# fpthink/PDGN

Hardware: AMD Instinct MI355X
Metric: generator+D step points/sec (B=35, 256->2048 pts) (higher is better)
Workload: dtype f32; 1 GPU; PDGNet_v2 G+D iteration (models/PDGNet_v2.py:171-256), chair-shaped synthetic batch, per-GPU batch 35, 256->2048 pts, random-init weights; global_batch=35, parallelism=dp1, losses_finite=True, hipgraph=False, issue=list

## Files before the change

### include/pdgn_hip.h

```cpp
#ifndef PDGN_HIP_H
#define PDGN_HIP_H

#include <stdint.h>

#ifdef __cplusplus
extern "C" {
#endif

#define PDGN_ERR_INVALID (-1)
#define PDGN_KNN_MAX_NSAMPLE 200

typedef void *pdgn_stream_t;

#define PDGN_ABI_VERSION 38
int pdgn_abi_version(void);

int pdgn_knnquery(int b, int n, int m, int nsample, const float *xyz, const float *new_xyz,
                  int32_t *idx, float *dist2, pdgn_stream_t stream);

int pdgn_grouping_forward(int b, int c, int n, int m, int nsample, const float *points,
                          const int32_t *idx, float *out, pdgn_stream_t stream);

int pdgn_grouping_backward(int b, int c, int n, int m, int nsample, const float *grad_out,
                           const int32_t *idx, float *grad_points, pdgn_stream_t stream);

int pdgn_nearestneighbor(int b, int n, int m, const float *unknown, const float *known,
                         float *dist2, int32_t *idx, pdgn_stream_t stream);

int pdgn_interpolation_forward(int b, int c, int m, int n, const float *points,
                               const int32_t *idx, const float *weight, float *out,
                               pdgn_stream_t stream);

int pdgn_interpolation_backward(int b, int c, int n, int m, const float *grad_out,
                                const int32_t *idx, const float *weight, float *grad_points,
                                pdgn_stream_t stream);

int pdgn_nndistance(int b, int n, const float *xyz, int m, const float *xyz2, float *result,
                    int32_t *result_i, float *result2, int32_t *result2_i, pdgn_stream_t stream);

int pdgn_nndistance_grad(int b, int n, const float *xyz1, int m, const float *xyz2,
                         const float *grad_dist1, const int32_t *idx1, const float *grad_dist2,
                         const int32_t *idx2, float *grad_xyz1, float *grad_xyz2,
                         pdgn_stream_t stream);

int pdgn_approxmatch(int b, int n, int m, const float *xyz1, const float *xyz2, float *match,
                     float *temp, pdgn_stream_t stream);

int pdgn_matchcost(int b, int n, int m, const float *xyz1, const float *xyz2,
                   const float *match, float *out, pdgn_stream_t stream);

int pdgn_matchcost_grad(int b, int n, int m, const float *xyz1, const float *xyz2,
                        const float *match, float *grad1, float *grad2, pdgn_stream_t stream);

long long pdgn_emd_cost_temp_floats(long long pairs, int n, int m);
int pdgn_emd_cost(int b, int n, int m, const float *xyz1, const float *xyz2, float *temp,
                  float *out, pdgn_stream_t stream);

int pdgn_feature_knn(int b, int f, int n, int k, const float *x, float *sqnorm, int32_t *idx,
                     pdgn_stream_t stream);

int pdgn_window_gather_sum(int b, int n, int k, int ldy, int T, int P, int C, int off, int offc,
                           const float *Y, const int32_t *idx, const float *bias, int bias_bstride,
                           float *out, pdgn_stream_t stream);
int pdgn_window_gather_sum_stats(int b, int n, int k, int ldy, int T, int P, int C, int off, int offc,
                                 const float *Y, const int32_t *idx, const float *bias, int bias_bstride,
                                 float *out, float *scratch, pdgn_stream_t stream);

int pdgn_window_gather_sum_backward(int b, int n, int k, int ldy, int T, int P, int C, int off,
                                    int offc, const float *dout, const int32_t *idx, float *dY,
                                    pdgn_stream_t stream);

int pdgn_knn_graph_transpose(int b, int n, int k, const int32_t *idx, int32_t *rowptr, int32_t *edges,
                             int32_t *scratch, pdgn_stream_t stream);
int pdgn_window_gather_sum_backward_csr(int b, int n, int k, int ldy, int T, int P, int C, int off,
                                        int offc, const float *dout, const int32_t *rowptr,
                                        const int32_t *edges, float *dY, unsigned *max_out, int max_init, pdgn_stream_t stream);

long long pdgn_bn_scratch_floats(long long rows, int c);
int pdgn_bn_stats(long long rows, int c, float eps, float momentum, const float *x, const float *gamma,
                  const float *beta, const float *pre_bias, float *running_mean, float *running_var,
                  float *scratch, float *stats, pdgn_stream_t stream);
int pdgn_bn_eval_stats(int c, float eps, const float *gamma, const float *beta, const float *pre_bias,
                       const float *running_mean, const float *running_var, float *stats,
                       pdgn_stream_t stream);
int pdgn_bn_stats_from_partials(long long rows, int c, float eps, float momentum, const float *gamma,
                                const float *beta, const float *pre_bias, float *running_mean, float *running_var,
                                const float *scratch, float *stats, pdgn_stream_t stream);
int pdgn_bn_stats_from_gemm_partials(long long rows, int c, long long nparts, int block_rows, float eps, float momentum,
                                     const float *gamma, const float *beta, const float *pre_bias,
                                     float *running_mean, float *running_var, const float *partials,
                                     float *stats, double *scratch, pdgn_stream_t stream);
long long pdgn_bn_blocks_scratch_doubles(int c, long long nparts);
int pdgn_bn_act_forward(long long rows, int c, int act, const float *x, const float *stats,
                        const float *mul, float *y, int interleave_n, pdgn_stream_t stream);
int pdgn_bn_act_backward(long long rows, int c, int act, int training, const float *x,
                         const float *dy, const float *mul, const float *stats, float *scratch,
                         float *bsums, float *dx, float *dmul, int interleave_n, pdgn_stream_t stream);

long long pdgn_bn_maxpool_scratch_floats(int b, int c);
int pdgn_bn_act_maxpool(int b, int n, int c, int act, const float *x, const float *stats, float *scratch,
                        float *ymax, int32_t *yarg, pdgn_stream_t stream);
long long pdgn_bn_stats_maxpool_scratch_floats(int b, int c);
int pdgn_bn_stats_act_maxpool(int b, int n, int c, int act, float eps, float momentum, const float *x, const float *gamma,
                              const float *beta, const float *pre_bias, float *running_mean, float *running_var, float *scratch,
                              float *stats, float *ymax, int32_t *yarg, pdgn_stream_t stream);
int pdgn_bn_act_maxpool_backward(int b, int n, int c, int act, int training, const float *x,
                                 const float *dout, const int32_t *yarg, const float *stats,
                                 float *scratch, float *bsums, float *dx, pdgn_stream_t stream);
long long pdgn_dense_bn_maxpool_backward_scratch(int b, int c, int k);
int pdgn_dense_bn_maxpool_backward(int b, int n, int c, int k, int act, const float *x, const float *dout, const int32_t *yarg,
                                   const float *stats, const float *h, int ldh, const float *W, int ldw, float *scratch,
                                   float *dh, float *dW, int lddw, float *bsums, pdgn_stream_t stream);
long long pdgn_dense_bn_maxpool_input_grad_scratch(int b, int c, int k);
int pdgn_dense_bn_maxpool_input_grad(int b, int n, int c, int k, int act, const float *x, const float *dout,
                                     const int32_t *yarg, const float *stats, const float *h, int ldh,
                                     const float *W, int ldw, float *scratch, float *dh, pdgn_stream_t stream);

int pdgn_group_colsum(long long groups, long long group_rows, int c, const float *x, long long ldx, float *out,
                      pdgn_stream_t stream);

int pdgn_softmax_slots_permute(long long m, int k, int c, const float *h, float *w, pdgn_stream_t stream);
int pdgn_bn_softmax_slots_permute(long long m, int k, int c, int act, const float *x, const float *stats,
                                  float *w, pdgn_stream_t stream);
int pdgn_bn_softmax_slots_permute_mul(long long m, int k, int c, int act, const float *x, const float *stats,
                                      int act_u, const float *u, const float *stats_u, float *w, float *y,
                                      unsigned *max_out, const float *gamma_u, const float *beta_u, float bound_scale,
                                      unsigned *cmax_out, pdgn_stream_t stream);
long long pdgn_bilateral_scratch_floats(long long m, int k, int c);
int pdgn_bilateral_weighting_backward(long long m, int k, int c, int act, int training, const float *x,
                                      const float *stats_x, const float *u, const float *stats_u, const float *w,
                                      const float *dy, float *scratch, float *bsums_x, float *bsums_u, float *dx,
                                      float *du, pdgn_stream_t stream);
int pdgn_softmax_slots_permute_backward(long long m, int k, int c, const float *w, const float *dw,
                                        float *dh, pdgn_stream_t stream);

int pdgn_skinny_nt(int R, int N, int K, const float *A, int lda, const float *B, int ldb, const float *bias, float *C, int ldc,
                   pdgn_stream_t stream);
int pdgn_skinny_nn(int R, int N, int K, const float *A, int lda, const float *B, int ldb, float *C, int ldc, pdgn_stream_t stream);
int pdgn_skinny_nt_act(int R, int N, int K, const float *A, int lda, const float *B, int ldb, const float *bias, float *C, int ldc,
                       int act, pdgn_stream_t stream);
int pdgn_skinny_nn_masked(int R, int N, int K, const float *A, int lda, const float *P, int ldp, int act, const float *B,
                          int ldb, float *C, int ldc, pdgn_stream_t stream);
int pdgn_skinny_tn(int R, int N, int K, const float *A, int lda, const float *B, int ldb, float *C, int ldc, pdgn_stream_t stream);
int pdgn_split_bf16x3(int rows, int cols, const float *src, int ld_src, unsigned short *planes, int ld_planes,
                      long long plane_stride, unsigned short *planes_t, int ld_planes_t, long long plane_stride_t,
                      pdgn_stream_t stream);
int pdgn_gemm_nt_ps(long long m, int n, int k, const float *A, int lda, const unsigned short *Wplanes, int ldw, long long wplane,
                    int parts, const float *bias, const float *addend, int ldadd, float *C, int ldc, float *stat_part,
                    const float *row_bias, int ld_rb, int rows_per_group, int act, const float *gate, int ldgate,
                    pdgn_stream_t stream);
long long pdgn_gemm_tail_workspace_floats(long long m, int n, int k, int with_stats);
long long pdgn_gemm_tn_big_workspace_floats(long long m, int n, int k);
int pdgn_gemm_set_tail_workspace(float *ws, long long floats);
int pdgn_gemm_nt_ps_launch_info(long long m, int n, int k, int parts, const void **sym, int *grid);
int pdgn_gemm_aux_symbols(const void **reduce, const void **scan);
int pdgn_gemm_set_mode(int mode);
int pdgn_gemm_set_scale_slots(void *slots, long long bytes);
int pdgn_absmax_rows_cols(long long rows, int cols, const float *src, int ld, unsigned *rowmax, unsigned *colmax,
                          pdgn_stream_t stream);
int pdgn_gemm_set_operand_scales(const unsigned *max_a, const unsigned *max_w);
int pdgn_gemm_two_part(long long m, int n, int k, long long scan_bytes);
int pdgn_gemm_two_part_planes(long long m, int n, int k, long long scan_bytes);
long long pdgn_gemm_nt_ps_stat_rows(long long m, int n, int k, int parts, int plain);
int pdgn_gemm_nt_ps_stat_block_rows(long long m, int n, int k, int parts, int plain);
int pdgn_gemm_nt_ps_row_panel(long long m, int n, int k, int parts, int plain);
long long pdgn_gemm_nt_ps_workspace_floats(long long m, int n, int k, int parts, int with_stats);
int pdgn_split_f16x2(int rows, int cols, const float *src, int ld_src, unsigned short *planes, int ld_planes,
                     long long plane_stride, unsigned short *planes_t, int ld_planes_t, long long plane_stride_t,
                     pdgn_stream_t stream);
int pdgn_gemm_set_config(int cfg);
int pdgn_gemm_set_shape(int shape);
int pdgn_gemm_nt(long long m, int n, int k, const float *A, int lda, const float *W, int ldw,
                 const float *bias, const float *addend, int ldadd, float *C, int ldc, float *stat_part,
                 pdgn_stream_t stream);
long long pdgn_thin_stat_rows(long long m);
int pdgn_thin_stat_block_rows(void);
int pdgn_thin_nt(long long m, int n, int k, const float *X, int ldx, const float *W, int wrs, int wcs,
                 const float *bias, float *Y, int ldy, float *stat_part, pdgn_stream_t stream);
int pdgn_thin_nt_ex(long long m, int n, int k, const float *X, int ldx, const float *W, int wrs, int wcs,
                    const float *bias, float *Y, int ldy, float *stat_part, const float *gate, int ldgate, pdgn_stream_t stream);
int pdgn_thin_tn(long long m, int ta, int wb, const float *A, int lda, const float *B, int ldb, float *O, int osi,
                 int osj, float *sum_a, float *sum_b, pdgn_stream_t stream);
int pdgn_gemm_nn(long long m, int n, int k, const float *A, int lda, const float *Wt, int ldw,
                 const float *bias, const float *addend, int ldadd, float *C, int ldc, float *stat_part,
                 pdgn_stream_t stream);
int pdgn_gemm_tn_big(long long m, int n, int k, const float *dY, int ldy, const float *X, int ldx, float *dW, int dw_is_zero,
                     pdgn_stream_t stream);
int pdgn_gemm_nt_ex(long long m, int n, int k, const float *A, int lda, const float *W, int ldw, const float *bias,
                    const float *addend, int ldadd, float *C, int ldc, float *stat_part, const float *row_bias, int ld_rb,
                    int rows_per_group, int act, const float *gate, int ldgate, int transposed_w, pdgn_stream_t stream);
long long pdgn_gemm_nt_stat_rows(long long m, int n, int k);
int pdgn_gemm_nt_stat_block_rows(long long m, int n, int k);
int pdgn_gemm_nt_config(long long m, int n, int k, int with_stats);

int pdgn_gemm_tn(long long m, int n, int k, const float *dY, const float *X, float *dW,
                 pdgn_stream_t stream);

int pdgn_local_stats(int b, int n, int m, int k, const float *xyz, const int32_t *idx, float *mu,
                     float *cov, pdgn_stream_t stream);
int pdgn_local_stats_backward(int b, int n, int m, int k, const float *xyz, const int32_t *idx,
                              const float *dmu, const float *dcov, float *dxyz, pdgn_stream_t stream);

int pdgn_chamfer_gram(int b, int m, int n, int d, const float *x, const float *y, float *minx,
                      int32_t *argx, float *miny, int32_t *argy, pdgn_stream_t stream);
int pdgn_chamfer_gram_grad(int b, int m, int n, int d, const float *x, const float *y,
                           const float *gminx, const int32_t *argx, const float *gminy,
                           const int32_t *argy, float *gx, float *gy, pdgn_stream_t stream);
int pdgn_chamfer_gram_grad_uniform(int b, int m, int n, int d, const float *x, const float *y, const float *g,
                                   float scale, const int32_t *argx, const int32_t *argy, float *gx, float *gy,
                                   pdgn_stream_t stream);
int pdgn_scaled_sum(long long n, const float *x, float scale, float *out, pdgn_stream_t stream);
int pdgn_mse_const(long long n, const float *x, float target, float scale, float *out, pdgn_stream_t stream);
int pdgn_mse_const_count(long long n, const float *x, float target, float scale, float boundary, float *out, int32_t *count,
                         pdgn_stream_t stream);
int pdgn_mse_const_backward(long long n, const float *x, float target, float scale, const float *g, float *dx,
                            pdgn_stream_t stream);

int pdgn_emd_cost_indexed(int npairs, int n, int m, const float *xyz1, const int32_t *ia,
                          const float *xyz2, const int32_t *ib, float *temp, float *out,
                          pdgn_stream_t stream);
int pdgn_chamfer_gram_indexed(int npairs, int m, int n, int d, const float *x, const int32_t *ia,
                              const float *y, const int32_t *ib, float *minx, int32_t *argx,
                              float *miny, int32_t *argy, pdgn_stream_t stream);

int pdgn_deconv_assemble(int F, int Fo, int k, int T, int fc, const float *Wi, const float *W2, const float *Wf,
                         float *WcatC, float *WcatV, float *Wb, pdgn_stream_t stream);
int pdgn_deconv_assemble_backward(int F, int Fo, int k, int T, int fc, const float *gWcatC, const float *gWcatV,
                                  const float *gWb, float *dWi, float *dW2, float *dWf, pdgn_stream_t stream);

int pdgn_sample_bias(int b, int ldy, int nspec, const int *T, const int *C, const int *off, const int *offc,
                     const float *const *bias, const float *Yc, float *bb, pdgn_stream_t stream);
int pdgn_sample_bias_backward(int b, int ldy, int nspec, const int *T, const int *C, const int *off, const int *offc,
                              const float *g, float *dYc, float *const *dbias, pdgn_stream_t stream);

int pdgn_small_mlp_forward(int r, int k, int n, int act, int bn_mode, float eps, float momentum, const float *x,
                           const float *W, const float *bias, const float *gamma, const float *beta,
                           float *running_mean, float *running_var, float *y, float *pre, float *stat,
                           pdgn_stream_t stream);
int pdgn_small_mlp_backward(int r, int k, int n, int act, int bn_mode, const float *x, const float *dy, const float *pre,
                            const float *stat, const float *gamma, const float *beta, float *dpre, float *dgamma,
                            float *dbeta, float *dbias, float *dW, pdgn_stream_t stream);

int pdgn_ballquery(int b, int n, int m, float radius, int nsample, const float *new_xyz, const float *xyz,
                   int32_t *idx, pdgn_stream_t stream);
int pdgn_furthestsampling(int b, int n, int m, const float *xyz, float *temp, int32_t *idx, pdgn_stream_t stream);
int pdgn_gathering_forward(int b, int c, int n, int m, const float *points, const int32_t *idx, float *out,
                           pdgn_stream_t stream);
int pdgn_gathering_backward(int b, int c, int n, int m, const float *grad_out, const int32_t *idx,
                            float *grad_points, pdgn_stream_t stream);
int pdgn_grouping_int_forward(int b, int c, int n, int m, int nsample, const long long *points, const int32_t *idx,
                              long long *out, pdgn_stream_t stream);
int pdgn_featuredistribute(int b, int n, int m, const float *max_xyz, const float *xyz, int32_t *distribute_idx,
                           pdgn_stream_t stream);
int pdgn_labelstat_idx(int b, int n, int m, int nsample, int nclass, const int32_t *label_stat, const int32_t *idx,
                       int32_t *new_label_stat, pdgn_stream_t stream);
int pdgn_labelstat_ballrange(int b, int n, int m, float radius, int nclass, const float *new_xyz, const float *xyz,
                             const int32_t *label_stat, int32_t *new_label_stat, pdgn_stream_t stream);
int pdgn_labelstat_and_ballquery(int b, int n, int m, float radius, int nsample, int nclass, const float *new_xyz,
                                 const float *xyz, const int32_t *label_stat, int32_t *idx, int32_t *new_label_stat,
                                 pdgn_stream_t stream);

long long pdgn_point_max_scratch(int b, int n, int c);
int pdgn_point_max(int b, int n, int c, const float *x, float *scratch_val, int32_t *scratch_arg, float *out, int32_t *arg,
                   pdgn_stream_t stream);
int pdgn_point_max_backward(int b, int n, int c, const float *grad_out, const int32_t *arg, float *grad_x,
                            pdgn_stream_t stream);

int pdgn_spin(unsigned int microseconds, pdgn_stream_t stream);

// ... 147 lines not shown
```

### pdgn_amd/csrc/bnact.hip

```cpp
#include "common.h"

#include "bn_geom.h"
#define ACT_NONE 0
#define ACT_RELU 1
#define ACT_LEAKY 2

__device__ __forceinline__ float act_fwd(float z, int act) {
    if (act == ACT_RELU) return fmaxf(z, 0.f);
    if (act == ACT_LEAKY) return z > 0.f ? z : 0.01f * z;
    return z;
}
__device__ __forceinline__ float act_grad(float z, int act) {
    if (act == ACT_RELU) return z > 0.f ? 1.f : 0.f;
    if (act == ACT_LEAKY) return z > 0.f ? 1.f : 0.01f;
    return 1.f;
}

struct ClGeom {
    int cg, cgb, rl;
};

__global__ __launch_bounds__(BN_THREADS) void cl_stats_kernel(long long R, int C, int cgb, int rows_per_block,
                                                              const float *__restrict__ x,
                                                              float *__restrict__ part) {
// ... 784 lines not shown
    return pdgn_launch_status();
}

#define MP_SPLIT 16

__global__ __launch_bounds__(BN_THREADS) void cl_apply_max_kernel(int N, int C, int cgb, int act,
                                                                  const float *__restrict__ x,
                                                                  const float *__restrict__ stats,
                                                                  float *__restrict__ pmax, int32_t *__restrict__ parg) {
    __shared__ float smax[BN_THREADS][4];
    __shared__ int sarg[BN_THREADS][4];
    const int cgl = threadIdx.x % cgb, rlane = threadIdx.x / cgb, rl = BN_THREADS / cgb;
    const int cgi = blockIdx.x * cgb + cgl;
    const bool cok = cgi * 4 < C;
    const int b = blockIdx.z, sp = blockIdx.y;
    const int per = (N + MP_SPLIT - 1) / MP_SPLIT;
    const int n0 = sp * per, n1 = min(N, n0 + per);
    float best[4] = {-INFINITY, -INFINITY, -INFINITY, -INFINITY};
    int arg[4] = {n0, n0, n0, n0};
    if (cok) {
        float sc[4], sh[4];
        *reinterpret_cast<float4 *>(sc) = *reinterpret_cast<const float4 *>(stats + cgi * 4);
        *reinterpret_cast<float4 *>(sh) = *reinterpret_cast<const float4 *>(stats + C + cgi * 4);
        const float *X = x + ((size_t)b * N) * C + cgi * 4;
        for (int n = n0 + rlane; n < n1; n += rl) {
            float v[4];
            *reinterpret_cast<float4 *>(v) = *reinterpret_cast<const float4 *>(X + (size_t)n * C);
#pragma unroll
            for (int j = 0; j < 4; ++j) {
                const float y = act_fwd(__fmaf_rn(v[j], sc[j], sh[j]), act);
                if (y > best[j]) { best[j] = y; arg[j] = n; }
            }
        }
    }
#pragma unroll
    for (int j = 0; j < 4; ++j) { smax[threadIdx.x][j] = best[j]; sarg[threadIdx.x][j] = arg[j]; }
    __syncthreads();
    if (rlane == 0 && cok) {
        for (int q = 1; q < rl; ++q)
#pragma unroll
            for (int j = 0; j < 4; ++j) {
                const float y = smax[q * cgb + cgl][j];
                const int a = sarg[q * cgb + cgl][j];
                if (y > best[j] || (y == best[j] && a < arg[j])) { best[j] = y; arg[j] = a; }
            }
        const size_t o = ((size_t)b * MP_SPLIT + sp) * C + cgi * 4;
        *reinterpret_cast<float4 *>(pmax + o) = *reinterpret_cast<float4 *>(best);
        *reinterpret_cast<int4 *>(parg + o) = *reinterpret_cast<int4 *>(arg);
    }
}

__global__ void cl_max_finalize_kernel(int B, int C, const float *__restrict__ pmax, const int32_t *__restrict__ parg,
                                       float *__restrict__ ymax, int32_t *__restrict__ yarg) {
    const int e = blockIdx.x * blockDim.x + threadIdx.x;
    if (e >= B * C) return;
    const int b = e / C, c = e % C;
    float best = -INFINITY;
    int arg = 0;
    for (int s = 0; s < MP_SPLIT; ++s) {
        const float y = pmax[((size_t)b * MP_SPLIT + s) * C + c];
        if (y > best) { best = y; arg = parg[((size_t)b * MP_SPLIT + s) * C + c]; }
    }
    ymax[e] = best;
    yarg[e] = arg;
}

__global__ __launch_bounds__(BN_THREADS) void cl_stats_max_kernel(int N, int C, int cgb, const float *__restrict__ x,
                                                                  float *__restrict__ part, float *__restrict__ pmax,
                                                                  int32_t *__restrict__ pargmax, float *__restrict__ pmin,
                                                                  int32_t *__restrict__ pargmin) {
    __shared__ float4 red[4][BN_THREADS];
    __shared__ int4 redi[2][BN_THREADS];
    const int cgl = threadIdx.x % cgb, rlane = threadIdx.x / cgb, rl = BN_THREADS / cgb;
    const int cgi = blockIdx.x * cgb + cgl;
    const bool cok = cgi * 4 < C;
    const int b = blockIdx.z, sp = blockIdx.y;
    const int per = (N + MP_SPLIT - 1) / MP_SPLIT;
    const int n0 = sp * per, n1 = min(N, n0 + per);
    float s[4] = {0.f, 0.f, 0.f, 0.f}, q[4] = {0.f, 0.f, 0.f, 0.f};
    float mx[4] = {-INFINITY, -INFINITY, -INFINITY, -INFINITY}, mn[4] = {INFINITY, INFINITY, INFINITY, INFINITY};
    int amx[4] = {n0, n0, n0, n0}, amn[4] = {n0, n0, n0, n0};
    if (cok) {
        float pv[4];
        *reinterpret_cast<float4 *>(pv) = *reinterpret_cast<const float4 *>(x + cgi * 4);
        const float *X = x + ((size_t)b * N) * C + cgi * 4;
        for (int n = n0 + rlane; n < n1; n += rl) {
            float v[4];
            *reinterpret_cast<float4 *>(v) = *reinterpret_cast<const float4 *>(X + (size_t)n * C);
#pragma unroll
            for (int j = 0; j < 4; ++j) {
                const float d = v[j] - pv[j];
                s[j] += d;
                q[j] = __fmaf_rn(d, d, q[j]);
                if (v[j] > mx[j]) { mx[j] = v[j]; amx[j] = n; }
                if (v[j] < mn[j]) { mn[j] = v[j]; amn[j] = n; }
            }
        }
    }
    red[0][threadIdx.x] = make_float4(s[0], s[1], s[2], s[3]);
    red[1][threadIdx.x] = make_float4(q[0], q[1], q[2], q[3]);
    red[2][threadIdx.x] = make_float4(mx[0], mx[1], mx[2], mx[3]);
    red[3][threadIdx.x] = make_float4(mn[0], mn[1], mn[2], mn[3]);
    redi[0][threadIdx.x] = make_int4(amx[0], amx[1], amx[2], amx[3]);
    redi[1][threadIdx.x] = make_int4(amn[0], amn[1], amn[2], amn[3]);
    __syncthreads();
    if (rlane || !cok) return;
    for (int k = 1; k < rl; ++k) {
        const int t = k * cgb + cgl;
        const float *a = &red[0][t].x, *bq = &red[1][t].x, *c2 = &red[2][t].x, *d2 = &red[3][t].x;
        const int *i2 = &redi[0][t].x, *j2 = &redi[1][t].x;
#pragma unroll
        for (int j = 0; j < 4; ++j) {
            s[j] += a[j];
            q[j] += bq[j];
            if (c2[j] > mx[j] || (c2[j] == mx[j] && i2[j] < amx[j])) { mx[j] = c2[j]; amx[j] = i2[j]; }
            if (d2[j] < mn[j] || (d2[j] == mn[j] && j2[j] < amn[j])) { mn[j] = d2[j]; amn[j] = j2[j]; }
        }
    }
    const size_t blk = (size_t)b * MP_SPLIT + sp;
    float *P = part + blk * 2 * C;
    *reinterpret_cast<float4 *>(P + cgi * 4) = make_float4(s[0], s[1], s[2], s[3]);
    *reinterpret_cast<float4 *>(P + C + cgi * 4) = make_float4(q[0], q[1], q[2], q[3]);
    const size_t o = blk * C + cgi * 4;
    *reinterpret_cast<float4 *>(pmax + o) = make_float4(mx[0], mx[1], mx[2], mx[3]);
    *reinterpret_cast<int4 *>(pargmax + o) = make_int4(amx[0], amx[1], amx[2], amx[3]);
    *reinterpret_cast<float4 *>(pmin + o) = make_float4(mn[0], mn[1], mn[2], mn[3]);
    *reinterpret_cast<int4 *>(pargmin + o) = make_int4(amn[0], amn[1], amn[2], amn[3]);
}

__global__ void cl_max_pick_kernel(int B, int C, int act, const float *__restrict__ stats, const float *__restrict__ pmax,
                                   const int32_t *__restrict__ pargmax, const float *__restrict__ pmin,
                                   const int32_t *__restrict__ pargmin, float *__restrict__ ymax, int32_t *__restrict__ yarg) {
    const int e = blockIdx.x * blockDim.x + threadIdx.x;
    if (e >= B * C) return;
    const int b = e / C, c = e - b * C;
    const float sc = stats[c], sh = stats[C + c];
    const bool up = sc >= 0.f;
    const float *pv = up ? pmax : pmin;
    const int32_t *pa = up ? pargmax : pargmin;
    float best = pv[((size_t)b * MP_SPLIT) * C + c];
    int arg = pa[((size_t)b * MP_SPLIT) * C + c];
    for (int s = 1; s < MP_SPLIT; ++s) {
        const float v = pv[((size_t)b * MP_SPLIT + s) * C + c];
        if (up ? v > best : v < best) { best = v; arg = pa[((size_t)b * MP_SPLIT + s) * C + c]; }
    }
    ymax[e] = act_fwd(__fmaf_rn(best, sc, sh), act);
    yarg[e] = arg;
}

__global__ __launch_bounds__(256) void cl_max_bwd_sums_kernel(int B, int N, int C, int act, int training,
                                                              const float *__restrict__ x, const float *__restrict__ dout,
                                                              const int32_t *__restrict__ yarg, const float *__restrict__ stats,
                                                              float *__restrict__ dz, float *__restrict__ bsums,
                                                              float *__restrict__ coef, float *__restrict__ zero, int nzero) {
    __shared__ double p1[16][17], p2[16][17];
    for (int e = blockIdx.x * 256 + threadIdx.x; e < nzero; e += gridDim.x * 256) zero[e] = 0.f;
    const int cl = threadIdx.x & 15, bl = threadIdx.x >> 4;
    const int c = blockIdx.x * 16 + cl;
    double s1 = 0, s2 = 0;
    float sc = 0.f, mu = 0.f, is = 0.f;
    if (c < C) {
        sc = stats[c];
        mu = stats[2 * C + c];
        is = stats[3 * C + c];
        const float sh = stats[C + c];
        for (int b = bl; b < B; b += 16) {
            const int n = yarg[b * C + c];
            const float v = x[((size_t)b * N + n) * C + c];
            const float g = dout[b * C + c] * act_grad(__fmaf_rn(v, sc, sh), act);
            dz[b * C + c] = g;
            s1 += g;
            s2 += (double)g * (double)((v - mu) * is);
        }
    }
    p1[bl][cl] = s1;
    p2[bl][cl] = s2;
    __syncthreads();
    if (bl || c >= C) return;
    for (int q = 1; q < 16; ++q) { s1 += p1[q][cl]; s2 += p2[q][cl]; }
    bsums[c] = (float)s1;
    bsums[C + c] = (float)s2;
    float ca = 0.f, cb = 0.f;
    if (training) {
        const double R = (double)B * (double)N;
        cb = sc * is * (float)(s2 / R);
        ca = sc * (float)(s1 / R) - cb * mu;
    }
    coef[c] = ca;
    coef[C + c] = cb;
}

__global__ __launch_bounds__(BN_THREADS) void cl_max_bwd_apply_kernel(int N, int C, int cgb, const float *__restrict__ x,
                                                                      const float *__restrict__ stats,
                                                                      const float *__restrict__ coef,
                                                                      const float *__restrict__ dz,
                                                                      const int32_t *__restrict__ yarg,
                                                                      float *__restrict__ dx) {
    const int cgl = threadIdx.x % cgb, rlane = threadIdx.x / cgb, rl = BN_THREADS / cgb;
    const int cgi = blockIdx.x * cgb + cgl;
    if (cgi * 4 >= C) return;
    const int b = blockIdx.z, sp = blockIdx.y;
    const int per = (N + MP_SPLIT - 1) / MP_SPLIT;
    const int n0 = sp * per, n1 = min(N, n0 + per);
    float sc[4], ca[4], cb[4], g[4];
    int arg[4];
    *reinterpret_cast<float4 *>(sc) = *reinterpret_cast<const float4 *>(stats + cgi * 4);
    *reinterpret_cast<float4 *>(ca) = *reinterpret_cast<const float4 *>(coef + cgi * 4);
    *reinterpret_cast<float4 *>(cb) = *reinterpret_cast<const float4 *>(coef + C + cgi * 4);
    *reinterpret_cast<float4 *>(g) = *reinterpret_cast<const float4 *>(dz + (size_t)b * C + cgi * 4);
    *reinterpret_cast<int4 *>(arg) = *reinterpret_cast<const int4 *>(yarg + (size_t)b * C + cgi * 4);
    const size_t base = ((size_t)b * N) * C + cgi * 4;
    for (int n = n0 + rlane; n < n1; n += rl) {
        float v[4], o[4];
        *reinterpret_cast<float4 *>(v) = *reinterpret_cast<const float4 *>(x + base + (size_t)n * C);
#pragma unroll
        for (int j = 0; j < 4; ++j) o[j] = (n == arg[j] ? sc[j] * g[j] : 0.f) - ca[j] - cb[j] * v[j];
        *reinterpret_cast<float4 *>(dx + base + (size_t)n * C) = *reinterpret_cast<float4 *>(o);
    }
}

static void mp_geometry(int C, int *cgb, int *gx) {
    const int cg = C / 4;
    int p = 1;
    while (p < cg && p < 64) p <<= 1;
    *cgb = p;
    *gx = (cg + p - 1) / p;
}

extern "C" long long pdgn_bn_maxpool_scratch_floats(int b, int c) { return 2LL * b * MP_SPLIT * c; }

extern "C" int pdgn_bn_act_maxpool(int b, int n, int c, int act, const float *x, const float *stats, float *scratch,
                                   float *ymax, int32_t *yarg, pdgn_stream_t stream) {
    if (b < 1 || n < 1 || c < 4 || c % 4 || act < 0 || act > 2 || b > 65535) return PDGN_ERR_INVALID;
    hipStream_t s = (hipStream_t)stream;
    int cgb, gx;
    mp_geometry(c, &cgb, &gx);
    float *pmax = scratch;
    int32_t *parg = reinterpret_cast<int32_t *>(scratch + (size_t)b * MP_SPLIT * c);
    hipLaunchKernelGGL(cl_apply_max_kernel, dim3(gx, MP_SPLIT, b), dim3(BN_THREADS), 0, s, n, c, cgb, act, x, stats, pmax, parg);
    hipLaunchKernelGGL(cl_max_finalize_kernel, dim3(cdiv((long long)b * c, 256)), dim3(256), 0, s, b, c, pmax, parg, ymax, yarg);
    return pdgn_launch_status();
}

extern "C" long long pdgn_bn_stats_maxpool_scratch_floats(int b, int c) { return 6LL * b * MP_SPLIT * c; }

extern "C" int pdgn_bn_stats_act_maxpool(int b, int n, int c, int act, float eps, float momentum, const float *x, const float *gamma,
                                         const float *beta, const float *pre_bias, float *running_mean, float *running_var,
                                         float *scratch, float *stats, float *ymax, int32_t *yarg, pdgn_stream_t stream) {
    if (b < 1 || n < 1 || c < 4 || c % 4 || act < 0 || act > 2 || b > 65535) return PDGN_ERR_INVALID;
    hipStream_t s = (hipStream_t)stream;
    int cgb, gx;
    mp_geometry(c, &cgb, &gx);
    const size_t bc = (size_t)b * MP_SPLIT * c;
    float *part = scratch, *pmax = part + 2 * bc, *pmin = pmax + 2 * bc;
    int32_t *pargmax = reinterpret_cast<int32_t *>(pmax + bc), *pargmin = reinterpret_cast<int32_t *>(pmin + bc);
    hipLaunchKernelGGL(cl_stats_max_kernel, dim3(gx, MP_SPLIT, b), dim3(BN_THREADS), 0, s, n, c, cgb, x, part, pmax, pargmax, pmin,
                       pargmin);
    hipLaunchKernelGGL(cl_finalize_kernel, dim3(cdiv(c, FIN_CH)), dim3(FIN_CH * FIN_PL), 0, s, (long long)b * n, c, b * MP_SPLIT, eps,
                       momentum, part, gamma, beta, pre_bias, running_mean, running_var, stats, x);
    hipLaunchKernelGGL(cl_max_pick_kernel, dim3(cdiv((long long)b * c, 256)), dim3(256), 0, s, b, c, act, stats, pmax, pargmax, pmin,
                       pargmin, ymax, yarg);
    return pdgn_launch_status();
}

extern "C" int pdgn_bn_act_maxpool_backward(int b, int n, int c, int act, int training, const float *x,
                                            const float *dout, const int32_t *yarg, const float *stats, float *scratch,
                                            float *bsums, float *dx, pdgn_stream_t stream) {
    if (b < 1 || n < 1 || c < 4 || c % 4 || act < 0 || act > 2 || b > 65535) return PDGN_ERR_INVALID;
    hipStream_t s = (hipStream_t)stream;
    float *dz = scratch, *coef = scratch + (size_t)b * c;
    hipLaunchKernelGGL(cl_max_bwd_sums_kernel, dim3(cdiv(c, 16)), dim3(256), 0, s, b, n, c, act, training, x, dout, yarg,
                       stats, dz, bsums, coef, nullptr, 0);
    int cgb, gx;
    mp_geometry(c, &cgb, &gx);
    hipLaunchKernelGGL(cl_max_bwd_apply_kernel, dim3(gx, MP_SPLIT, b), dim3(BN_THREADS), 0, s, n, c, cgb, x, stats, coef, dz,
                       yarg, dx);
    return pdgn_launch_status();
}

#define CF_TILE 32
#define CF_CSPLIT 8
#define CF_RSPLIT 32

__global__ __launch_bounds__(256) void cf_gram_kernel(int C, int K, const float *__restrict__ W, int ldw,
                                                      const float *__restrict__ coef, float *__restrict__ Gneg,
                                                      float *__restrict__ vneg) {
    __shared__ float part[3][64][20];
    const int t = threadIdx.x, o = t & 63, sl = __builtin_amdgcn_readfirstlane(t >> 6);
    const int i = blockIdx.y * CF_TILE + (o >> 3) * 4, j = blockIdx.x * CF_TILE + (o & 7) * 4;
    const bool ok = i < K && j < K, do_v = blockIdx.y == 0 && (o >> 3) == 0 && j < K;
    const int ii = min(i, K - 4), jj = min(j, K - 4);
    const int nsl = CF_CSPLIT * 4, per = (C + nsl - 1) / nsl;
    const int c0 = (blockIdx.z * 4 + sl) * per, c1 = min(C, c0 + per);
    const float *cb = coef + C;
    float acc[4][4] = {}, av[4] = {};
    for (int c = c0; c < c1; c += 8) {
        float4 wi[8], wj[8];
#pragma unroll
        for (int u = 0; u < 8; ++u) {
            const float *w = W + (size_t)min(c + u, c1 - 1) * ldw;
            wi[u] = *reinterpret_cast<const float4 *>(w + ii);
            wj[u] = *reinterpret_cast<const float4 *>(w + jj);
        }
        __builtin_amdgcn_sched_barrier(0);
#pragma unroll
        for (int u = 0; u < 8; ++u) {
            const int cc = min(c + u, c1 - 1);
            const float live = c + u < c1 ? 1.f : 0.f;
            const float s = cb[cc] * live, a = coef[cc] * live;
            const float x[4] = {wi[u].x * s, wi[u].y * s, wi[u].z * s, wi[u].w * s};
            const float y[4] = {wj[u].x, wj[u].y, wj[u].z, wj[u].w};
#pragma unroll
            for (int p = 0; p < 4; ++p)
#pragma unroll
                for (int q = 0; q < 4; ++q) acc[p][q] = __fmaf_rn(x[p], y[q], acc[p][q]);
#pragma unroll
            for (int q = 0; q < 4; ++q) av[q] = __fmaf_rn(a, y[q], av[q]);
        }
    }
    if (sl) {
#pragma unroll
        for (int p = 0; p < 4; ++p)
#pragma unroll
            for (int q = 0; q < 4; ++q) part[sl - 1][o][p * 4 + q] = acc[p][q];
#pragma unroll
        for (int q = 0; q < 4; ++q) part[sl - 1][o][16 + q] = av[q];
    }
    __syncthreads();
    if (sl) return;
#pragma unroll
    for (int w = 0; w < 3; ++w) {
#pragma unroll
        for (int p = 0; p < 4; ++p)
#pragma unroll
            for (int q = 0; q < 4; ++q) acc[p][q] += part[w][o][p * 4 + q];
#pragma unroll
        for (int q = 0; q < 4; ++q) av[q] += part[w][o][16 + q];
    }
    if (ok)
#pragma unroll
        for (int p = 0; p < 4; ++p)
#pragma unroll
            for (int q = 0; q < 4; ++q) atomicAdd(&Gneg[(size_t)(i + p) * K + j + q], -acc[p][q]);
    if (do_v)
#pragma unroll
        for (int q = 0; q < 4; ++q) atomicAdd(&vneg[j + q], -av[q]);
}

__global__ __launch_bounds__(256) void cf_scatter_kernel(int N, int C, int K, const float *__restrict__ W, int ldw,
                                                         const float *__restrict__ stats, const float *__restrict__ dz,
                                                         const int32_t *__restrict__ yarg, float *__restrict__ dh) {
    extern __shared__ unsigned char cf_lds[];
    __shared__ unsigned int ndist;
    const int maxd = min(N, C);
    unsigned short *table = reinterpret_cast<unsigned short *>(cf_lds);
    unsigned short *rows = table + N;
    unsigned short *args = rows + maxd;
    unsigned int *cnt = reinterpret_cast<unsigned int *>(cf_lds + (((size_t)(N + maxd + C) * 2 + 15) & ~(size_t)15));
    float *cf = reinterpret_cast<float *>(cnt + 256);
    const int t = threadIdx.x, b = blockIdx.y;
    const int32_t *arg = yarg + (size_t)b * C;
    for (int n = t; n < N; n += 256) table[n] = 0;
    __syncthreads();
    for (int c = t; c < C; c += 256) {
        const int a = arg[c];
        table[a] = 1;
        args[c] = (unsigned short)a;
        cf[c] = stats[c] * dz[(size_t)b * C + c];
    }
    __syncthreads();
    const int per = (N + 255) / 256, lo = t * per, hi = min(N, lo + per);
    unsigned int mine = 0;
    for (int n = lo; n < hi; ++n) mine += table[n];
    cnt[t] = mine;
    __syncthreads();
    if (t < 64) {
        const unsigned int v0 = cnt[4 * t], v1 = cnt[4 * t + 1], v2 = cnt[4 * t + 2], v3 = cnt[4 * t + 3];
        const unsigned int s = v0 + v1 + v2 + v3;
        unsigned int incl = s;
#pragma unroll
        for (int d = 1; d < 64; d <<= 1) {
            const unsigned int up = __shfl_up(incl, d, 64);
            if (t >= d) incl += up;
        }
        const unsigned int ex = incl - s;
        cnt[4 * t] = ex;
        cnt[4 * t + 1] = ex + v0;
        cnt[4 * t + 2] = ex + v0 + v1;
        cnt[4 * t + 3] = ex + v0 + v1 + v2;
    }
    __syncthreads();
    unsigned int at = cnt[t];
    for (int n = lo; n < hi; ++n)
        if (table[n]) rows[at++] = (unsigned short)n;
    if (t == 255) ndist = at;
    __syncthreads();
    const int nd = (int)ndist, lane = t & 63, wv = t >> 6;
    const bool lok = lane * 4 < K;
    const int col = min(lane * 4, K - 4);
    for (int r = blockIdx.x * 4 + wv; r < nd; r += CF_RSPLIT * 4) {
        const int n = rows[r];
        float *dst = dh + ((size_t)b * N + n) * K + col;
        const float4 cur = *reinterpret_cast<const float4 *>(dst);
        float4 acc = make_float4(0.f, 0.f, 0.f, 0.f);
        for (int c0 = 0; c0 < C; c0 += 64) {
            unsigned long long m = __ballot(c0 + lane < C && args[min(c0 + lane, C - 1)] == n);
            while (m) {
                const int c = c0 + __builtin_ctzll(m);
                m &= m - 1;
                const float g = cf[c];
                const float4 w = *reinterpret_cast<const float4 *>(W + (size_t)c * ldw + col);
                acc.x = __fmaf_rn(g, w.x, acc.x);
                acc.y = __fmaf_rn(g, w.y, acc.y);
                acc.z = __fmaf_rn(g, w.z, acc.z);
                acc.w = __fmaf_rn(g, w.w, acc.w);
            }
        }
        if (lok) *reinterpret_cast<float4 *>(dst) = make_float4(cur.x + acc.x, cur.y + acc.y, cur.z + acc.z, cur.w + acc.w);
    }
}

static size_t cf_scatter_lds(int n, int c) {
    const int maxd = n < c ? n : c;
    return (((size_t)(n + maxd + c) * 2 + 15) & ~(size_t)15) + 256 * 4 + (size_t)c * 4;
}

#define CFS_THREADS 1024
__global__ __launch_bounds__(CFS_THREADS) void cf_colsum_kernel(long long rows, int K, const float *__restrict__ h, int ldh,
                                                                float *__restrict__ hs) {
    __shared__ float4 red[CFS_THREADS];
    const int kg = K / 4, cg = threadIdx.x % kg, rl = threadIdx.x / kg, nrl = CFS_THREADS / kg;
    const long long per = (rows + gridDim.x - 1) / gridDim.x, r0 = blockIdx.x * per, r1 = min(rows, r0 + per);
    float4 acc = make_float4(0.f, 0.f, 0.f, 0.f);
    for (long long r = r0 + rl; r < r1; r += 8 * nrl) {
        float4 v[8];
#pragma unroll
        for (int u = 0; u < 8; ++u) {
            const long long rr = r + (long long)u * nrl;
            v[u] = rr < r1 ? *reinterpret_cast<const float4 *>(h + rr * ldh + cg * 4) : make_float4(0.f, 0.f, 0.f, 0.f);
        }
#pragma unroll
        for (int u = 0; u < 8; ++u) { acc.x += v[u].x; acc.y += v[u].y; acc.z += v[u].z; acc.w += v[u].w; }
    }
    red[threadIdx.x] = acc;
    __syncthreads();
    if (rl) return;
    for (int q = 1; q < nrl; ++q) {
        const float4 v = red[q * kg + cg];
        acc.x += v.x; acc.y += v.y; acc.z += v.z; acc.w += v.w;
    }
    atomicAdd(&hs[cg * 4], acc.x); atomicAdd(&hs[cg * 4 + 1], acc.y); atomicAdd(&hs[cg * 4 + 2], acc.z); atomicAdd(&hs[cg * 4 + 3], acc.w);
}

__global__ __launch_bounds__(256) void cf_dw_kernel(int B, int N, int C, int K, const float *__restrict__ h, int ldh,
                                                    const int32_t *__restrict__ yarg, const float *__restrict__ stats,
                                                    const float *__restrict__ dz, const float *__restrict__ coef,
                                                    const float *__restrict__ hs, const float *__restrict__ T,
                                                    float *__restrict__ dW, int lddw) {
    const int lane = threadIdx.x & 63, c = blockIdx.x * 4 + (threadIdx.x >> 6);
    if (c >= C || lane * 4 >= K) return;
    const int col = lane * 4;
    const float sc = stats[c];
    float4 acc = make_float4(0.f, 0.f, 0.f, 0.f);
    for (int b0 = 0; b0 < B; b0 += 8) {
        float4 v[8];
        float g[8];
#pragma unroll
        for (int u = 0; u < 8; ++u) {
            const int b = min(b0 + u, B - 1);
            g[u] = b0 + u < B ? sc * dz[(size_t)b * C + c] : 0.f;
            v[u] = *reinterpret_cast<const float4 *>(h + ((size_t)b * N + yarg[(size_t)b * C + c]) * ldh + col);
        }
#pragma unroll
        for (int u = 0; u < 8; ++u) {
            acc.x = __fmaf_rn(g[u], v[u].x, acc.x);
            acc.y = __fmaf_rn(g[u], v[u].y, acc.y);
            acc.z = __fmaf_rn(g[u], v[u].z, acc.z);
            acc.w = __fmaf_rn(g[u], v[u].w, acc.w);
        }
    }
    const float ca = coef[c], cb = coef[C + c];
    const float4 s = *reinterpret_cast<const float4 *>(hs + col), t = *reinterpret_cast<const float4 *>(T + (size_t)c * K + col);
    *reinterpret_cast<float4 *>(dW + (size_t)c * lddw + col) =
        make_float4(acc.x - ca * s.x - cb * t.x, acc.y - ca * s.y - cb * t.y, acc.z - ca * s.z - cb * t.z, acc.w - ca * s.w - cb * t.w);
}

extern "C" long long pdgn_dense_bn_maxpool_backward_scratch(int b, int c, int k) {
    return (long long)b * c + 2LL * c + 2LL * ((long long)k * k + k) + (long long)c * k;
}

extern "C" int pdgn_dense_bn_maxpool_backward(int b, int n, int c, int k, int act, const float *x, const float *dout,
                                              const int32_t *yarg, const float *stats, const float *h, int ldh, const float *W,
                                              int ldw, float *scratch, float *dh, float *dW, int lddw, float *bsums,
                                              pdgn_stream_t stream) {
    if (b < 1 || n < 1 || n > 65535 || c < 4 || c % 4 || k < 4 || k % 4 || k > 256 || ldw % 4 || ((uintptr_t)W & 15) ||
        ((uintptr_t)dh & 15) || act < 0 || act > 2 || b > 65535 || cf_scatter_lds(n, c) > 64 * 1024)
        return PDGN_ERR_INVALID;
    if (dW && (k < 16 || (k & (k - 1)) || ldh % 4 || lddw % 4 || ((uintptr_t)h & 15) || ((uintptr_t)dW & 15)))
        return PDGN_ERR_INVALID;
    hipStream_t s = (hipStream_t)stream;
    const size_t kk = (size_t)k * k;
    float *dz = scratch, *coef = dz + (size_t)b * c, *G = coef + 2 * (size_t)c, *v = G + kk, *H = v + k, *hs = H + kk, *T = hs + k;
    float *bs = bsums ? bsums : T;
    hipLaunchKernelGGL(cl_max_bwd_sums_kernel, dim3(cdiv(c, 16)), dim3(256), 0, s, b, n, c, act, 1, x, dout, yarg, stats, dz, bs,
                       coef, G, (int)(2 * (kk + k)));
    int rc = pdgn_launch_status();
    if (rc) return rc;
    if (dh) {
        const int gt = cdiv(k, CF_TILE);
        hipLaunchKernelGGL(cf_gram_kernel, dim3(gt, gt, CF_CSPLIT), dim3(256), 0, s, c, k, W, ldw, coef, G, v);
        if ((rc = pdgn_launch_status())) return rc;
        if ((rc = pdgn_gemm_nt((long long)b * n, k, k, h, ldh, G, k, v, nullptr, 0, dh, k, nullptr, stream))) return rc;
        hipLaunchKernelGGL(cf_scatter_kernel, dim3(CF_RSPLIT, b), dim3(256), cf_scatter_lds(n, c), s, n, c, k, W, ldw, stats, dz,
                           yarg, dh);
        if ((rc = pdgn_launch_status())) return rc;
    }
    if (dW) {
        const long long rows = (long long)b * n;
        hipLaunchKernelGGL(cf_colsum_kernel, dim3(rows >= 32768 ? 128 : (rows >= 8192 ? 64 : 16)), dim3(CFS_THREADS), 0, s, rows, k, h, ldh, hs);
        if ((rc = pdgn_launch_status())) return rc;
        if ((rc = pdgn_gemm_tn_big(rows, k, k, h, ldh, h, ldh, H, 1, stream))) return rc;
        if ((rc = pdgn_gemm_nt(c, k, k, W, ldw, H, k, nullptr, nullptr, 0, T, k, nullptr, stream))) return rc;
        hipLaunchKernelGGL(cf_dw_kernel, dim3(cdiv(c, 4)), dim3(256), 0, s, b, n, c, k, h, ldh, yarg, stats, dz, coef, hs, T, dW, lddw);
        rc = pdgn_launch_status();
    }
    return rc;
}

extern "C" long long pdgn_dense_bn_maxpool_input_grad_scratch(int b, int c, int k) {
    return pdgn_dense_bn_maxpool_backward_scratch(b, c, k);
}

extern "C" int pdgn_dense_bn_maxpool_input_grad(int b, int n, int c, int k, int act, const float *x, const float *dout,
                                                const int32_t *yarg, const float *stats, const float *h, int ldh,
                                                const float *W, int ldw, float *scratch, float *dh, pdgn_stream_t stream) {
    return pdgn_dense_bn_maxpool_backward(b, n, c, k, act, x, dout, yarg, stats, h, ldh, W, ldw, scratch, dh, nullptr, 4, nullptr,
                                          stream);
}

__global__ __launch_bounds__(256) void group_colsum_kernel(long long group_rows, int C, const float *__restrict__ x, long long ldx,
                                                           float *__restrict__ out) {
    __shared__ float4 red[256];
    const int kg = C / 4, per_pass = kg < 256 ? kg : 256;
    const int cgl = threadIdx.x % per_pass, rl = threadIdx.x / per_pass, nrl = 256 / per_pass;
    const long long g = blockIdx.y;
    const long long per = (group_rows + gridDim.x - 1) / gridDim.x, r0 = blockIdx.x * per, r1 = min(group_rows, r0 + per);
    const float *X = x + g * group_rows * ldx;
    for (int c0 = 0; c0 < kg; c0 += per_pass) {
        const int cg = c0 + cgl;
        float4 acc = make_float4(0.f, 0.f, 0.f, 0.f);
        for (long long r = r0 + rl; r < r1; r += 8 * nrl) {
            float4 v[8];
#pragma unroll
            for (int u = 0; u < 8; ++u) {
                const long long rr = r + (long long)u * nrl;
                v[u] = rr < r1 ? *reinterpret_cast<const float4 *>(X + rr * ldx + cg * 4) : make_float4(0.f, 0.f, 0.f, 0.f);
            }
#pragma unroll
            for (int u = 0; u < 8; ++u) { acc.x += v[u].x; acc.y += v[u].y; acc.z += v[u].z; acc.w += v[u].w; }
        }
        __syncthreads();
        red[threadIdx.x] = acc;
        __syncthreads();
        if (rl == 0) {
            for (int q = 1; q < nrl; ++q) {
                const float4 v = red[q * per_pass + cgl];
                acc.x += v.x; acc.y += v.y; acc.z += v.z; acc.w += v.w;
            }
            float *o = out + g * C + cg * 4;
            if (gridDim.x == 1) *reinterpret_cast<float4 *>(o) = acc;
            else { atomicAdd(o, acc.x); atomicAdd(o + 1, acc.y); atomicAdd(o + 2, acc.z); atomicAdd(o + 3, acc.w); }
        }
    }
}

extern "C" int pdgn_group_colsum(long long groups, long long group_rows, int c, const float *x, long long ldx, float *out,
                                 pdgn_stream_t stream) {
    if (groups < 1 || group_rows < 1 || c < 16 || c > 1024 || (c & (c - 1)) || ldx < c || ldx % 4 || ((uintptr_t)x & 15) ||
        ((uintptr_t)out & 15) || groups > 65535)
        return PDGN_ERR_INVALID;
    const int kg = c / 4, nrl = kg < 256 ? 256 / kg : 1;
    long long splits = 1024 / groups;
    splits = splits > 128 ? 128 : splits;
    const long long max_splits = group_rows / (8LL * nrl * 8) > 0 ? group_rows / (8LL * nrl * 8) : 1;
    splits = splits < 1 ? 1 : (splits > max_splits ? max_splits : splits);
    hipLaunchKernelGGL(group_colsum_kernel, dim3((unsigned)splits, (unsigned)groups), dim3(256), 0, (hipStream_t)stream, group_rows, c, x,
                       ldx, out);
    return pdgn_launch_status();
}
```

### pdgn_amd/csrc/gemm_shared.h

```cpp
#pragma once
#include <type_traits>

#include "common.h"

typedef float f32x4 __attribute__((ext_vector_type(4)));
typedef unsigned u32x4 __attribute__((ext_vector_type(4)));
typedef __attribute__((address_space(3))) void lds_void_t;

#define NT_BK 32
#define NT_GROUP_M 8
#define NT_OOB 0x40000000u

typedef int i32x4 __attribute__((ext_vector_type(4)));

__device__ __forceinline__ i32x4 nt_srd(const void *base, unsigned bytes) {
    const unsigned long long b = (unsigned long long)base;
    i32x4 r;
    r.x = __builtin_amdgcn_readfirstlane((int)(unsigned)b);
    r.y = __builtin_amdgcn_readfirstlane((int)((unsigned)(b >> 32) & 0xffffu));
    r.z = __builtin_amdgcn_readfirstlane((int)bytes);
    r.w = 0x00020000;
    return r;
}

__device__ __forceinline__ void nt_dma16(i32x4 srd, unsigned lds_base, unsigned voff, unsigned soff) {
    asm volatile("s_mov_b32 m0, %0\n\ts_nop 0\n\tbuffer_load_dwordx4 %1, %2, %3 offen lds"
                 :
                 : "s"(lds_base), "v"(voff), "s"(srd), "s"(soff)
                 : "memory", "m0");
}

struct NtArgs {
    long long M;
    int N, K, lda, ldw, ldc, ldadd;
    const float *A, *W, *bias, *addend;
    float *C, *stat_part;
    int tiles_m, tiles_n, tile_begin, tile_end, kchunks;
    long long sk_per_wg;
    int sk_split;
    float *sk_ws;
    int sk_seg;
    int dbg;
    const float *row_bias;
    int ld_rb, rows_per_group;
    unsigned rpg_magic;
    int rb_bytes;
    int act;
    const float *gate;
    int ldgate;
    const unsigned short *Wp;
    long long wplane;
    const unsigned *max_a, *max_w;
};

__device__ __forceinline__ int x2_exponent(unsigned maxbits) {
    const int e = 14 - ((int)(maxbits >> 23) - 127);
    return e > 126 ? 126 : (e < -126 ? -126 : e);
}
__device__ __forceinline__ int x2_scale_field(unsigned maxbits) {
    const int f = 268 - (int)(maxbits >> 23);
    return f < 1 ? 1 : (f > 253 ? 253 : f);
}
__device__ __forceinline__ float x2_scale(unsigned maxbits) { return __int_as_float(x2_scale_field(maxbits) << 23); }
__device__ __forceinline__ float x2_unscale(unsigned maxbits) { return __int_as_float((254 - x2_scale_field(maxbits)) << 23); }

struct NtDev {
    int cus;
};
static inline int nt_cus() {
    static int cached = 0;
    if (!cached) {
        int dev = 0, cus = 0;
        if (hipGetDevice(&dev) != hipSuccess ||
            hipDeviceGetAttribute(&cus, hipDeviceAttributeMultiprocessorCount, dev) != hipSuccess || cus < 1)
            return 256;
        cached = cus;
    }
    return cached;
}

struct NtSwitches {
    int mode, cfg, splitk, shape16, shape16_default;
};
NtSwitches &nt_switches();

struct NtEpi {
    const float *row_bias = nullptr;
    int ld_rb = 0, rows_per_group = 1, act = 0;
    const float *gate = nullptr;
    int ldgate = 0;
    bool any() const { return row_bias || act || gate; }
};


int fp32_gemm_nt(long long m, int n, int k, const float *A, int lda, const float *W, int ldw, const float *bias,
                 const float *addend, int ldadd, float *C, int ldc, float *stat_part, pdgn_stream_t stream);
int fp32_gemm_nn(long long m, int n, int k, const float *A, int lda, const float *Wt, int ldw, const float *bias,
                 const float *addend, int ldadd, float *C, int ldc, float *stat_part, pdgn_stream_t stream);
int fp32_gemm_nt_ex(long long m, int n, int k, const float *A, int lda, const float *W, int ldw, const float *bias,
                    const float *addend, int ldadd, float *C, int ldc, float *stat_part, const float *row_bias, int ld_rb,
                    int rows_per_group, int act, const float *gate, int ldgate, int transposed_w, pdgn_stream_t stream);
int fp32_gemm_tn_big(long long m, int n, int k, const float *dY, int ldy, const float *X, int ldx, float *dW,
                     pdgn_stream_t stream);
long long fp32_gemm_nt_stat_rows(long long m, int n, int k);
int fp32_gemm_nt_stat_block_rows(long long m, int n, int k);
int fp32_gemm_nt_config(long long m, int n, int k, int with_stats);
```

### pdgn_amd/csrc/gemm_x3.hip

```cpp
#include <atomic>
#include <type_traits>

#include "gemm_shared.h"

#ifndef X3_FENCE
#define X3_FENCE 2
#endif
#ifndef X3_DEFAULT_MASK
#define X3_DEFAULT_MASK 0x000
#endif
#ifndef X3_FENCE16
#define X3_FENCE16 2
#endif
#ifndef X3_ABLATE
#define X3_ABLATE 0
#endif

typedef float f32x16 __attribute__((ext_vector_type(16)));
typedef float f32x2 __attribute__((ext_vector_type(2)));
typedef __bf16 bf16x8 __attribute__((ext_vector_type(8)));
typedef __bf16 bf16x2 __attribute__((ext_vector_type(2)));

struct X3Parts {
    u32x4 h, m, l;
};

__device__ __forceinline__ unsigned x3_cvt_pk(float a, float b) {
    const f32x2 v = {a, b};
    return __builtin_bit_cast(unsigned, __builtin_convertvector(v, bf16x2));
}

__device__ __forceinline__ void x3_split_pair(float a, float b, X3Parts &P, int e) {
    const unsigned h = x3_cvt_pk(a, b);
    const float ra = a - __uint_as_float(h << 16), rb = b - __uint_as_float(h & 0xffff0000u);
    const unsigned m = x3_cvt_pk(ra, rb);
    const float sa = ra - __uint_as_float(m << 16), sb = rb - __uint_as_float(m & 0xffff0000u);
    P.h[e] = h;
    P.m[e] = m;
    P.l[e] = x3_cvt_pk(sa, sb);
}

__device__ __forceinline__ f32x16 x3_mfma(const u32x4 a, const u32x4 b, const f32x16 c) {
    return __builtin_amdgcn_mfma_f32_32x32x16_bf16(__builtin_bit_cast(bf16x8, a), __builtin_bit_cast(bf16x8, b), c, 0, 0, 0);
}

typedef _Float16 f16x8 __attribute__((ext_vector_type(8)));
typedef _Float16 f16x2 __attribute__((ext_vector_type(2)));
__device__ __forceinline__ unsigned x2_cvt_pk(float a, float b) {
    const f32x2 v = {a, b};
    return __builtin_bit_cast(unsigned, __builtin_convertvector(v, f16x2));
}
__device__ __forceinline__ f32x16 x2_mfma(const u32x4 a, const u32x4 b, const f32x16 c) {
    return __builtin_amdgcn_mfma_f32_32x32x16_f16(__builtin_bit_cast(f16x8, a), __builtin_bit_cast(f16x8, b), c, 0, 0, 0);
}
#ifndef X2_PRODUCTS
#define X2_PRODUCTS 3
#endif

typedef float f32x4a __attribute__((ext_vector_type(4)));
__device__ __forceinline__ f32x4a x3_mfma16(const u32x4 a, const u32x4 b, const f32x4a c) {
    return __builtin_amdgcn_mfma_f32_16x16x32_bf16(__builtin_bit_cast(bf16x8, a), __builtin_bit_cast(bf16x8, b), c, 0, 0, 0);
}

template <int MS>
__device__ __forceinline__ unsigned x3_sw(unsigned r) {
    const unsigned x = (r >> 2) & 3u;
    return MS == 32 ? x : ((0x78u >> (2u * x)) & 3u);
}

template <int CTRL, int ROW_MASK>
__device__ __forceinline__ float x3_dpp_add(float v) {
    return v + __int_as_float(__builtin_amdgcn_update_dpp(0, __float_as_int(v), CTRL, ROW_MASK, 0xf, true));
}

__device__ __forceinline__ float x3_half_wave_sum(float v) {
    v = x3_dpp_add<0x111, 0xf>(v);
    v = x3_dpp_add<0x112, 0xf>(v);
    v = x3_dpp_add<0x114, 0xf>(v);
    v = x3_dpp_add<0x118, 0xf>(v);
    return x3_dpp_add<0x142, 0xa>(v);
}

__device__ __forceinline__ float x3_row_sum(float v) {
    v = x3_dpp_add<0x111, 0xf>(v);
    v = x3_dpp_add<0x112, 0xf>(v);
    v = x3_dpp_add<0x114, 0xf>(v);
    return x3_dpp_add<0x118, 0xf>(v);
}

template <int TM, int TN, int WM, int WN, int OCC, bool ATOMIC, bool WT, bool AT, bool EPI = false, bool PW = false, int MS = 32, int NP = 3>
__global__ __launch_bounds__(64 * WM * WN, OCC) void gemm_x3_kernel(const NtArgs p) {
    static_assert(!PW || (!WT && !AT), "pre-split second operand: row-major (N x K) planes only");
    static_assert(MS == 32 || MS == 16, "matrix instruction: 32x32x16 or 16x16x32");
    static_assert(NP == 3 || (NP == 2 && MS == 32), "parts: three bf16, or two fp16 on the 32x32x16 instruction");
    constexpr int NW = WM * WN, NTH = 64 * NW, BM = 32 * TM * WM, BN = 32 * TN * WN;
    constexpr int PART_A = BM * 64, PART_W = BN * 64, STAGE = NP * (PART_A + PART_W);
    constexpr int UNT = NP == 2 ? (BM + BN) * 4 : 0;
    constexpr bool STG = OCC == 1 && !ATOMIC && !(X3_ABLATE & 128) && 2 * STAGE + NW * 4096 + UNT <= 160 * 1024;
    __shared__ __attribute__((aligned(1024))) unsigned char smem[2 * STAGE + (STG ? NW * 4096 : 0) + UNT];
    float *const untab = reinterpret_cast<float *>(smem + 2 * STAGE + (STG ? NW * 4096 : 0));

    const int tid = threadIdx.x, lane = tid & 63;
    const int wave = __builtin_amdgcn_readfirstlane(tid >> 6);
    const int wm = wave / WN, wn = wave % WN;
    const int li = MS == 32 ? lane & 31 : lane & 15, lg = MS == 32 ? lane >> 5 : lane >> 4;

    const int G = gridDim.x, pid = blockIdx.x;
    const int gq = G >> 3, gr = G & 7, xcd = pid & 7;
    const int v = xcd * gq + min(xcd, gr) + (pid >> 3);

    const int KC = p.kchunks;
    auto decode = [&](int tile, int &tm, int &tn) {
        const int per_group = NT_GROUP_M * p.tiles_n;
        const int grp = tile / per_group, r = tile - grp * per_group;
        const int first = grp * NT_GROUP_M;
        const int gsz = min(NT_GROUP_M, p.tiles_m - first);
        tn = r / gsz;
        tm = first + (r - tn * gsz);
    };
    struct Cur {
        int tile, kb, kc, ke;
        int j;
        long long f, f1;
        bool valid;
    };
    auto next_item = [&](Cur &c) {
        if (p.sk_split && (ATOMIC || p.sk_ws)) {
            const int slice = v / p.sk_split;
            c.tile = p.tile_begin + v % p.sk_split;
            c.kc = c.kb = (int)(slice * p.sk_per_wg);
            c.ke = min(KC, c.kb + (int)p.sk_per_wg);
            c.valid = c.j == 0 && c.kb < KC;
            c.j++;
        } else if (ATOMIC || (p.sk_ws && p.sk_seg)) {
            c.valid = c.f < c.f1;
            c.j++;
            if (c.valid) {
                c.tile = p.tile_begin + (int)(c.f / KC);
                c.kc = c.kb = (int)(c.f % KC);
                const long long left = c.f1 - c.f;
                c.ke = (left < (long long)(KC - c.kc)) ? c.kc + (int)left : KC;
                c.f += c.ke - c.kc;
            }
        } else {
            c.tile = p.tile_begin + v + c.j * G;
            c.valid = c.tile < p.tile_end;
            c.kc = c.kb = 0;
            c.ke = KC;
            c.j++;
        }
    };
    Cur ld, cp;
    ld.j = 0;
    ld.f = (long long)v * p.sk_per_wg;
    {
        const long long total = (long long)(p.tile_end - p.tile_begin) * KC;
        ld.f1 = min(total, ld.f + p.sk_per_wg);
    }
    ld.tile = ld.kb = ld.kc = ld.ke = 0;
    ld.valid = false;
    next_item(ld);
    cp = ld;
    if (!ld.valid) return;

    constexpr int QA = BM * 8 / NTH, QW = PW ? BN * 4 / NTH : BN * 8 / NTH, NQ = QA + QW;
    static_assert(QA * NTH == BM * 8 && QW * NTH == BN * (PW ? 4 : 8), "loader quads must divide over the threads");
    constexpr int CUA = QA % 4 == 0 ? 4 : 2, CUW = QW % 4 == 0 ? 4 : 2;
    static_assert((!AT || QA % CUA == 0) && (!WT || QW % CUW == 0), "transposed operand: whole units per thread");
    float raw[NQ][4];
    unsigned rawp[PW ? QW : 1][12];
    unsigned goffA0, goffW0, woffA0, woffW0;
    int kqA, kqW;
    {
        const int r8 = lane >> 3, c16 = lane & 7;
        kqA = kqW = c16;
        if (!AT) {
            const int row = wave * 8 + r8;
            goffA0 = (unsigned)(row * p.lda + 4 * c16) * 4u;
            woffA0 = (unsigned)(row * 64 + (((c16 >> 1) ^ x3_sw<MS>(row)) * 16) + (c16 & 1) * 8);
        } else {
            const int cq = tid % (BM / CUA), kq = tid / (BM / CUA);
            goffA0 = (unsigned)((4 * kq) * p.lda + CUA * cq) * 4u;
            woffA0 = 0;
        }
        if (PW) {
            const int row = tid >> 2, col = tid & 3;
            kqW = 2 * col;
            goffW0 = (unsigned)(row * p.ldw + 8 * col) * 2u;
            woffW0 = (unsigned)(NP * PART_A + row * 64 + ((col ^ x3_sw<MS>(row)) * 16));
        } else if (!WT) {
            const int row = wave * 8 + r8;
            goffW0 = (unsigned)(row * p.ldw + 4 * c16) * 4u;
            woffW0 = (unsigned)(NP * PART_A + row * 64 + (((c16 >> 1) ^ x3_sw<MS>(row)) * 16) + (c16 & 1) * 8);
        } else {
            const int cq = tid % (BN / CUW), kq = tid / (BN / CUW);
            goffW0 = (unsigned)((4 * kq) * p.ldw + CUW * cq) * 4u;
            woffW0 = 0;
        }
    }
    constexpr int KQ_STEP_A = NTH / (BM / CUA > NTH ? NTH : BM / CUA), KQ_STEP_W = NTH / (BN / CUW > NTH ? NTH : BN / CUW);
    static_assert(!AT || (BM / CUA <= NTH && NTH % (BM / CUA) == 0), "A^T units");
    static_assert(!WT || (BN / CUW <= NTH && NTH % (BN / CUW) == 0), "W^T units");

    __amdgpu_buffer_rsrc_t rsA, rsW;
    long long ld_m0 = 0;
    int ld_n0 = 0, ld_mrows = 0, ld_nrows = 0;
    constexpr int NSA = NP == 2 ? (AT ? CUA : QA) : 1, NSW = (NP == 2 && !PW) ? (WT ? CUW : QW) : 1;
    float scA[NSA], scW[NSW];
    unsigned nxA[NSA], nxW[NSW];
    auto make_srds = [&](int tile) {
        int tm, tn;
        decode(tile, tm, tn);
        ld_m0 = (long long)tm * BM;
        ld_n0 = tn * BN;
        ld_mrows = (int)min((long long)BM, p.M - ld_m0);
        ld_nrows = min(BN, p.N - ld_n0);
    };
    make_srds(ld.tile);
    auto fetch_maxima = [&]() {
        if (NP != 2) return;
        int lane_ = __builtin_amdgcn_mbcnt_hi(~0u, __builtin_amdgcn_mbcnt_lo(~0u, 0u));
        asm volatile("" : "+v"(lane_));
        const int tid_ = wave * 64 + lane_;
        const __amdgpu_buffer_rsrc_t rA = __builtin_amdgcn_make_buffer_rsrc((void *)(p.max_a + ld_m0), 0, ld_mrows * 4, 0x00020000);
        if (!AT) {
#pragma unroll
            for (int j = 0; j < NSA; ++j) nxA[j] = (unsigned)__builtin_amdgcn_raw_buffer_load_b32(rA, (unsigned)(wave * 8 + (lane_ >> 3) + j * NW * 8) * 4u, 0, 0);
        } else if (CUA == 4) {
            const u32x4 x = __builtin_bit_cast(u32x4, __builtin_amdgcn_raw_buffer_load_b128(rA, (unsigned)(tid_ % (BM / CUA)) * 16u, 0, 0));
#pragma unroll
            for (int j = 0; j < NSA; ++j) nxA[j] = x[j];
        } else {
            typedef unsigned u32x2_ __attribute__((ext_vector_type(2)));
            const u32x2_ x = __builtin_bit_cast(u32x2_, __builtin_amdgcn_raw_buffer_load_b64(rA, (unsigned)(tid_ % (BM / CUA)) * 8u, 0, 0));
#pragma unroll
            for (int j = 0; j < NSA; ++j) nxA[j] = x[j];
        }
        if (PW) return;
        const __amdgpu_buffer_rsrc_t rW = __builtin_amdgcn_make_buffer_rsrc((void *)(p.max_w + ld_n0), 0, ld_nrows * 4, 0x00020000);
        if (!WT) {
#pragma unroll
            for (int j = 0; j < NSW; ++j) nxW[j] = (unsigned)__builtin_amdgcn_raw_buffer_load_b32(rW, (unsigned)(wave * 8 + (lane_ >> 3) + j * NW * 8) * 4u, 0, 0);
        } else if (CUW == 4) {
            const u32x4 x = __builtin_bit_cast(u32x4, __builtin_amdgcn_raw_buffer_load_b128(rW, (unsigned)(tid_ % (BN / CUW)) * 16u, 0, 0));
#pragma unroll
            for (int j = 0; j < NSW; ++j) nxW[j] = x[j];
        } else {
            typedef unsigned u32x2_ __attribute__((ext_vector_type(2)));
            const u32x2_ x = __builtin_bit_cast(u32x2_, __builtin_amdgcn_raw_buffer_load_b64(rW, (unsigned)(tid_ % (BN / CUW)) * 8u, 0, 0));
#pragma unroll
            for (int j = 0; j < NSW; ++j) nxW[j] = x[j];
// ... 93 lines not shown
            const float a2 = a * sc, b2 = b * sc;
            const unsigned h = x2_cvt_pk(a2, b2);
            const f16x2 hh = __builtin_bit_cast(f16x2, h);
            cvh[e] = h;
            cvl[e] = x2_cvt_pk(a2 - (float)hh[0], b2 - (float)hh[1]);
            return;
        }
        const unsigned h = x3_cvt_pk(a, b);
        const float ra = a - __uint_as_float(h << 16), rb = b - __uint_as_float(h & 0xffff0000u);
        const unsigned m = x3_cvt_pk(ra, rb);
        const float sa = ra - __uint_as_float(m << 16), sb = rb - __uint_as_float(m & 0xffff0000u);
        cvh[e] = h;
        cvm[e] = m;
        cvl[e] = x3_cvt_pk(sa, sb);
    };
    auto conv_write = [&](int st, int q) {
        const bool isA = q < QA;
        const bool tr = isA ? AT : WT;
        const int j = isA ? q : q - QA;
        const int ps = isA ? PART_A : PART_W;
        unsigned off = isA ? woffA0 : woffW0;
        if (PW && !isA) {
            off += (unsigned)(j * (NTH / 4) * 64);
        } else if (!tr) {
            off += (unsigned)(j * NW * 8 * 64);
        } else {
            const int CU = isA ? CUA : CUW;
            const int d = (j / CU) * (isA ? KQ_STEP_A : KQ_STEP_W);
            const int kq0 = isA ? (int)(tid / (BM / CUA)) : (int)(tid / (BN / CUW));
            const int cq = isA ? (int)(tid % (BM / CUA)) : (int)(tid % (BN / CUW));
            const int row = CU * cq + (j % CU), kq = kq0 + d;
            off = (unsigned)((isA ? 0 : NP * PART_A) + row * 64 + (((kq >> 1) ^ x3_sw<MS>(row)) * 16) + (kq & 1) * 8);
        }
        unsigned char *dst = smem + st * STAGE + off;
        typedef unsigned u32x2 __attribute__((ext_vector_type(2)));
        if (PW && !isA) {
#pragma unroll
            for (int part = 0; part < NP; ++part)
                *reinterpret_cast<u32x4 *>(dst + part * ps) = (u32x4){rawp[j][4 * part], rawp[j][4 * part + 1], rawp[j][4 * part + 2], rawp[j][4 * part + 3]};
            return;
        }
        if (X3_ABLATE & 64) {
            *reinterpret_cast<u32x2 *>(dst) = (u32x2){cvh[0] ^ cvm[0] ^ cvl[0], cvh[1] ^ cvm[1] ^ cvl[1]};
            return;
        }
        *reinterpret_cast<u32x2 *>(dst) = (u32x2){cvh[0], cvh[1]};
        if (NP == 2) {
            *reinterpret_cast<u32x2 *>(dst + ps) = (u32x2){cvl[0], cvl[1]};
            return;
        }
        *reinterpret_cast<u32x2 *>(dst + ps) = (u32x2){cvm[0], cvm[1]};
        *reinterpret_cast<u32x2 *>(dst + 2 * ps) = (u32x2){cvl[0], cvl[1]};
    };

    constexpr int FR = MS == 32 ? 32 : 16;
    constexpr int FA = 32 * TM / FR, FW = 32 * TN / FR, NPAR = MS == 32 ? 2 : 1;
    const unsigned a_rd = (unsigned)((wm * 32 * TM + li) * 64 + ((lg ^ x3_sw<MS>(li)) * 16));
    const unsigned w_rd = (unsigned)(NP * PART_A + (wn * 32 * TN + li) * 64 + ((lg ^ x3_sw<MS>(li)) * 16));
    X3Parts fa[NPAR][FA], fw[NPAR][FW];
    auto read_frag = [&](int st, int s, int par, int r) {
        const int f = r / NP, part = NP == 2 ? 2 * (r % NP) : r % NP;
        if (f < FA) {
            const u32x4 x = *reinterpret_cast<const u32x4 *>(smem + st * STAGE + ((a_rd ^ (unsigned)(32 * s)) + f * FR * 64 + (NP == 2 ? part / 2 : part) * PART_A));
            if (part == 0) fa[par][f].h = x;
            else if (part == 1) fa[par][f].m = x;
            else fa[par][f].l = x;
        } else {
            const int b = f - FA;
            const u32x4 x = *reinterpret_cast<const u32x4 *>(smem + st * STAGE + ((w_rd ^ (unsigned)(32 * s)) + b * FR * 64 + (NP == 2 ? part / 2 : part) * PART_W));
            if (part == 0) fw[par][b].h = x;
            else if (part == 1) fw[par][b].m = x;
            else fw[par][b].l = x;
        }
    };
    auto read_part = [&](int st, bool isA, int part, int f) {
        read_frag(st, 0, 0, 3 * (isA ? f : FA + f) + part);
    };

    f32x16 acc[TM][TN];
#pragma unroll
    for (int a = 0; a < TM; ++a)
#pragma unroll
        for (int b = 0; b < TN; ++b)
#pragma unroll
            for (int r = 0; r < 16; ++r) acc[a][b][r] = 0.f;

    constexpr int NBB = MS == 32 ? 4 * TN : 2 * TN, NA = FA;
    auto coloff = [](int bb) { return MS == 32 ? 32 * (bb >> 2) + 8 * (bb & 3) : 16 * bb; };
    auto get4 = [&](int a, int bb) {
        const int A_ = MS == 32 ? a : a >> 1, b = MS == 32 ? bb >> 2 : bb >> 1, q = MS == 32 ? bb & 3 : 2 * (a & 1) + (bb & 1);
        return (f32x4){acc[A_][b][4 * q], acc[A_][b][4 * q + 1], acc[A_][b][4 * q + 2], acc[A_][b][4 * q + 3]};
    };
    auto set4 = [&](int a, int bb, const f32x4 x) {
        const int A_ = MS == 32 ? a : a >> 1, b = MS == 32 ? bb >> 2 : bb >> 1, q = MS == 32 ? bb & 3 : 2 * (a & 1) + (bb & 1);
        acc[A_][b][4 * q] = x[0]; acc[A_][b][4 * q + 1] = x[1]; acc[A_][b][4 * q + 2] = x[2]; acc[A_][b][4 * q + 3] = x[3];
    };
    const int ldc_eff = (!ATOMIC && p.sk_ws) ? BN : p.ldc;
    __amdgpu_buffer_rsrc_t rsC = __builtin_amdgcn_make_buffer_rsrc((void *)p.C, 0, 0, 0x00020000);
    unsigned st_off[NBB];
#pragma unroll
    for (int bb = 0; bb < NBB; ++bb) st_off[bb] = NT_OOB;
    unsigned stg_off[TN];
#pragma unroll
    for (int b = 0; b < TN; ++b) stg_off[b] = NT_OOB;
    unsigned char *const stg = smem + 2 * STAGE + wave * 4096;
    u32x4 pend[4];
    auto stage_block = [&](int a, int b) {
        int lane = __builtin_amdgcn_mbcnt_hi(~0u, __builtin_amdgcn_mbcnt_lo(~0u, 0u));
        asm volatile("" : "+v"(lane));
        const int li = MS == 32 ? lane & 31 : lane & 15, lg = MS == 32 ? lane >> 5 : lane >> 4;
        const unsigned stg_wr = (unsigned)(li * 128), stg_sw = (unsigned)(li & 7);
        const unsigned stg_rd = (unsigned)((lane >> 3) * 128 + (((lane & 7) ^ (lane >> 3)) * 16));
#pragma unroll
        for (int q = 0; q < 4; ++q) {
            if (MS == 32)
                *reinterpret_cast<u32x4 *>(stg + stg_wr + (((unsigned)(2 * q + lg) ^ stg_sw) * 16)) = __builtin_bit_cast(u32x4, get4(a, 4 * b + q));
            else
                *reinterpret_cast<u32x4 *>(stg + stg_wr + (q >> 1) * 2048 + (((unsigned)(4 * (q & 1) + lg) ^ stg_sw) * 16)) =
                    __builtin_bit_cast(u32x4, get4(2 * a + (q >> 1), 2 * b + (q & 1)));
        }
#pragma unroll
        for (int j = 0; j < 4; ++j) pend[j] = *reinterpret_cast<const u32x4 *>(stg + stg_rd + j * 1024);
    };
    auto flush_block = [&](int a, int b) {
#pragma unroll
        for (int j = 0; j < 4; ++j)
            if (!(X3_ABLATE & 4))
                __builtin_amdgcn_raw_buffer_store_b128(pend[j], rsC, stg_off[b] + (unsigned)((a * 32 + 8 * j) * ldc_eff) * 4u, 0, 0);
    };
    auto store_block = [&](int a, int b) {
        if (STG) {
            stage_block(a, b);
            flush_block(a, b);
            return;
        }
#pragma unroll
        for (int q = 0; q < 4; ++q) {
            const int ra = MS == 32 ? a : 2 * a + (q >> 1), bb = MS == 32 ? 4 * b + q : 2 * b + (q & 1);
            const unsigned off = st_off[bb] + (unsigned)(ra * FR * ldc_eff) * 4u;
            if (!(X3_ABLATE & 4)) __builtin_amdgcn_raw_buffer_store_b128(__builtin_bit_cast(u32x4, get4(ra, bb)), rsC, off, 0, 0);
        }
    };
    auto finish_item = [&]() {
        int lane = __builtin_amdgcn_mbcnt_hi(~0u, __builtin_amdgcn_mbcnt_lo(~0u, 0u));
        asm volatile("" : "+v"(lane));
        const int li = MS == 32 ? lane & 31 : lane & 15, lg = MS == 32 ? lane >> 5 : lane >> 4;
        const int mloc0 = wm * 32 * TM + li, nloc0 = wn * 32 * TN + 4 * lg;
        int tm, tn;
        decode(cp.tile, tm, tn);
        const long long m0 = (long long)tm * BM;
        const int n0 = tn * BN;
        const bool to_ws = !ATOMIC && p.sk_ws != nullptr;
        if (NP == 2) {
            if (!ATOMIC) {
                float ua[TM];
#pragma unroll
                for (int a = 0; a < TM; ++a) ua[a] = untab[mloc0 + 32 * a];
#pragma unroll
                for (int bb = 0; bb < NBB; ++bb) {
                    const f32x4 uw = *reinterpret_cast<const f32x4 *>(untab + BM + nloc0 + coloff(bb));
#pragma unroll
                    for (int a = 0; a < TM; ++a) set4(a, bb, (get4(a, bb) * ua[a]) * uw);
                }
            } else {
                const int mla = wm * 32 * TM + 4 * lg, nla = wn * 32 * TN + li;
#pragma unroll
                for (int b = 0; b < TN; ++b) {
                    const float uw = untab[BM + nla + 32 * b];
#pragma unroll
                    for (int a = 0; a < TM; ++a)
#pragma unroll
                        for (int q = 0; q < 4; ++q) {
                            const f32x4 ua4 = *reinterpret_cast<const f32x4 *>(untab + mla + 32 * a + 8 * q);
#pragma unroll
                            for (int r = 0; r < 4; ++r) acc[a][b][4 * q + r] = (acc[a][b][4 * q + r] * ua4[r]) * uw;
                        }
                }
            }
        }
        const long long mrows = to_ws ? BM : min((long long)BM, p.M - m0);
        const int ncols = to_ws ? BN : min(BN, p.N - n0);
        if (!ATOMIC) {
            if (to_ws) rsC = __builtin_amdgcn_make_buffer_rsrc((void *)(p.sk_ws + (size_t)(p.sk_seg ? v * p.sk_seg + (cp.j - 1) : v) * BM * BN), 0,
                                                               BM * BN * 4, 0x00020000);
            else rsC = __builtin_amdgcn_make_buffer_rsrc((void *)(p.C + m0 * p.ldc + n0), 0, (int)(mrows * p.ldc * 4), 0x00020000);
#pragma unroll
            for (int bb = 0; bb < NBB; ++bb)
                st_off[bb] = (nloc0 + coloff(bb) < ncols && !(p.dbg & 1)) ? (unsigned)(mloc0 * ldc_eff + nloc0 + coloff(bb)) * 4u : NT_OOB;
#pragma unroll
            for (int b = 0; b < TN; ++b) {
                const int nl = wn * 32 * TN + 32 * b + 4 * (lane & 7);
                stg_off[b] = (nl < ncols && !(p.dbg & 1)) ? (unsigned)((wm * 32 * TM + (lane >> 3)) * ldc_eff + nl) * 4u : NT_OOB;
            }
            if (p.addend) {
                __amdgpu_buffer_rsrc_t rsD = __builtin_amdgcn_make_buffer_rsrc((void *)(p.addend + m0 * p.ldadd + n0), 0,
                                                                               (int)(mrows * p.ldadd * 4), 0x00020000);
#pragma unroll
                for (int bb = 0; bb < NBB; ++bb)
#pragma unroll
                    for (int a = 0; a < NA; ++a) {
                        const int ml = mloc0 + FR * a, nl = nloc0 + coloff(bb);
                        set4(a, bb, get4(a, bb) + __builtin_bit_cast(f32x4, __builtin_amdgcn_raw_buffer_load_b128(
                                                      rsD, nl < ncols ? (unsigned)(ml * p.ldadd + nl) * 4u : NT_OOB, 0, 0)));
                    }
            }
            if (p.bias) {
                __amdgpu_buffer_rsrc_t rsB = __builtin_amdgcn_make_buffer_rsrc((void *)(p.bias + n0), 0, ncols * 4, 0x00020000);
#pragma unroll
                for (int bb = 0; bb < NBB; ++bb) {
                    const f32x4 bz = __builtin_bit_cast(f32x4, __builtin_amdgcn_raw_buffer_load_b128(rsB, (unsigned)(nloc0 + coloff(bb)) * 4u, 0, 0));
#pragma unroll
                    for (int a = 0; a < NA; ++a) set4(a, bb, get4(a, bb) + bz);
                }
            }
            if (EPI && p.row_bias) {
                __amdgpu_buffer_rsrc_t rsR = __builtin_amdgcn_make_buffer_rsrc((void *)p.row_bias, 0, p.rb_bytes, 0x00020000);
#pragma unroll
                for (int a = 0; a < NA; ++a) {
                    const unsigned row = (unsigned)(m0 + mloc0 + FR * a);
                    const unsigned grp = row < (unsigned)p.M ? (p.rows_per_group == 1 ? row : __umulhi(row, p.rpg_magic)) : 0u;
#pragma unroll
                    for (int bb = 0; bb < NBB; ++bb) {
                        const int nl = nloc0 + coloff(bb);
                        set4(a, bb, get4(a, bb) + __builtin_bit_cast(f32x4, __builtin_amdgcn_raw_buffer_load_b128(
                                                      rsR, nl < ncols ? (grp * (unsigned)p.ld_rb + n0 + nl) * 4u : NT_OOB, 0, 0)));
                    }
                }
            }
            if (EPI && p.act == 2) {
#pragma unroll
                for (int a = 0; a < TM; ++a)
#pragma unroll
                    for (int b = 0; b < TN; ++b)
#pragma unroll
                        for (int r = 0; r < 16; ++r) acc[a][b][r] = acc[a][b][r] > 0.f ? acc[a][b][r] : 0.01f * acc[a][b][r];
            }
            if (EPI && p.gate) {
                __amdgpu_buffer_rsrc_t rsG = __builtin_amdgcn_make_buffer_rsrc((void *)(p.gate + m0 * p.ldgate + n0), 0,
                                                                               (int)(mrows * p.ldgate * 4), 0x00020000);
#pragma unroll
                for (int bb = 0; bb < NBB; ++bb)
#pragma unroll
                    for (int a = 0; a < NA; ++a) {
                        const int ml = mloc0 + FR * a, nl = nloc0 + coloff(bb);
                        const f32x4 g = __builtin_bit_cast(f32x4, __builtin_amdgcn_raw_buffer_load_b128(
                                                                     rsG, nl < ncols ? (unsigned)(ml * p.ldgate + nl) * 4u : NT_OOB, 0, 0));
                        f32x4 x = get4(a, bb);
#pragma unroll
                        for (int r = 0; r < 4; ++r) x[r] *= g[r] > 0.f ? 1.f : 0.01f;
                        set4(a, bb, x);
                    }
            }
            if (p.stat_part) {
                float *P = p.stat_part + ((size_t)tm * WM + wm) * 3 * p.N;
#pragma unroll
                for (int bb = 0; bb < NBB; ++bb) {
                    float cs[4] = {0.f, 0.f, 0.f, 0.f}, cq[4] = {0.f, 0.f, 0.f, 0.f}, pv[4];
                    const f32x4 x0 = get4(0, bb);
#pragma unroll
                    for (int r = 0; r < 4; ++r) {
                        if (MS == 32) {
                            const float p0 = __int_as_float(__builtin_amdgcn_readlane(__float_as_int(x0[r]), 0));
                            const float p1 = __int_as_float(__builtin_amdgcn_readlane(__float_as_int(x0[r]), 32));
                            pv[r] = lg ? p1 : p0;
                        } else {
                            const float p0 = __int_as_float(__builtin_amdgcn_readlane(__float_as_int(x0[r]), 0));
                            const float p1 = __int_as_float(__builtin_amdgcn_readlane(__float_as_int(x0[r]), 16));
                            const float p2 = __int_as_float(__builtin_amdgcn_readlane(__float_as_int(x0[r]), 32));
                            const float p3 = __int_as_float(__builtin_amdgcn_readlane(__float_as_int(x0[r]), 48));
                            pv[r] = (lg & 2) ? ((lg & 1) ? p3 : p2) : ((lg & 1) ? p1 : p0);
                        }
                    }
#pragma unroll
                    for (int a = 0; a < NA; ++a)
                        if (mloc0 + FR * a < mrows) {
                            const f32x4 x = get4(a, bb);
#pragma unroll
                            for (int r = 0; r < 4; ++r) {
                                const float d = x[r] - pv[r];
                                cs[r] += d;
                                cq[r] = __fmaf_rn(d, d, cq[r]);
                            }
                        }
#pragma unroll
                    for (int r = 0; r < 4; ++r) {
                        cs[r] = MS == 32 ? x3_half_wave_sum(cs[r]) : x3_row_sum(cs[r]);
                        cq[r] = MS == 32 ? x3_half_wave_sum(cq[r]) : x3_row_sum(cq[r]);
                    }
                    const int nl = nloc0 + coloff(bb);
                    if (li == FR - 1 && nl < ncols) {
                        *reinterpret_cast<float4 *>(P + n0 + nl) = make_float4(cs[0], cs[1], cs[2], cs[3]);
                        *reinterpret_cast<float4 *>(P + p.N + n0 + nl) = make_float4(cq[0], cq[1], cq[2], cq[3]);
                        *reinterpret_cast<float4 *>(P + 2 * p.N + n0 + nl) = make_float4(pv[0], pv[1], pv[2], pv[3]);
                    }
                }
            }
        } else {
            const bool head = cp.kb == 0;
            const int mla = wm * 32 * TM + 4 * lg, nla = wn * 32 * TN + li;
#pragma unroll
            for (int b = 0; b < FW; ++b) {
                const int nl = nla + FR * b;
                const bool nok = nl < ncols;
                const float bz = (head && p.bias && nok) ? p.bias[n0 + nl] : 0.f;
#pragma unroll
                for (int a = 0; a < FA; ++a)
#pragma unroll
                    for (int j = 0; j < (MS == 32 ? 16 : 4); ++j) {
                        const int ml = mla + FR * a + (MS == 32 ? 8 * (j >> 2) + (j & 3) : j);
                        if (nok && ml < mrows) {
                            float o = (MS == 32 ? acc[a][b][j] : acc[a >> 1][b >> 1][4 * (2 * (a & 1) + (b & 1)) + j]) + bz;
                            if (head && p.addend) o += p.addend[(m0 + ml) * p.ldadd + n0 + nl];
                            atomicAdd(p.C + (m0 + ml) * p.ldc + n0 + nl, o);
                        }
                    }
            }
        }
    };

    constexpr int NPROD = NP == 3 ? 6 : X2_PRODUCTS;
    constexpr int SM = NPROD * TM * TN, NM = 2 * SM, NFR = NP * (TM + TN);
    constexpr int BAR = 2 * TM * TN > NFR + 2 ? 2 * TM * TN : NFR + 2;
    constexpr int CT_PER_Q = 4, NCT = NQ * CT_PER_Q;
    constexpr int C_LO = 1, C_HI = NM - BAR - 1;
    static_assert(MS == 16 || (BAR < SM && NFR + 2 <= SM), "k step too short for its fragment reads");
    auto conv_task = [&](int st, int k) {
        const int q = k / CT_PER_Q, sub = k % CT_PER_Q;
        if (X3_ABLATE & 1) return;
        if (sub < 2) conv_pair(q, sub);
        else if (sub == 2) conv_write(st, q);
        else {
            const bool tr = q < QA ? AT : WT;
            if (X3_ABLATE & 2) return;
            const int CU = q < QA ? CUA : CUW, j = q < QA ? q : q - QA;
            if (!tr) load_quad(q);
            else if (j % CU == CU - 1) load_quad(q - (CU - 1));
        }
    };
    auto chunk = [&](auto first_c, int st) {
        constexpr bool FIRST = decltype(first_c)::value;
#pragma unroll
        for (int s = 0; s < 2; ++s)
#pragma unroll
            for (int t = 0; t < NPROD; ++t)
#pragma unroll
                for (int a = 0; a < TM; ++a)
#pragma unroll
                    for (int b = 0; b < TN; ++b) {
                        const int is = (t * TM + a) * TN + b, idx = s * SM + is;
                        if (idx == NM - BAR) {
                            __builtin_amdgcn_sched_barrier(0);
                            asm volatile("s_waitcnt lgkmcnt(0)" ::: "memory");
                            if (!(X3_ABLATE & 8)) __builtin_amdgcn_s_barrier();
                            asm volatile("" ::: "memory");
                            __builtin_amdgcn_sched_barrier(0);
                        }
                        f32x16 c = acc[a][b];
                        if (FIRST && s == 0 && t == 0) {
                            if (STG) {
                                if (a + b > 0) flush_block(b ? a : a - 1, b ? b - 1 : TN - 1);
                                stage_block(a, b);
                            } else if (!ATOMIC) {
                                store_block(a, b);
                            }
#pragma unroll
                            for (int r = 0; r < 16; ++r) c[r] = 0.f;
                        }
                        if (FIRST && STG && s == 0 && t == 1 && a == 0 && b == 0) flush_block(TM - 1, TN - 1);
                        const X3Parts &A = fa[s][a], &W = fw[s][b];
                        if (NP == 2) {
                            const int u = t + 4 - NPROD;
                            const u32x4 ap = u <= 1 ? A.l : A.h, wp = (u == 0 || u == 2) ? W.l : W.h;
                            acc[a][b] = ATOMIC ? x2_mfma(ap, wp, c) : x2_mfma(wp, ap, c);
                        } else {
                        const u32x4 ap = t == 0 ? A.l : (t == 1 || t == 3) ? A.m : A.h;
                        const u32x4 wp = t == 2 ? W.l : (t == 1 || t == 4) ? W.m : W.h;
                        acc[a][b] = ATOMIC ? x3_mfma(ap, wp, c) : x3_mfma(wp, ap, c);
                        }
                        if (idx % X3_FENCE == 0) __builtin_amdgcn_sched_barrier(0);
                        if (!(X3_ABLATE & 16)) {
                            if (s == 0 && is >= 1 && is < 1 + NFR) read_frag(st, 1, 1, is - 1);
                            if (s == 1 && idx >= NM - BAR && idx < NM - BAR + NFR) read_frag(st ^ 1, 0, 0, idx - (NM - BAR));
                        }
                        if (idx >= C_LO && idx < C_HI) {
                            const int i0 = idx - C_LO, span = C_HI - C_LO;
                            const int k0 = (i0 * NCT) / span, k1 = ((i0 + 1) * NCT) / span;
#pragma unroll
                            for (int k = k0; k < k1; ++k) conv_task(st ^ 1, k);
                        }
                    }
    };

    constexpr int PM = FA * FW, NM16 = 6 * PM;
    constexpr int SP = PM >= 32 ? 4 : (PM >= 16 ? 2 : 1);
    constexpr int BAR16 = 2 * FA + 4 > NM16 / 5 ? 2 * FA + 4 : NM16 / 5;
    constexpr int C_HI16 = NM16 - BAR16 - 1;
    constexpr int L1 = 2 * FW + 2 * FA;
    static_assert(MS == 32 || (1 + SP * (FW - 1) + 6 <= PM && 1 + SP * (2 * FW - 1) + 6 <= 2 * PM && 1 + SP * (2 * FW + FA - 1) + 6 <= 3 * PM &&
                               1 + SP * (L1 - 1) + 6 <= 4 * PM && 1 + SP * (L1 - 1) < NM16 - BAR16),
                  "16x16x32: a part would not be back before its first use");
    static_assert(MS == 32 || (NM16 - BAR16 >= 3 * PM && NM16 - BAR16 + 1 + 2 * (FA - 1) < NM16 && 5 * PM + 2 * (FW - 1) < NM16),
                  "16x16x32: the next chunk's first parts do not fit behind the barrier");
    auto chunk16 = [&](auto first_c, int st) {
        constexpr bool FIRST = decltype(first_c)::value;
#pragma unroll
        for (int t = 0; t < 6; ++t)
#pragma unroll
        for (int sb = 0; sb < PM / 4; ++sb)
#pragma unroll
        for (int q = 0; q < 4; ++q) {
            const int idx = t * PM + 4 * sb + q;
            const int a32 = sb / TN, b32 = sb % TN, a16 = 2 * a32 + (q >> 1), b16 = 2 * b32 + (q & 1);
            if (idx == NM16 - BAR16) {
                __builtin_amdgcn_sched_barrier(0);
                asm volatile("s_waitcnt lgkmcnt(0)" ::: "memory");
                if (!(X3_ABLATE & 8)) __builtin_amdgcn_s_barrier();
                asm volatile("" ::: "memory");
                __builtin_amdgcn_sched_barrier(0);
            }
            f32x4a c = {acc[a32][b32][4 * q], acc[a32][b32][4 * q + 1], acc[a32][b32][4 * q + 2], acc[a32][b32][4 * q + 3]};
            if (FIRST && t == 0) {
                if (q == 0) {
                    if (STG) {
                        if (sb > 0) flush_block((sb - 1) / TN, (sb - 1) % TN);
                        stage_block(a32, b32);
                    } else if (!ATOMIC) {
                        store_block(a32, b32);
                    }
                }
                c = (f32x4a){0.f, 0.f, 0.f, 0.f};
            }
            if (FIRST && STG && idx == PM) flush_block(TM - 1, TN - 1);
            const X3Parts &A = fa[0][a16], &W = fw[0][b16];
            const u32x4 ap = t <= 2 ? A.h : (t == 4 ? A.l : A.m);
            const u32x4 wp = (t == 0 || t == 3 || t == 4) ? W.h : (t == 2 ? W.l : W.m);
            c = ATOMIC ? x3_mfma16(ap, wp, c) : x3_mfma16(wp, ap, c);
            acc[a32][b32][4 * q] = c[0]; acc[a32][b32][4 * q + 1] = c[1]; acc[a32][b32][4 * q + 2] = c[2]; acc[a32][b32][4 * q + 3] = c[3];
            if (idx % X3_FENCE16 == 0) __builtin_amdgcn_sched_barrier(0);
            if (!(X3_ABLATE & 16)) {
                if (idx >= 1 && idx < 1 + SP * L1 && (idx - 1) % SP == 0) {
                    const int j = (idx - 1) / SP;
                    if (j < FW) read_part(st, false, 1, j);
                    else if (j < 2 * FW) read_part(st, false, 2, j - FW);
                    else if (j < 2 * FW + FA) read_part(st, true, 1, j - 2 * FW);
                    else read_part(st, true, 2, j - 2 * FW - FA);
                }
                const int ja = idx - (NM16 - BAR16 + 1), jw = idx - 5 * PM;
                if (ja >= 0 && ja < 2 * FA && ja % 2 == 0) read_part(st ^ 1, true, 0, ja / 2);
                if (jw >= 0 && jw < 2 * FW && jw % 2 == 0) read_part(st ^ 1, false, 0, jw / 2);
            }
            if (idx >= C_LO && idx < C_HI16) {
                const int i0 = idx - C_LO, span = C_HI16 - C_LO;
                const int k0 = (i0 * NCT) / span, k1 = ((i0 + 1) * NCT) / span;
#pragma unroll
                for (int k = k0; k < k1; ++k) conv_task(st ^ 1, k);
            }
        }
    };

    constexpr int NUN = NP == 2 ? (BM + BN + NTH - 1) / NTH : 1;
    unsigned unb[NUN];
    auto fetch_unscales = [&]() {
        if (NP != 2) return;
        int tm, tn;
        decode(cp.tile, tm, tn);
        const long long m0 = (long long)tm * BM;
        const int n0 = tn * BN;
        const int mrows = (int)min((long long)BM, p.M - m0), ncols = min(BN, p.N - n0);
        const __amdgpu_buffer_rsrc_t rA = __builtin_amdgcn_make_buffer_rsrc((void *)(p.max_a + m0), 0, mrows * 4, 0x00020000);
        const __amdgpu_buffer_rsrc_t rW = __builtin_amdgcn_make_buffer_rsrc((void *)(p.max_w + n0), 0, ncols * 4, 0x00020000);
        int lane_ = __builtin_amdgcn_mbcnt_hi(~0u, __builtin_amdgcn_mbcnt_lo(~0u, 0u));
        asm volatile("" : "+v"(lane_));
#pragma unroll
        for (int i = 0; i < NUN; ++i) {
            const int e = wave * 64 + lane_ + i * NTH;
            unb[i] = (unsigned)__builtin_amdgcn_raw_buffer_load_b32(rA, e < BM ? (unsigned)e * 4u : NT_OOB, 0, 0) |
                     (unsigned)__builtin_amdgcn_raw_buffer_load_b32(rW, e >= BM ? (unsigned)(e - BM) * 4u : NT_OOB, 0, 0);
        }
    };
    auto store_unscales = [&]() {
        if (NP != 2) return;
        int lane_ = __builtin_amdgcn_mbcnt_hi(~0u, __builtin_amdgcn_mbcnt_lo(~0u, 0u));
        asm volatile("" : "+v"(lane_));
#pragma unroll
        for (int i = 0; i < NUN; ++i) {
            const int e = wave * 64 + lane_ + i * NTH;
            if (e < BM + BN) untab[e] = x2_unscale(unb[i]);
        }
    };

    issue_begin();
    fetch_maxima();
    adopt_scales();
#pragma unroll
    for (int q = 0; q < NQ; ++q) load_quad(q);
    advance_load();
#pragma unroll
    for (int q = 0; q < NQ; ++q) {
        conv_pair(q, 0);
        conv_pair(q, 1);
        conv_write(0, q);
    }
    if (NP == 2 && ld.valid && ld.kc == ld.kb) {
        fetch_maxima();
        adopt_scales();
    }
    issue_begin();
#pragma unroll
    for (int q = 0; q < NQ; ++q) load_quad(q);
    advance_load();
    asm volatile("s_waitcnt lgkmcnt(0)" ::: "memory");
    __builtin_amdgcn_s_barrier();
    asm volatile("" ::: "memory");
    if (MS == 32) {
#pragma unroll
        for (int r = 0; r < NFR; ++r) read_frag(0, 0, 0, r);
    } else {
#pragma unroll
        for (int f = 0; f < FA; ++f) read_part(0, true, 0, f);
#pragma unroll
        for (int f = 0; f < FW; ++f) read_part(0, false, 0, f);
    }
    int stage = 0;
    while (cp.valid) {
        const bool open0 = NP == 2 && ld.valid && ld.kc == ld.kb;
        if (open0) fetch_maxima();
        fetch_unscales();
        issue_begin();
        __builtin_amdgcn_sched_barrier(0);
        if constexpr (MS == 32) chunk(std::true_type(), stage);
        else chunk16(std::true_type(), stage);
        __builtin_amdgcn_sched_barrier(0);
        if (open0) adopt_scales();
        store_unscales();
        advance_load();
        stage ^= 1;
        cp.kc++;
        while (cp.kc != cp.ke) {
            const bool open1 = NP == 2 && ld.valid && ld.kc == ld.kb;
            if (open1) fetch_maxima();
            issue_begin();
            __builtin_amdgcn_sched_barrier(0);
            if constexpr (MS == 32) chunk(std::false_type(), stage);
            else chunk16(std::false_type(), stage);
            __builtin_amdgcn_sched_barrier(0);
            if (open1) adopt_scales();
            advance_load();
            stage ^= 1;
            cp.kc++;
        }
        __builtin_amdgcn_sched_barrier(0);
        if (NP == 2 && cp.ke - cp.kb == 1) {
            asm volatile("s_waitcnt lgkmcnt(0)" ::: "memory");
            __builtin_amdgcn_s_barrier();
            asm volatile("" ::: "memory");
        }
        finish_item();
        __builtin_amdgcn_sched_barrier(0);
        next_item(cp);
    }
    if (!ATOMIC) {
#pragma unroll
        for (int a = 0; a < TM; ++a)
#pragma unroll
            for (int b = 0; b < TN; ++b) store_block(a, b);
    }
}

#ifndef X3_KERNEL_ONLY
static bool x3_shape16(int cfg_index, bool atomic, bool epi, bool pw);

static thread_local float *x3_tail_ws = nullptr;
static thread_local long long x3_tail_ws_floats = 0;
static thread_local float *x3_cur_ws;
static thread_local long long x3_cur_ws_floats;
static float *x3_take_workspace(size_t floats) {
    static const bool off = [] { const char *e = getenv("PDGN_X3_SK_WS"); return e && e[0] == '0'; }();
    float *p = (!off && x3_cur_ws && (size_t)x3_cur_ws_floats >= floats) ? x3_cur_ws : nullptr;
    x3_cur_ws = nullptr;
    x3_cur_ws_floats = 0;
    return p;
}

__global__ __launch_bounds__(256) void x3_sk_reduce_kernel(const float *__restrict__ ws, int S, int T, int BM, int BN, int tile_begin,
                                                           int tiles_m, int tiles_n, long long M, int N, float *__restrict__ C, int ldc,
                                                           const float *__restrict__ bias, const float *__restrict__ addend, int ldadd,
                                                           int seg, long long per, int KC) {
    const int t = blockIdx.x, tile = tile_begin + t;
    const int per_group = NT_GROUP_M * tiles_n;
    const int grp = tile / per_group, r = tile - grp * per_group, first = grp * NT_GROUP_M;
    const int gsz = min(NT_GROUP_M, tiles_m - first);
    const int tn = r / gsz, tm = first + (r - tn * gsz);
    const long long m0 = (long long)tm * BM;
    const int n0 = tn * BN;
    const int mrows = (int)min((long long)BM, M - m0), ncols = min(BN, N - n0);
    const int q4 = BN / 4;
    const int rows_per = BM / (int)gridDim.y;
    const int ne = rows_per * q4;
    const int G = (!seg && ne < 256) ? 256 / ne : 1;
    __shared__ float4 red[256];
    for (int e0 = 0; e0 < ne; e0 += 256 / G) {
        const int e = e0 + (int)threadIdx.x % (256 / G), g = (int)threadIdx.x / (256 / G);
        const int row = blockIdx.y * rows_per + e / q4, c4 = (e % q4) * 4;
        const bool in = e < ne && row < mrows && c4 < ncols;
        float4 a = make_float4(0.f, 0.f, 0.f, 0.f);
        if (in && !seg) {
            bool have = false;
#pragma unroll 4
            for (int sl = g; sl < S; sl += G) {
                const float4 b = *reinterpret_cast<const float4 *>(ws + (((size_t)sl * T + t) * BM + row) * BN + c4);
                if (!have) { a = b; have = true; }
                else { a.x += b.x; a.y += b.y; a.z += b.z; a.w += b.w; }
            }
        } else if (in) {
            const long long f0 = (long long)t * KC, f1 = f0 + KC - 1;
            const long long v0 = f0 / per, v1 = f1 / per;
            for (long long vv = v0; vv <= v1; ++vv) {
                const size_t slot = (size_t)(vv * seg + (t - (vv * per) / KC));
                const float4 b = *reinterpret_cast<const float4 *>(ws + (slot * BM + row) * BN + c4);
                a.x += b.x; a.y += b.y; a.z += b.z; a.w += b.w;
            }
        }
        if (G > 1) {
            red[threadIdx.x] = a;
            __syncthreads();
            if (g == 0)
                for (int gg = 1; gg < G; ++gg) {
                    const float4 b = red[gg * (256 / G) + (int)threadIdx.x];
                    a.x += b.x; a.y += b.y; a.z += b.z; a.w += b.w;
                }
            __syncthreads();
        }
        if (!in || g != 0) continue;
        if (bias) { const float4 b = *reinterpret_cast<const float4 *>(bias + n0 + c4); a.x += b.x; a.y += b.y; a.z += b.z; a.w += b.w; }
        if (addend) {
            const float4 b = *reinterpret_cast<const float4 *>(addend + (m0 + row) * ldadd + n0 + c4);
            a.x += b.x; a.y += b.y; a.z += b.z; a.w += b.w;
        }
        *reinterpret_cast<float4 *>(C + (m0 + row) * ldc + n0 + c4) = a;
    }
}
template <int NU>
__global__ __launch_bounds__(1024) void x2_maxima_kernel(const float *__restrict__ X, long long rows, int cols, int ld, int slab_units,
                                                         long long rows_per_wg, unsigned *__restrict__ rowmax,
                                                         unsigned *__restrict__ colmax, int row_atomic, int upr) {
    extern __shared__ unsigned x2_cmax[];
    const int lane = threadIdx.x & 63, wave = threadIdx.x >> 6;
    const int u0 = blockIdx.y * slab_units, nu = min(slab_units, cols / 4 - u0);
    const long long r0 = (long long)blockIdx.x * rows_per_wg, r1 = min(rows, r0 + rows_per_wg);
    if (colmax) {
        for (int i = threadIdx.x; i < 4 * nu; i += 1024) x2_cmax[i] = 0u;
        __syncthreads();
    }
    const int G = 64 / upr, ul = lane & (upr - 1), gl = lane / upr;
    uint4 cm[NU];
#pragma unroll
    for (int i = 0; i < NU; ++i) cm[i] = make_uint4(0u, 0u, 0u, 0u);
    for (long long r = r0 + (long long)wave * G + gl; r < r1; r += 16 * G) {
        const uint4 *__restrict__ P = reinterpret_cast<const uint4 *>(X + r * ld) + u0;
        uint4 v[NU];
#pragma unroll
        for (int i = 0; i < NU; ++i) v[i] = ul + 64 * i < nu ? P[ul + 64 * i] : make_uint4(0u, 0u, 0u, 0u);
        unsigned rm = 0u;
#pragma unroll
        for (int i = 0; i < NU; ++i) {
            v[i].x &= 0x7fffffffu; v[i].y &= 0x7fffffffu; v[i].z &= 0x7fffffffu; v[i].w &= 0x7fffffffu;
            rm = max(rm, max(max(v[i].x, v[i].y), max(v[i].z, v[i].w)));
            cm[i].x = max(cm[i].x, v[i].x); cm[i].y = max(cm[i].y, v[i].y); cm[i].z = max(cm[i].z, v[i].z); cm[i].w = max(cm[i].w, v[i].w);
        }
        if (rowmax) {
            for (int o = upr >> 1; o >= 1; o >>= 1) rm = max(rm, (unsigned)__shfl_xor((int)rm, o));
            if (ul == 0) {
                if (row_atomic) atomicMax(rowmax + r, rm);
                else rowmax[r] = rm;
            }
        }
    }
    if (!colmax) return;
#pragma unroll
    for (int i = 0; i < NU; ++i)
        if (ul + 64 * i < nu) {
            unsigned *c = x2_cmax + 4 * (ul + 64 * i);
            atomicMax(c, cm[i].x); atomicMax(c + 1, cm[i].y); atomicMax(c + 2, cm[i].z); atomicMax(c + 3, cm[i].w);
        }
    __syncthreads();
    for (int i = threadIdx.x; i < 4 * nu; i += 1024) atomicMax(colmax + 4 * u0 + i, x2_cmax[i]);
}
static int x2_maxima_launch(const float *X, long long rows, int cols, int ld, unsigned *rowmax, unsigned *colmax, hipStream_t s) {
    if (rows < 1 || cols < 4 || cols % 4 || ld % 4 || ld < cols || ((uintptr_t)X & 15) || (!rowmax && !colmax)) return PDGN_ERR_INVALID;
    const int units = cols / 4;
    const int per = (units + 63) / 64;
    const int NU = per <= 1 ? 1 : per <= 2 ? 2 : per <= 4 ? 4 : 8;
    const int slab = 64 * NU, slabs = (units + slab - 1) / slab;
    const int cus = nt_cus();
    int upr = 64;
    if (NU == 1) { upr = 1; while (upr < units) upr *= 2; }
    long long wgs = (rows + 16 * (64 / upr) - 1) / (16 * (64 / upr));
    const long long cap = colmax ? (long long)cus / slabs + 1 : 8LL * cus;
    wgs = wgs < 1 ? 1 : (wgs > cap ? cap : wgs);
    const int rq = 16 * (64 / upr);
    const long long rpw = ((rows + wgs - 1) / wgs + rq - 1) / rq * rq;
    wgs = (rows + rpw - 1) / rpw;
    if (wgs > 0x7fffffffLL || slabs > 65535) return PDGN_ERR_INVALID;
    const int row_atomic = rowmax && slabs > 1;
    if (row_atomic && hipMemsetAsync(rowmax, 0, (size_t)rows * 4, s) != hipSuccess) return pdgn_launch_status();
    if (colmax && hipMemsetAsync(colmax, 0, (size_t)cols * 4, s) != hipSuccess) return pdgn_launch_status();
    const size_t lds = colmax ? (size_t)slab * 16 : 0;
#define X2_MAX_CALL(N_)                                                                                                         \
    hipLaunchKernelGGL((x2_maxima_kernel<N_>), dim3((unsigned)wgs, (unsigned)slabs), dim3(1024), lds, s, X, rows, cols, ld, slab, rpw, \
                       rowmax, colmax, row_atomic, upr)
    switch (NU) {
        case 1: X2_MAX_CALL(1); break;
        case 2: X2_MAX_CALL(2); break;
        case 4: X2_MAX_CALL(4); break;
// ... 17 lines not shown
        const unsigned long long at = next.fetch_add(need);
        const unsigned long long pos = at % slots;
        if (pos + need <= slots) return ring + (size_t)pos * 256;
    }
}
const unsigned *x2_scan(const float *X, long long rows, int cols, int ld, bool bycol, hipStream_t s) {
    unsigned *out = x2_arena_take(bycol ? cols : rows);
    if (!out) return nullptr;
    if (x2_maxima_launch(X, rows, cols, ld, bycol ? nullptr : out, bycol ? out : nullptr, s) != 0) return nullptr;
    return out;
}
static thread_local const unsigned *x2_next_max_a = nullptr, *x2_next_max_w = nullptr;

static thread_local const unsigned *x2_cur_max_a = nullptr, *x2_cur_max_w = nullptr;
struct X3Handover {
    X3Handover() {
        x3_cur_ws = x3_tail_ws; x3_cur_ws_floats = x3_tail_ws_floats;
        x2_cur_max_a = x2_next_max_a; x2_cur_max_w = x2_next_max_w;
        x3_tail_ws = nullptr; x3_tail_ws_floats = 0;
        x2_next_max_a = x2_next_max_w = nullptr;
    }
    ~X3Handover() {
        x3_cur_ws = nullptr; x3_cur_ws_floats = 0;
        x2_cur_max_a = x2_cur_max_w = nullptr;
    }
};

static int x3_reduce_split(int tiles) {
    int y = 8;
    while (tiles * y < 512 && y < 64) y *= 2;
    return y;
}

bool rp_takes(long long m, int n, int k);
int rp_launch(long long m, int n, int k, const float *A, int lda, const unsigned short *Wp, int ldw, long long wplane, float *C, int ldc,
              float *stat_part, hipStream_t s);
void x3_launch16(int cfg, int flags, int grid, hipStream_t s, const NtArgs &a);
void x3_launch_h2(int flags, int grid, hipStream_t s, const NtArgs &a, bool eight_waves);
const void *x3_symbol_h2(int flags, bool eight_waves);
static bool x2_pays(int cfg, long long m, int n, int k, long long scan_bytes) {
    if (nt_switches().mode != 2 || cfg != 0 || k < 128 || m >= (1LL << 28)) return false;
    const double flops = 2.0 * (double)m * n * k;
    static const double min_flops = [] { const char *e = getenv("PDGN_X2_MIN_GFLOP"); return (e && *e) ? atof(e) * 1e9 : 2e10; }();
    return flops >= min_flops && (double)scan_bytes <= 4.5e-3 * flops;
}

template <int TM, int TN, int WM, int WN, int OCC, int RATE, int CFG>
struct X3Cfg {
    static constexpr int BM = 32 * TM * WM, BN = 32 * TN * WN;
    static constexpr int LDS = 2 * 3 * (BM + BN) * 64;
    static constexpr int WG_PER_CU = OCC;

    struct Plan {
        int tiles_m, tiles_n, kchunks, grid_dp, dp_tiles, grid_sk;
        long long sk_per_wg;
        double cost;
    };
    static int dp_grid(long long tiles, int slots, int kc) {
        int tpw = (64 + kc - 1) / kc;
        tpw = tpw < 1 ? 1 : (tpw > 8 ? 8 : tpw);
        const long long g = (tiles + tpw - 1) / tpw;
        const long long lo = tiles < slots ? tiles : slots;
        return (int)(g < lo ? lo : g);
    }
    static double chunk_us(int w) { return 2.0 * BM * BN * NT_BK * w / (RATE * 1e3); }
    static Plan plan(long long m, int n, int k, bool allow_sk) {
        Plan pl;
        pl.tiles_m = cdiv(m, BM);
        pl.tiles_n = cdiv(n, BN);
        pl.kchunks = cdiv(k, NT_BK);
        const long long T = (long long)pl.tiles_m * pl.tiles_n;
        const int cus = nt_cus(), slots = cus * WG_PER_CU, KC = pl.kchunks;
        const long long rounds = T / slots, tail = T - rounds * slots;
        const double ov = 2.0;
        const double full = (double)rounds * (KC + ov) * chunk_us(WG_PER_CU);
        pl.dp_tiles = (int)T;
        pl.grid_dp = dp_grid(T, slots, KC);
        pl.grid_sk = 0;
        pl.sk_per_wg = 0;
        pl.cost = full + (tail ? (KC + ov) * chunk_us((int)((tail + cus - 1) / cus)) : 0.0);
        if (allow_sk && tail > 0) {
            const long long iters = tail * KC;
            const long long cand[3] = {(long long)slots, (long long)cus, iters / 16};
            for (int ci = 0; ci < 3; ++ci) {
                long long g = cand[ci] < 1 ? 1 : (cand[ci] > slots ? slots : cand[ci]);
                g = g < iters ? g : iters;
                const long long per = (iters + g - 1) / g;
                if (per < 8 && g > 1) continue;
                g = (iters + per - 1) / per;
                const double zero_rows = (double)(m - (long long)((rounds * slots) / (NT_GROUP_M * pl.tiles_n)) * NT_GROUP_M * BM);
                const double c = full + (per + ov) * chunk_us((int)((g + cus - 1) / cus)) + (double)(g + tail) * BM * BN * 4 / 1.3e6 +
                                 zero_rows * n * 4 / 3.0e6 + 4.0;
                if (c < pl.cost) {
                    pl.cost = c;
                    pl.dp_tiles = (int)(rounds * slots);
                    pl.grid_dp = rounds ? dp_grid(rounds * slots, slots, KC) : 0;
                    pl.grid_sk = (int)g;
                    pl.sk_per_wg = per;
                }
            }
        }
        return pl;
    }

    template <bool ATOMIC, bool WT, bool AT, bool EPI, bool PW = false>
    static void go(int grid, hipStream_t s, const NtArgs &a, bool two_part = false) {
        const int flags = (ATOMIC ? 1 : 0) | (WT ? 2 : 0) | (AT ? 4 : 0) | (EPI ? 8 : 0) | (PW ? 16 : 0);
        if (two_part) x3_launch_h2(flags, grid, s, a, a.stat_part == nullptr);
        else if (x3_shape16(CFG, ATOMIC, EPI, PW)) x3_launch16(CFG, flags, grid, s, a);
        else hipLaunchKernelGGL((gemm_x3_kernel<TM, TN, WM, WN, OCC, ATOMIC, WT, AT, EPI, PW, 32>), dim3(grid), dim3(64 * WM * WN), 0, s, a);
    }

    struct Tail {
        int t_tail, s_tail, per_tail, grid, seg;
        long long per_flat, floats;
    };
    static Tail tail_layout(const Plan &pl) {
        Tail t = {0, 0, 0, 0, 0, 0, 0};
        if (!pl.grid_sk) return t;
        const long long T = (long long)pl.tiles_m * pl.tiles_n;
        const int slots_ = nt_cus() * WG_PER_CU;
        t.t_tail = (int)(T - pl.dp_tiles);
        t.s_tail = slots_ / t.t_tail < 1 ? 1 : slots_ / t.t_tail;
        t.s_tail = t.s_tail > pl.kchunks ? pl.kchunks : t.s_tail;
        t.per_tail = (pl.kchunks + t.s_tail - 1) / t.s_tail;
        t.s_tail = (pl.kchunks + t.per_tail - 1) / t.per_tail;
        t.grid = t.s_tail * t.t_tail;
        const long long iters = (long long)t.t_tail * pl.kchunks;
        if (t.grid * 5 < slots_ * 4 && iters >= (long long)slots_ * 8) {
            t.per_flat = (iters + slots_ - 1) / slots_;
            t.grid = (int)((iters + t.per_flat - 1) / t.per_flat);
            t.seg = (int)((t.per_flat + pl.kchunks - 2) / pl.kchunks) + 1;
            t.floats = (long long)t.grid * t.seg * BM * BN;
        } else {
            t.floats = (long long)t.grid * BM * BN;
        }
        return t;
    }
    static long long tail_floats(long long m, int n, int k, bool allow_sk) { return tail_layout(plan(m, n, k, allow_sk)).floats; }
    static int at_slices(const Plan &pl) {
        const long long T = (long long)pl.tiles_m * pl.tiles_n;
        const int slots = nt_cus() * WG_PER_CU;
        const int S = (int)(slots / T) < pl.kchunks ? (int)(slots / T) : pl.kchunks;
        const int per = (pl.kchunks + S - 1) / S;
        return (pl.kchunks + per - 1) / per;
    }
    static long long at_floats(long long m, int n, int k) {
        const Plan pl = plan(m, n, k, true);
        const long long T = (long long)pl.tiles_m * pl.tiles_n;
        if (T > nt_cus() * WG_PER_CU || !nt_switches().splitk) return 0;
        return (long long)at_slices(pl) * T * BM * BN;
    }

    template <bool WT, bool AT = false>
    static int launch(long long m, int n, int k, const float *A, int lda, const float *W, int ldw, const float *bias,
                      const float *addend, int ldadd, float *C, int ldc, float *stat_part, hipStream_t s,
                      const NtEpi &epi = NtEpi(), bool prezeroed = false, const unsigned short *Wp = nullptr, long long wplane = 0,
                      int parts = 3) {
        const bool allow_sk = stat_part == nullptr && ldc == n && !epi.any();
        const Plan pl = plan(m, n, k, allow_sk);
        NtArgs a;
        a.M = m; a.N = n; a.K = k; a.lda = lda; a.ldw = ldw; a.ldc = ldc; a.ldadd = ldadd;
        a.A = A; a.W = W; a.bias = bias; a.addend = addend; a.C = C; a.stat_part = stat_part;
        a.row_bias = epi.row_bias; a.ld_rb = epi.ld_rb; a.rows_per_group = epi.rows_per_group > 0 ? epi.rows_per_group : 1;
        a.rpg_magic = a.rows_per_group > 1 ? (unsigned)(0x100000000ULL / (unsigned)a.rows_per_group) + 1u : 0u;
        a.rb_bytes = epi.row_bias ? (int)((((m + a.rows_per_group - 1) / a.rows_per_group - 1) * (long long)epi.ld_rb + n) * 4) : 0;
        a.act = epi.act; a.gate = epi.gate; a.ldgate = epi.ldgate; a.sk_split = 0;
        a.Wp = Wp; a.wplane = wplane;
        a.sk_ws = nullptr;
        a.sk_seg = 0;
        a.max_a = a.max_w = nullptr;
        const unsigned *hand_a = x2_cur_max_a, *hand_w = x2_cur_max_w;
        x2_cur_max_a = x2_cur_max_w = nullptr;
        const bool two = Wp ? parts == 2
                            : x2_pays(CFG, m, n, k, (hand_a ? 0 : (long long)m * k * 4) + (hand_w ? 0 : (long long)n * k * 4));
        if (two && CFG != 0) return PDGN_ERR_INVALID;
        if (two) {
            a.max_a = hand_a ? hand_a : x2_scan(A, AT ? (long long)k : m, AT ? (int)m : k, lda, AT, s);
            if (Wp) a.max_w = reinterpret_cast<const unsigned *>(Wp + 2 * wplane);
            else a.max_w = hand_w ? hand_w : x2_scan(W, WT ? k : n, WT ? n : k, ldw, WT, s);
            if (!a.max_a || !a.max_w) return PDGN_ERR_INVALID;
        }
        a.tiles_m = pl.tiles_m; a.tiles_n = pl.tiles_n; a.kchunks = pl.kchunks;
        a.dbg = 0;
#ifdef PDGN_NT_DEBUG
        { const char *e = getenv("PDGN_NT_DBG"); a.dbg = e ? atoi(e) : 0; }
#endif
        const long long T = (long long)pl.tiles_m * pl.tiles_n;
        if (AT && T <= nt_cus() * WG_PER_CU && nt_switches().splitk) {
            const int slots = nt_cus() * WG_PER_CU;
            const int S = (int)(slots / T) < pl.kchunks ? (int)(slots / T) : pl.kchunks;
            a.tile_begin = 0; a.tile_end = (int)T; a.sk_split = (int)T; a.sk_per_wg = (pl.kchunks + S - 1) / S;
            const int s_ws = at_slices(pl);
            float *ws = x3_take_workspace((size_t)s_ws * T * BM * BN);
            if (ws) {
                a.sk_ws = ws;
                go<false, WT, AT, false>((int)T * s_ws, s, a, two);
                hipLaunchKernelGGL(x3_sk_reduce_kernel, dim3((int)T, x3_reduce_split((int)T)), dim3(256), 0, s, ws, s_ws, (int)T, BM, BN, 0, pl.tiles_m, pl.tiles_n, m, n,
                                   C, ldc, nullptr, nullptr, 0, 0, 0LL, pl.kchunks);
                return pdgn_launch_status();
            }
            if (!prezeroed && hipMemsetAsync(C, 0, (size_t)m * ldc * sizeof(float), s) != hipSuccess) return pdgn_launch_status();
            go<true, WT, AT, false>((int)T * S, s, a, two);
            return pdgn_launch_status();
        }
        const Tail tl = tail_layout(pl);
        float *ws = (tl.t_tail > 0 && !AT) ? x3_take_workspace((size_t)tl.floats) : nullptr;
        if (pl.grid_sk && !ws) {
            const long long r0 = (long long)(pl.dp_tiles / (NT_GROUP_M * pl.tiles_n)) * NT_GROUP_M * BM;
            if (!prezeroed && hipMemsetAsync(C + r0 * ldc, 0, (size_t)(m - r0) * ldc * sizeof(float), s) != hipSuccess) return pdgn_launch_status();
        }
        constexpr bool CAN_PW = !WT && !AT;
        if (pl.grid_dp) {
            a.tile_begin = 0; a.tile_end = pl.dp_tiles; a.sk_per_wg = 0;
            if (CAN_PW && Wp) {
                if (epi.any()) go<false, false, false, true, CAN_PW>(pl.grid_dp, s, a, two);
                else go<false, false, false, false, CAN_PW>(pl.grid_dp, s, a, two);
            } else if (!AT && epi.any()) go<false, WT, false, true>(pl.grid_dp, s, a, two);
            else go<false, WT, AT, false>(pl.grid_dp, s, a, two);
        }
        if (pl.grid_sk && ws) {
            a.tile_begin = pl.dp_tiles; a.tile_end = (int)T; a.sk_ws = ws;
            a.sk_split = tl.seg ? 0 : tl.t_tail; a.sk_seg = tl.seg; a.sk_per_wg = tl.seg ? tl.per_flat : tl.per_tail;
            a.bias = nullptr; a.addend = nullptr;
            if (CAN_PW && Wp) go<false, false, false, false, CAN_PW>(tl.grid, s, a, two);
            else go<false, WT, AT, false>(tl.grid, s, a, two);
            hipLaunchKernelGGL(x3_sk_reduce_kernel, dim3(tl.t_tail, x3_reduce_split(tl.t_tail)), dim3(256), 0, s, ws, tl.s_tail, tl.t_tail, BM, BN, pl.dp_tiles, pl.tiles_m,
                               pl.tiles_n, m, n, C, ldc, bias, addend, ldadd, tl.seg, tl.per_flat, pl.kchunks);
        } else if (pl.grid_sk) {
            a.tile_begin = pl.dp_tiles; a.tile_end = (int)T; a.sk_per_wg = pl.sk_per_wg;
            if (CAN_PW && Wp) go<true, false, false, false, CAN_PW>(pl.grid_sk, s, a, two);
            else go<true, WT, AT, false>(pl.grid_sk, s, a, two);
        }
        return pdgn_launch_status();
    }
};

typedef X3Cfg<2, 2, 2, 2, 1, 660, 1> X3Square;
typedef X3Cfg<4, 2, 2, 2, 1, 760, 0> X3Big;
typedef X3Cfg<2, 1, 2, 2, 2, 540, 2> X3Narrow;

NtSwitches &nt_switches() {
    static NtSwitches sw = [] {
        NtSwitches s;
        const char *e = getenv("PDGN_GEMM");
        s.mode = (e && e[0] == 'f') ? 0 : (e && e[0] == 'x' && e[1] == '3') ? 1 : 2;
        e = getenv("PDGN_NT_CFG");
        s.cfg = (e && *e) ? atoi(e) : -1;
        e = getenv("PDGN_X3_SPLITK");
        s.splitk = !(e && e[0] == '0');
        s.shape16 = X3_DEFAULT_MASK;
        e = getenv("PDGN_X3_SHAPE");
        if (e && *e) s.shape16 = atoi(e) == 16 ? 0xfff : 0;
        e = getenv("PDGN_X3_SHAPE16_MASK");
        if (e && *e) s.shape16 = (int)strtol(e, nullptr, 16) & 0xfff;
        s.shape16_default = s.shape16;
        return s;
    }();
    return sw;
}

extern "C" int pdgn_gemm_set_mode(int mode) {
    const int old = nt_switches().mode;
    if (mode >= 0) nt_switches().mode = mode > 2 ? 1 : mode;
    return old;
}

extern "C" int pdgn_gemm_set_scale_slots(void *slots, long long bytes) {
    if (bytes < 0 || ((uintptr_t)slots & 15)) return PDGN_ERR_INVALID;
    const long long n = bytes / 1024;
    x2_ring_slots.store(0);
    x2_ring.store((unsigned *)slots);
    x2_ring_slots.store(slots ? (unsigned)(n > 0x7fffffff ? 0x7fffffff : n) : 0u);
    return 0;
}

extern "C" int pdgn_absmax_rows_cols(long long rows, int cols, const float *src, int ld, unsigned *rowmax, unsigned *colmax,
                                     pdgn_stream_t stream) {
    if (!src) return PDGN_ERR_INVALID;
    return x2_maxima_launch(src, rows, cols, ld, rowmax, colmax, (hipStream_t)stream);
}
extern "C" int pdgn_gemm_set_operand_scales(const unsigned *max_a, const unsigned *max_w) {
    x2_next_max_a = max_a;
    x2_next_max_w = max_w;
    return 0;
}

extern "C" int pdgn_gemm_set_config(int cfg) {
    const int old = nt_switches().cfg;
    if (cfg >= -1) nt_switches().cfg = cfg > 3 ? 3 : cfg;
    return old;
}

extern "C" int pdgn_gemm_set_shape(int shape) {
    const int old = nt_switches().shape16;
    if (shape == 16) nt_switches().shape16 = 0xfff;
    else if (shape == 32) nt_switches().shape16 = 0;
    else if (shape == -1) nt_switches().shape16 = nt_switches().shape16_default;
    else if (shape >= 0x1000 && shape <= 0x1fff) nt_switches().shape16 = shape & 0xfff;
    return old;
}

static int x3_mode() { return nt_switches().mode; }
static bool x3_shape16(int cfg_index, bool atomic, bool epi, bool pw) {
    const int cls = epi ? 3 : atomic ? 2 : pw ? 1 : 0;
    return (nt_switches().shape16 >> (4 * cfg_index + cls)) & 1;
}

static int x3_pick(long long m, int n, int k, bool stats) {
    const int forced = nt_switches().cfg;
    if (forced >= 0) return forced > 2 ? 2 : forced;
    const bool sk = !stats;
    const double c[3] = {X3Big::plan(m, n, k, sk).cost, X3Square::plan(m, n, k, sk).cost, X3Narrow::plan(m, n, k, sk).cost};
    int best = 0;
    for (int i = 1; i < 3; ++i)
        if (c[i] < c[best]) best = i;
    return best;
}

extern "C" int pdgn_gemm_two_part_planes(long long m, int n, int k, long long scan_bytes) {
    if (nt_switches().mode != 2 || m < 256 || n < 4 || k < 32) return 0;
    const double flops = 2.0 * (double)m * n * k;
    return (flops >= 2e9 && (double)scan_bytes <= 4.5e-3 * flops) ? 1 : 0;
}
extern "C" long long pdgn_gemm_nt_ps_workspace_floats(long long m, int n, int k, int parts, int with_stats);

extern "C" int pdgn_gemm_two_part(long long m, int n, int k, long long scan_bytes) {
    if (!x3_mode() || m < 1 || n < 4 || k < 4) return 0;
    return x2_pays(x3_pick(m, n, k, false), m, n, k, scan_bytes) ? 1 : 0;
}
static bool x3_args_ok(long long m, int n, int k, int lda, int ldw, int ldadd, int ldc, const float *addend, bool wt) {
    return m >= 1 && n >= 4 && k >= 4 && n % 4 == 0 && k % 4 == 0 && lda % 4 == 0 && ldw % 4 == 0 && ldc % 4 == 0 &&
           lda >= k && ldw >= (wt ? n : k) && ldc >= n && (!addend || (ldadd % 4 == 0 && ldadd >= n)) && lda < (1 << 19) &&
           ldw < (1 << 19) && ldc < (1 << 19) && (long long)cdiv(m, 128) * cdiv(n, 64) < 0x7fffffffLL &&
           (!wt || (long long)k * ldw < (1LL << 27));
}

template <bool WT>
static int x3_dispatch(long long m, int n, int k, const float *A, int lda, const float *W, int ldw, const float *bias,
                       const float *addend, int ldadd, float *C, int ldc, float *stat_part, hipStream_t s,
                       const NtEpi &epi = NtEpi(), const unsigned short *Wp = nullptr, long long wplane = 0, int parts = 3) {
    int cfg = x3_pick(m, n, k, stat_part != nullptr || epi.any());
    if (Wp && parts == 2) {
        if (stat_part && cfg != 0) return PDGN_ERR_INVALID;
        cfg = 0;
    }
    switch (cfg) {
        case 0: return X3Big::launch<WT>(m, n, k, A, lda, W, ldw, bias, addend, ldadd, C, ldc, stat_part, s, epi, false, Wp, wplane, parts);
        case 2: return X3Narrow::launch<WT>(m, n, k, A, lda, W, ldw, bias, addend, ldadd, C, ldc, stat_part, s, epi, false, Wp, wplane, parts);
        default: return X3Square::launch<WT>(m, n, k, A, lda, W, ldw, bias, addend, ldadd, C, ldc, stat_part, s, epi, false, Wp, wplane, parts);
    }
}

extern "C" int pdgn_gemm_nt(long long m, int n, int k, const float *A, int lda, const float *W, int ldw,
                            const float *bias, const float *addend, int ldadd, float *C, int ldc, float *stat_part,
                            pdgn_stream_t stream) {
    const X3Handover handover;
    if (!x3_mode()) return fp32_gemm_nt(m, n, k, A, lda, W, ldw, bias, addend, ldadd, C, ldc, stat_part, stream);
    if (!x3_args_ok(m, n, k, lda, ldw, ldadd, ldc, addend, false)) return PDGN_ERR_INVALID;
    return x3_dispatch<false>(m, n, k, A, lda, W, ldw, bias, addend, ldadd, C, ldc, stat_part, (hipStream_t)stream);
}

extern "C" int pdgn_gemm_nn(long long m, int n, int k, const float *A, int lda, const float *Wt, int ldw,
                            const float *bias, const float *addend, int ldadd, float *C, int ldc, float *stat_part,
                            pdgn_stream_t stream) {
    const X3Handover handover;
    if (!x3_mode()) return fp32_gemm_nn(m, n, k, A, lda, Wt, ldw, bias, addend, ldadd, C, ldc, stat_part, stream);
    if (!x3_args_ok(m, n, k, lda, ldw, ldadd, ldc, addend, true)) return PDGN_ERR_INVALID;
    return x3_dispatch<true>(m, n, k, A, lda, Wt, ldw, bias, addend, ldadd, C, ldc, stat_part, (hipStream_t)stream);
}

extern "C" int pdgn_gemm_nt_ex(long long m, int n, int k, const float *A, int lda, const float *W, int ldw, const float *bias,
                               const float *addend, int ldadd, float *C, int ldc, float *stat_part, const float *row_bias,
                               int ld_rb, int rows_per_group, int act, const float *gate, int ldgate, int transposed_w,
                               pdgn_stream_t stream) {
    const X3Handover handover;
    if (!x3_mode())
        return fp32_gemm_nt_ex(m, n, k, A, lda, W, ldw, bias, addend, ldadd, C, ldc, stat_part, row_bias, ld_rb, rows_per_group,
                               act, gate, ldgate, transposed_w, stream);
    if (!x3_args_ok(m, n, k, lda, ldw, ldadd, ldc, addend, transposed_w != 0)) return PDGN_ERR_INVALID;
    if ((act != 0 && act != 2) || (row_bias && (ld_rb < n || ld_rb % 4 || rows_per_group < 1)) ||
        (gate && (ldgate < n || ldgate % 4)) || m >= (1LL << 31) || (row_bias && m * rows_per_group >= (1LL << 32)) ||
        (row_bias && rows_per_group >= 1 && ((m + rows_per_group - 1) / rows_per_group) * (long long)ld_rb * 4 >= (long long)NT_OOB))
        return PDGN_ERR_INVALID;
    NtEpi e;
    e.row_bias = row_bias; e.ld_rb = ld_rb; e.rows_per_group = rows_per_group; e.act = act; e.gate = gate; e.ldgate = ldgate;
    return transposed_w ? x3_dispatch<true>(m, n, k, A, lda, W, ldw, bias, addend, ldadd, C, ldc, stat_part, (hipStream_t)stream, e)
                        : x3_dispatch<false>(m, n, k, A, lda, W, ldw, bias, addend, ldadd, C, ldc, stat_part, (hipStream_t)stream, e);
}

extern "C" int pdgn_gemm_nt_ps(long long m, int n, int k, const float *A, int lda, const unsigned short *Wplanes, int ldw,
                               long long wplane, int parts, const float *bias, const float *addend, int ldadd, float *C, int ldc,
                               float *stat_part, const float *row_bias, int ld_rb, int rows_per_group, int act, const float *gate,
                               int ldgate, pdgn_stream_t stream) {
    const X3Handover handover;
    if (!x3_mode() || !Wplanes || (parts != 3 && parts != 2)) return PDGN_ERR_INVALID;
    if (!x3_args_ok(m, n, k, lda, ldw, ldadd, ldc, addend, false)) return PDGN_ERR_INVALID;
    if (wplane < (long long)(n - 1) * ldw + k || wplane >= (1LL << 28) || ldw % 8 || wplane % 8 || ((uintptr_t)Wplanes & 15))
        return PDGN_ERR_INVALID;
    if ((act != 0 && act != 2) || (row_bias && (ld_rb < n || ld_rb % 4 || rows_per_group < 1)) ||
        (gate && (ldgate < n || ldgate % 4)) || m >= (1LL << 31) || (row_bias && m * rows_per_group >= (1LL << 32)) ||
        (row_bias && rows_per_group >= 1 && ((m + rows_per_group - 1) / rows_per_group) * (long long)ld_rb * 4 >= (long long)NT_OOB))
        return PDGN_ERR_INVALID;
    if (parts == 2 && x3_mode() == 2 && !bias && !addend && !row_bias && !act && !gate && rp_takes(m, n, k)) {
        return rp_launch(m, n, k, A, lda, Wplanes, ldw, wplane, C, ldc, stat_part, (hipStream_t)stream);
    }
    NtEpi e;
    e.row_bias = row_bias; e.ld_rb = ld_rb; e.rows_per_group = rows_per_group > 0 ? rows_per_group : 1; e.act = act; e.gate = gate;
    e.ldgate = ldgate;
    return x3_dispatch<false>(m, n, k, A, lda, nullptr, ldw, bias, addend, ldadd, C, ldc, stat_part, (hipStream_t)stream, e, Wplanes,
                              wplane, parts);
}

extern "C" long long pdgn_gemm_tail_workspace_floats(long long m, int n, int k, int with_stats) {
    if (!x3_mode() || m < 1 || n < 4 || k < 4) return 0;
    const bool sk = !with_stats;
    switch (x3_pick(m, n, k, with_stats != 0)) {
        case 0: return X3Big::tail_floats(m, n, k, sk);
        case 2: return X3Narrow::tail_floats(m, n, k, sk);
        default: return X3Square::tail_floats(m, n, k, sk);
    }
}
extern "C" long long pdgn_gemm_nt_ps_workspace_floats(long long m, int n, int k, int parts, int with_stats) {
    if (!x3_mode() || m < 1 || n < 4 || k < 4) return 0;
    if (parts == 2 && rp_takes(m, n, k)) return 0;
    if (parts == 2) return with_stats ? 0 : X3Big::tail_floats(m, n, k, true);
    return pdgn_gemm_tail_workspace_floats(m, n, k, with_stats);
}
extern "C" int pdgn_gemm_set_tail_workspace(float *ws, long long floats) {
    if (floats < 0 || ((uintptr_t)ws & 15)) return PDGN_ERR_INVALID;
    x3_tail_ws = ws;
    x3_tail_ws_floats = ws ? floats : 0;
    return 0;
}

extern "C" int pdgn_gemm_nt_ps_launch_info(long long m, int n, int k, int parts, const void **sym, int *grid) {
    if (!x3_mode() || m < 1 || n < 4 || k < 4 || !sym || !grid) return PDGN_ERR_INVALID;
    const int cfg = x3_pick(m, n, k, false);
    const bool s16 = x3_shape16(cfg, false, false, true);
    *sym = nullptr;
    if (parts == 2) {
        *grid = X3Big::plan(m, n, k, true).grid_dp;
        *sym = x3_symbol_h2(16, true);
    } else if (cfg == 0) {
        *grid = X3Big::plan(m, n, k, true).grid_dp;
        if (!s16) *sym = (const void *)gemm_x3_kernel<4, 2, 2, 2, 1, false, false, false, false, true, 32>;
    } else if (cfg == 2) {
        *grid = X3Narrow::plan(m, n, k, true).grid_dp;
        if (!s16) *sym = (const void *)gemm_x3_kernel<2, 1, 2, 2, 2, false, false, false, false, true, 32>;
    } else {
        *grid = X3Square::plan(m, n, k, true).grid_dp;
        if (!s16) *sym = (const void *)gemm_x3_kernel<2, 2, 2, 2, 1, false, false, false, false, true, 32>;
    }
    return 0;
}

extern "C" int pdgn_gemm_aux_symbols(const void **reduce, const void **scan) {
    if (reduce) *reduce = (const void *)x3_sk_reduce_kernel;
    if (scan) *scan = (const void *)x2_maxima_kernel<8>;
    return 0;
}

extern "C" int pdgn_gemm_tn_big(long long m, int n, int k, const float *dY, int ldy, const float *X, int ldx, float *dW,
                                int dw_is_zero, pdgn_stream_t stream) {
    const X3Handover handover;
    if (!x3_mode()) return fp32_gemm_tn_big(m, n, k, dY, ldy, X, ldx, dW, stream);
    if (m < 1 || n < 4 || k < 4 || n % 4 || k % 4 || ldy % 4 || ldx % 4 || ldy < n || ldx < k || ldy >= (1 << 19) ||
        ldx >= (1 << 19) || m > 0x7fffffffLL * 16)
        return PDGN_ERR_INVALID;
    hipStream_t s = (hipStream_t)stream;
    const int cfg = x3_pick(n, k, (int)(m > 0x7fffffff ? 0x7fffffff : m), false);
    switch (cfg) {
        case 0: return X3Big::launch<true, true>(n, k, (int)m, dY, ldy, X, ldx, nullptr, nullptr, 0, dW, k, nullptr, s, NtEpi(), dw_is_zero != 0);
        case 2: return X3Narrow::launch<true, true>(n, k, (int)m, dY, ldy, X, ldx, nullptr, nullptr, 0, dW, k, nullptr, s, NtEpi(), dw_is_zero != 0);
        default: return X3Square::launch<true, true>(n, k, (int)m, dY, ldy, X, ldx, nullptr, nullptr, 0, dW, k, nullptr, s, NtEpi(), dw_is_zero != 0);
    }
}

extern "C" long long pdgn_gemm_tn_big_workspace_floats(long long m, int n, int k) {
    if (!x3_mode() || m < 1 || n < 4 || k < 4) return 0;
    const int red = (int)(m > 0x7fffffff ? 0x7fffffff : m);
    switch (x3_pick(n, k, red, false)) {
        case 0: return X3Big::at_floats(n, k, red);
        case 2: return X3Narrow::at_floats(n, k, red);
        default: return X3Square::at_floats(n, k, red);
    }
}

extern "C" int pdgn_gemm_nt_ps_row_panel(long long m, int n, int k, int parts, int plain) {
    return (x3_mode() == 2 && parts == 2 && plain && m >= 1 && rp_takes(m, n, k)) ? 1 : 0;
}
extern "C" long long pdgn_gemm_nt_ps_stat_rows(long long m, int n, int k, int parts, int plain) {
    if (x3_mode() == 2 && parts == 2 && plain && m >= 1 && rp_takes(m, n, k)) return (m + 255) / 256;
    return pdgn_gemm_nt_stat_rows(m, n, k);
}
extern "C" int pdgn_gemm_nt_ps_stat_block_rows(long long m, int n, int k, int parts, int plain) {
    if (x3_mode() == 2 && parts == 2 && plain && m >= 1 && rp_takes(m, n, k)) return 256;
    return pdgn_gemm_nt_stat_block_rows(m, n, k);
}

extern "C" long long pdgn_gemm_nt_stat_rows(long long m, int n, int k) {
    if (!x3_mode()) return fp32_gemm_nt_stat_rows(m, n, k);
    if (m < 1 || n < 1 || k < 1) return PDGN_ERR_INVALID;
    switch (x3_pick(m, n, k, true)) {
        case 0: return (long long)cdiv(m, X3Big::BM) * 2;
        case 2: return (long long)cdiv(m, X3Narrow::BM) * 2;
        default: return (long long)cdiv(m, X3Square::BM) * 2;
    }
}

extern "C" int pdgn_gemm_nt_stat_block_rows(long long m, int n, int k) {
    if (!x3_mode()) return fp32_gemm_nt_stat_block_rows(m, n, k);
    if (m < 1 || n < 1 || k < 1) return PDGN_ERR_INVALID;
    switch (x3_pick(m, n, k, true)) {
        case 0: return X3Big::BM / 2;
// ... 16 lines not shown
```

### pdgn_amd/csrc/gemm_x3_h2.hip

```cpp
#define X3_KERNEL_ONLY
#include "gemm_x3.hip"

#define X2_INSTANCES(X)                                                                                                          \
    X(true, false, false, false, false) X(false, false, false, true, true) X(false, false, false, false, true)                    \
    X(true, false, false, false, true) X(false, false, false, true, false) X(false, false, false, false, false)                   \
    X(true, true, false, false, false) X(false, true, false, true, false) X(false, true, false, false, false)                     \
    X(true, true, true, false, false) X(false, true, true, false, false)

template <int TM, int TN, int WM, int WN>
static const void *x2_symbol_tile(int flags) {
#define X2_CASE(A_, WT_, AT_, EPI_, PW_)                                                                                          \
    case ((A_ ? 1 : 0) | (WT_ ? 2 : 0) | (AT_ ? 4 : 0) | (EPI_ ? 8 : 0) | (PW_ ? 16 : 0)):                                         \
        return (const void *)gemm_x3_kernel<TM, TN, WM, WN, 1, A_, WT_, AT_, EPI_, PW_, 32, 2>;
    switch (flags) {
        X2_INSTANCES(X2_CASE)
        default: return nullptr;
    }
#undef X2_CASE
}

const void *x3_symbol_h2(int flags, bool eight_waves) {
    return eight_waves ? x2_symbol_tile<2, 2, 4, 2>(flags) : x2_symbol_tile<4, 2, 2, 2>(flags);
}

void x3_launch_h2(int flags, int grid, hipStream_t s, const NtArgs &a, bool eight_waves) {
    const void *f = x3_symbol_h2(flags, eight_waves);
    if (!f) abort();
    NtArgs args = a;
    void *params[] = {&args};
    (void)hipLaunchKernel(f, dim3(grid), dim3(eight_waves ? 512 : 256), params, 0, s);
}
```

### pdgn_amd/deconv.py

```python
import ctypes

import torch
import torch.nn as nn
import torch.nn.functional as F
from ._fn import Function

from . import _lib
from . import streams as _streams
from ._lib import check, ptr, require, stream_of
from .fused import (Planes, split_planes, skinny_linear, _zeros, bilateral_weighting, bn_act,
                    small_sequential, bn_act_maxpool, bn_softmax_slots_permute, flush_bn_counters,
                    has_zero_colsum, linear_cl, softmax_slots_permute, DenseInput, group_colsum, mark_maxima, row_maxima_buffer)
from .fused import _STATS_MAX as STATS_MAX

F32, I32 = torch.float32, torch.int32
_KNN_OVERLAP = __import__("os").environ.get("PDGN_KNN_OVERLAP", "1") == "1"
_KNN_CONST = __import__("os").environ.get("PDGN_KNN_CONST", "0") == "1"

def _knn_stream(device):
    return _streams.plan(device).knn


def _w2d(conv):
    w = conv.weight
    return w.view(w.shape[0], w.shape[1])


KNN_LOG = None


def feature_knn(x, k):
    require(x, "x", F32, 3)
    b, f, n = x.shape
    if KNN_LOG is not None:
        KNN_LOG.append((b, f, n))
    idx = torch.empty((b, n, k), dtype=I32, device=x.device)
    sq = torch.empty((b, n), dtype=F32, device=x.device)
    check(_lib.lib().pdgn_feature_knn(b, f, n, int(k), ptr(x), ptr(sq), ptr(idx), stream_of(x)),
          "pdgn_feature_knn")
    return idx


def start_feature_knn(xt, const, k, x_cf=None):
    want_csr = torch.is_grad_enabled() and xt.requires_grad

    def channel_major():
        if x_cf is not None:
            return x_cf.detach().contiguous()
        x = xt.detach().transpose(1, 2)
        if const is not None and _KNN_CONST:
            x = torch.cat((const.detach().unsqueeze(2).expand(-1, -1, xt.shape[1]), x), 1)
        return x.contiguous()

    with torch.no_grad():
        if not (xt.is_cuda and _KNN_OVERLAP):
            return feature_knn(channel_major(), k), None
        cur = torch.cuda.current_stream(xt.device)
        side = _knn_stream(xt.device)
        side.wait_stream(cur)
        for t in (xt, const, x_cf):
            if t is not None:
                t.record_stream(side)
        with torch.cuda.stream(side):
            x_knn = channel_major()
            idx = feature_knn(x_knn, k)
            ready = torch.cuda.Event()
            ready.record(side)
            if want_csr:
                transposed_graph(idx)
                idx._pdgn_csr_ready = torch.cuda.Event()
                idx._pdgn_csr_ready.record(side)
    return idx, ready


class EdgeGatherSum(Function):

    @staticmethod
    def forward(ctx, Y, idx, specs, *biases):
        require(Y, "Y", F32, 3)
        require(idx, "idx", I32, 3)
        b, n, ldy = Y.shape
        k = idx.shape[2]
        outs, partials = [], []
        L = _lib.lib()
        for spec, bias in zip(specs, biases):
            T, P, C, off, offc = spec[:5]
            out = torch.empty((b, n, P, C), dtype=F32, device=Y.device)
            if bias is not None and bias.dim() == 2 and bias.stride(1) == 1:
                bias_c, bstride = bias.detach(), bias.stride(0)
            else:
                bias_c = bias.detach().contiguous() if bias is not None else None
                bstride = C if (bias is not None and bias.dim() == 2) else 0
            if len(spec) > 5 and spec[5]:
                scr = torch.empty(L.pdgn_bn_scratch_floats(b * n * P, C), dtype=F32, device=Y.device)
                check(L.pdgn_window_gather_sum_stats(b, n, k, ldy, T, P, C, off, offc, ptr(Y), ptr(idx), ptr(bias_c),
                                                     bstride, ptr(out), ptr(scr), stream_of(Y)),
                      "pdgn_window_gather_sum_stats")
                partials.append(scr)
            else:
                check(L.pdgn_window_gather_sum(b, n, k, ldy, T, P, C, off, offc, ptr(Y), ptr(idx),
                                               ptr(bias_c), bstride, ptr(out), stream_of(Y)),
                      "pdgn_window_gather_sum")
            outs.append(out)
        specs = tuple(tuple(spec[:5]) for spec in specs)
        ctx.mark_non_differentiable(*partials)
        ctx.set_materialize_grads(False)
        ctx.specs, ctx.shape = specs, (b, n, ldy, k)
        ctx.has_bias = [0 if bias is None else bias.dim() for bias in biases]
        ctx.save_for_backward(idx)
        return tuple(outs) + tuple(partials)

    @staticmethod
    def backward(ctx, *douts):
        (idx,) = ctx.saved_tensors
        b, n, ldy, k = ctx.shape
        douts = [d if d is not None else torch.zeros((b, n, P, C), dtype=F32, device=idx.device)
                 for d, (T, P, C, off, offc) in zip(douts, ctx.specs)]
        L = _lib.lib()
        covered = sum(T * C + (C if offc >= 0 else 0) for (T, P, C, off, offc) in ctx.specs)
        vec_ok = ldy % 4 == 0 and k <= 31 and all(C % 4 == 0 and off % 4 == 0 and (offc < 0 or offc % 4 == 0)
                                                 for (T, P, C, off, offc) in ctx.specs)
        dbias = []
        if vec_ok and covered == ldy:
            rowptr, edges = transposed_graph(idx)
            dY = torch.empty((b, n, ldy), dtype=F32, device=idx.device)
            dmax = row_maxima_buffer(b * n, idx.device) if (_lib.gemm_mode() == "x2" and b * n * ldy >= (1 << 24)) else None
            first = 1
            for (T, P, C, off, offc), dout, hb in zip(ctx.specs, douts, ctx.has_bias):
                hb = 3 if hb == 1 and has_zero_colsum(dout) else hb
                dout = dout.contiguous()
                check(L.pdgn_window_gather_sum_backward_csr(b, n, k, ldy, T, P, C, off, offc, ptr(dout), ptr(rowptr),
                                                            ptr(edges), ptr(dY), ptr(dmax), first, stream_of(dout)),
                      "pdgn_window_gather_sum_backward_csr")
                first = 0
                if hb == 2 and offc >= 0:
                    dbias.append(group_colsum(dY.view(b * n, ldy)[:, offc:offc + C], n))
                else:
                    dbias.append(_dbias(dout, hb))
            if dmax is not None:
                mark_maxima(dY, dmax)
            return (dY, None, None) + tuple(dbias)
        dY = torch.zeros((b, n, ldy), dtype=F32, device=idx.device)
        for (T, P, C, off, offc), dout, hb in zip(ctx.specs, douts, ctx.has_bias):
            hb = 3 if hb == 1 and has_zero_colsum(dout) else hb
            dout = dout.contiguous()
            check(L.pdgn_window_gather_sum_backward(b, n, k, ldy, T, P, C, off, offc, ptr(dout), ptr(idx), ptr(dY),
                                                    stream_of(dout)), "pdgn_window_gather_sum_backward")
            dbias.append(_dbias(dout, hb))
        return (dY, None, None) + tuple(dbias)


def _dbias(dout, kind):
    if kind == 0:
        return None
    if kind == 3:
        return _zeros((dout.shape[-1],), dout.device)
    C = dout.shape[-1]
    if dout.is_contiguous():
        return group_colsum(dout.view(-1, C))[0] if kind == 1 else group_colsum(dout.view(-1, C), dout.shape[1] * dout.shape[2])
    return dout.sum(dim=(0, 1, 2)) if kind == 1 else dout.sum(dim=(1, 2))


def transposed_graph(idx):
    cached = getattr(idx, "_pdgn_csr", None)
    if cached is not None:
        ev = getattr(idx, "_pdgn_csr_ready", None)
# ... 272 lines not shown
```

### pdgn_amd/fused.py

```python
import os
import weakref

import torch
from ._fn import Function

from . import _lib
from ._lib import check, ptr, require, stream_of

F32 = torch.float32
ACT = {"none": 0, "relu": 1, "leaky_relu": 2}


def _scratch_floats(L, rows, C):
    n = L.pdgn_bn_scratch_floats(rows, C)
    if n < 0:
        raise _lib.PdgnHipError("pdgn_bn_scratch_floats: argument outside the supported range")
    return n


_ZERO_COLSUM = {}


def mark_zero_colsum(dx):
    _ZERO_COLSUM[dx.data_ptr()] = weakref.ref(dx)


def has_zero_colsum(dy):
    ref = _ZERO_COLSUM.pop(dy.data_ptr(), None)
    src = ref() if ref is not None else None
    return src is not None and (src is dy or dy._base is src) and dy.numel() == src.numel() \
        and dy.shape[-1] == src.shape[-1]


def clear_zero_colsum():
    _ZERO_COLSUM.clear()
    _INPUT_GRADS.clear()
    _GRAD_MAXIMA.clear()


_GRAD_MAXIMA = {}


def mark_maxima(g, slot):
    _GRAD_MAXIMA[g.data_ptr()] = (weakref.ref(g), slot)


def take_maxima(dy):
    ent = _GRAD_MAXIMA.pop(dy.data_ptr(), None)
    if ent is None:
        return None
    src = ent[0]()
    same = src is not None and (src is dy or (dy.numel() == src.numel() and dy.is_contiguous() and src.is_contiguous()
                                              and (dy._base is src or (dy._base is not None and dy._base is src._base))))
    return ent[1] if same else None


_INPUT_GRADS = {}
_CLOSED_TAIL = os.environ.get("PDGN_CLOSED_TAIL", "1") == "1"
_STATS_MAX = os.environ.get("PDGN_STATS_MAX", "1") == "1"
_CLOSED_DW = os.environ.get("PDGN_CLOSED_DW", "1") == "1"


class DenseInput:

    def __init__(self, h, w):
        self.h, self.w = h, w


_NAN_SLOTS = {}


def _placeholder_with_input_grad(rows, C, dh, dw, device):
    pool = _NAN_SLOTS.get(device)
    if pool is None:
        pool = _NAN_SLOTS[device] = [torch.full((256,), float("nan"), dtype=F32, device=device), 0]
    i = pool[1]
    pool[1] = (i + 1) % 256
    tok = pool[0][i:i + 1].expand(rows, C)
    _INPUT_GRADS[tok.data_ptr()] = (weakref.ref(tok), (dh, dw))
    return tok


def is_placeholder(dy):
    return dy.dim() == 2 and dy.stride(0) == 0 and dy.stride(1) == 0 and dy.numel() > 1


def take_input_grad(dy):
    hit = _INPUT_GRADS.pop(dy.data_ptr(), None) if dy.stride(0) == 0 else None
    if hit is None:
        return None
    src = hit[0]()
    return hit[1] if src is not None and (src is dy or dy._base is src or dy._base is src._base) and dy.shape == src.shape else None


_ARENA = {"buf": None, "off": 0, "need": 0, "owner": None}


def reset_zero_arena(device, owner):
    a = _ARENA
    if a["owner"] is not None:
        a["owner"].zero_arena_floats = max(getattr(a["owner"], "zero_arena_floats", 0), a["need"])
    size = getattr(owner, "zero_arena_floats", 0)
    a["buf"] = torch.zeros(size, dtype=F32, device=device) if size else None
    a["off"] = a["need"] = 0
    a["owner"] = owner


def release_zero_arena():
    a = _ARENA
    if a["owner"] is not None:
        a["owner"].zero_arena_floats = max(getattr(a["owner"], "zero_arena_floats", 0), a["need"])
    a["buf"] = None
    a["owner"] = None
    a["off"] = a["need"] = 0


def _zeros(shape, device):
    n = 1
    for d in shape:
        n *= d
    step = (n + 63) // 64 * 64
    a = _ARENA
    a["need"] += step
    buf = a["buf"]
    if buf is None or buf.device != device or a["off"] + step > buf.numel():
        return torch.zeros(shape, dtype=F32, device=device)
    v = buf[a["off"]:a["off"] + n].view(shape)
    a["off"] += step
    return v


_GROUP_COLSUM = os.environ.get("PDGN_GROUP_COLSUM", "1") == "1"


def group_colsum(x2d, group_rows=None):
    rows, C = x2d.shape
    gr = rows if group_rows is None else int(group_rows)
    if not (_GROUP_COLSUM and x2d.is_cuda and x2d.dtype == F32 and x2d.stride(1) == 1 and x2d.stride(0) % 4 == 0
            and x2d.data_ptr() % 16 == 0 and 16 <= C <= 1024 and (C & (C - 1)) == 0 and gr > 0 and rows % gr == 0
            and rows // gr <= 65535):
        return x2d.sum(dim=0, keepdim=True) if gr == rows else x2d.reshape(rows // gr, gr, C).sum(dim=1)
    out = _zeros((rows // gr, C), x2d.device)
    check(_lib.lib().pdgn_group_colsum(rows // gr, gr, C, ptr(x2d), x2d.stride(0), ptr(out), stream_of(x2d)), "pdgn_group_colsum")
    return out


def _bn_stats(L, x, rows, C, g, b, pre_bias, running_mean, running_var, training, momentum, eps, partials=None):
    stats = torch.empty(4 * C, dtype=F32, device=x.device)
    pb = pre_bias.detach().contiguous() if pre_bias is not None else None
    block = None
    if isinstance(partials, tuple):
        partials, block = partials
    if training and block is not None:
        nparts = partials.shape[0]
        nd = L.pdgn_bn_blocks_scratch_doubles(C, nparts)
        scr = torch.empty(nd, dtype=torch.float64, device=x.device) if nd > 0 else None
        check(L.pdgn_bn_stats_from_gemm_partials(rows, C, nparts, block, eps, momentum, ptr(g), ptr(b), ptr(pb),
                                                 ptr(running_mean), ptr(running_var), ptr(partials), ptr(stats), ptr(scr), stream_of(x)),
              "pdgn_bn_stats_from_gemm_partials")
    elif training and partials is not None:
        check(L.pdgn_bn_stats_from_partials(rows, C, eps, momentum, ptr(g), ptr(b), ptr(pb), ptr(running_mean), ptr(running_var), ptr(partials),
                                            ptr(stats), stream_of(x)), "pdgn_bn_stats_from_partials")
    elif training:
        scratch = torch.empty(_scratch_floats(L, rows, C), dtype=F32, device=x.device)
        check(L.pdgn_bn_stats(rows, C, eps, momentum, ptr(x), ptr(g), ptr(b), ptr(pb), ptr(running_mean), ptr(running_var), ptr(scratch), ptr(stats),
                              stream_of(x)), "pdgn_bn_stats")
    else:
        check(L.pdgn_bn_eval_stats(C, eps, ptr(g), ptr(b), ptr(pb), ptr(running_mean),
                                   ptr(running_var), ptr(stats), stream_of(x)), "pdgn_bn_eval_stats")
    return stats


_NO_FOLD = os.environ.get("PDGN_FOLD_BIAS", "1") == "0"


def _fold_pre_bias(x2d, pre_bias, training):
    if pre_bias is not None and (_NO_FOLD or (not training and torch.is_grad_enabled() and pre_bias.requires_grad)):
        return x2d + pre_bias, None
    return x2d, pre_bias


def _pre_bias_grad(ctx_has, C, device):
    return _zeros((C,), device) if ctx_has else None


class BNActCL(Function):

    @staticmethod
    def forward(ctx, x, gamma, beta, running_mean, running_var, training, momentum, eps, act, mul, pre_bias=None,
                partials=None, interleave_n=0):
        rows, C = x.shape
        x = x.contiguous()
        L = _lib.lib()
        g, b = gamma.detach().contiguous(), beta.detach().contiguous()
        stats = _bn_stats(L, x, rows, C, g, b, pre_bias, running_mean, running_var, training, momentum, eps, partials)
        ctx.has_pre_bias = pre_bias is not None
        mul_c = mul.contiguous() if mul is not None else None
        y = torch.empty((rows * 2, C // 2), dtype=F32, device=x.device) if interleave_n else torch.empty_like(x)
        check(L.pdgn_bn_act_forward(rows, C, act, ptr(x), ptr(stats), ptr(mul_c), ptr(y), int(interleave_n), stream_of(x)), "pdgn_bn_act_forward")
        ctx.save_for_backward(x, stats, mul_c)
        ctx.cfg = (rows, C, act, bool(training), mul is not None and mul.requires_grad, int(interleave_n))
        return y

    @staticmethod
    def backward(ctx, dy):
        x, stats, mul = ctx.saved_tensors
        rows, C, act, training, need_dmul, inter = ctx.cfg
        dy = dy.contiguous()
        L = _lib.lib()
        scratch = torch.empty(_scratch_floats(L, rows, C), dtype=F32, device=x.device)
        bs = torch.empty(2 * C, dtype=F32, device=x.device)
        dx = torch.empty_like(x)
        dmul = torch.empty_like(x) if need_dmul else None
# ... 787 lines not shown
            return (skinny_nn_masked(dy, y, act, weight) if act else dy.matmul(weight)), None, None, None
        dev = dy.device
        dpre = torch.empty((R, N), dtype=F32, device=dev)
        dW = torch.empty((N, K), dtype=F32, device=dev) if ctx.needs_input_grad[1] else None
        dbias = torch.empty(N, dtype=F32, device=dev) if has_bias and ctx.needs_input_grad[2] else None
        check(_lib.lib().pdgn_small_mlp_backward(R, K, N, act, 0, ptr(x), ptr(dy), ptr(y), None, None, None, ptr(dpre), None, None,
                                                 ptr(dbias), ptr(dW), stream_of(dy)), "pdgn_small_mlp_backward")
        dx = skinny_nn(dpre, weight) if ctx.needs_input_grad[0] else None
        return dx, dW, dbias, None


_SKINNY_HEAD = os.environ.get("PDGN_SKINNY_HEAD", "1") == "1"


def small_sequential(seq, x, training):
    mods = list(seq)
    fusable = x.is_cuda and x.dim() == 2 and x.shape[0] <= 64 and all(
        isinstance(m, (torch.nn.Linear, torch.nn.BatchNorm1d, torch.nn.LeakyReLU, torch.nn.ReLU)) for m in mods)
    if fusable:
        fusable = all(m.in_features <= 1024 and x.shape[0] * (m.in_features + 4) * 4 + 1024 <= 160 * 1024
                      for m in mods if isinstance(m, torch.nn.Linear))
    if not fusable:
        return seq(x)
    i = 0
    while i < len(mods):
        lin = mods[i]
        if not isinstance(lin, torch.nn.Linear):
            return seq(x)
        i += 1
        bn = None
        if i < len(mods) and isinstance(mods[i], torch.nn.BatchNorm1d):
            bn = mods[i]
            i += 1
        act = 0
        if i < len(mods) and isinstance(mods[i], torch.nn.LeakyReLU):
            if mods[i].negative_slope != 0.01:
                return seq(x)
            act = 2
            i += 1
        elif i < len(mods) and isinstance(mods[i], torch.nn.ReLU):
            act = 1
            i += 1
        if bn is not None:
            use_batch = training or not bn.track_running_stats
            if training and bn.track_running_stats:
                _PENDING_COUNTS[bn.num_batches_tracked] = _PENDING_COUNTS.get(bn.num_batches_tracked, 0) + 1
            x = SmallLinearBNAct.apply(x, lin.weight, lin.bias, bn.weight, bn.bias,
                                       bn.running_mean if bn.track_running_stats else None,
                                       bn.running_var if bn.track_running_stats else None, 1 if use_batch else 2,
                                       bn.momentum if bn.momentum is not None else 0.1, bn.eps, act)
        elif _SKINNY_HEAD and _sk_ok(x, lin.weight) and lin.in_features % 4 == 0:
            x = SkinnyLinearAct.apply(x, lin.weight, lin.bias, act)
        else:
            x = SmallLinearBNAct.apply(x, lin.weight, lin.bias, None, None, None, None, 0, 0.0, 0.0, act)
    return x


class BNActMaxPool(Function):

    @staticmethod
    def forward(ctx, x, gamma, beta, running_mean, running_var, training, momentum, eps, act, B, N, pre_bias=None,
                partials=None, dense=None):
        x = x.contiguous()
        rows, C = x.shape
        dev = x.device
        L = _lib.lib()
        g, b = gamma.detach().contiguous(), beta.detach().contiguous()
        ctx.has_pre_bias = pre_bias is not None
        ymax = torch.empty((B, C), dtype=F32, device=dev)
        yarg = torch.empty((B, C), dtype=torch.int32, device=dev)
        if training and partials is None and _STATS_MAX:
            stats = torch.empty(4 * C, dtype=F32, device=dev)
            pb = pre_bias.detach().contiguous() if pre_bias is not None else None
            scr = torch.empty(L.pdgn_bn_stats_maxpool_scratch_floats(B, C), dtype=F32, device=dev)
            check(L.pdgn_bn_stats_act_maxpool(B, N, C, act, eps, momentum, ptr(x), ptr(g), ptr(b), ptr(pb),
                                              ptr(running_mean), ptr(running_var), ptr(scr), ptr(stats), ptr(ymax), ptr(yarg),
                                              stream_of(x)), "pdgn_bn_stats_act_maxpool")
        else:
            stats = _bn_stats(L, x, rows, C, g, b, pre_bias, running_mean, running_var, training, momentum, eps, partials)
            scr = torch.empty(L.pdgn_bn_maxpool_scratch_floats(B, C), dtype=F32, device=dev)
            check(L.pdgn_bn_act_maxpool(B, N, C, act, ptr(x), ptr(stats), ptr(scr), ptr(ymax), ptr(yarg), stream_of(x)),
                  "pdgn_bn_act_maxpool")
        ctx.save_for_backward(x, stats, yarg)
        ctx.cfg = (B, N, C, act, bool(training))
        ctx.dense = dense if (dense is not None and _CLOSED_TAIL and training
                              and not (pre_bias is not None and pre_bias.requires_grad and not _CLOSED_DW)
                              and _dense_input_ok(dense, x, rows, C, N)) else None
        return ymax

    @staticmethod
    def backward(ctx, dout):
        x, stats, yarg = ctx.saved_tensors
        B, N, C, act, training = ctx.cfg
        dout = dout.contiguous()
        if ctx.dense is not None:
            h, w = ctx.dense.h, ctx.dense.w
            K = w.shape[1]
            L = _lib.lib()
            want_w, want_bn = w.requires_grad, any(ctx.needs_input_grad[1:3])
            scr = torch.empty(L.pdgn_dense_bn_maxpool_backward_scratch(B, C, K), dtype=F32, device=x.device)
            dh = torch.empty((B * N, K), dtype=F32, device=x.device) if h.requires_grad else None
            dw = torch.empty((C, K), dtype=F32, device=x.device) if want_w else None
            bs = torch.empty(2 * C, dtype=F32, device=x.device) if want_bn else None
            check(L.pdgn_dense_bn_maxpool_backward(B, N, C, K, act, ptr(x), ptr(dout), ptr(yarg), ptr(stats), ptr(h), h.stride(0),
                                                   ptr(w), w.stride(0), ptr(scr), ptr(dh), ptr(dw), K, ptr(bs), stream_of(x)),
                  "pdgn_dense_bn_maxpool_backward")
            tok = _placeholder_with_input_grad(B * N, C, dh, dw, x.device)
            return (tok, bs[C:] if want_bn else None, bs[:C] if want_bn else None, None, None, None, None, None, None, None, None,
                    _pre_bias_grad(ctx.has_pre_bias, C, x.device), None, None)
        scr = torch.empty(B * C + 2 * C, dtype=F32, device=x.device)
        bs = torch.empty(2 * C, dtype=F32, device=x.device)
        dx = torch.empty_like(x)
        check(_lib.lib().pdgn_bn_act_maxpool_backward(B, N, C, act, int(training), ptr(x), ptr(dout), ptr(yarg),
                                                      ptr(stats), ptr(scr), ptr(bs), ptr(dx), stream_of(x)),
              "pdgn_bn_act_maxpool_backward")
        if training:
            mark_zero_colsum(dx)
        return (dx, bs[C:], bs[:C], None, None, None, None, None, None, None, None,
                _pre_bias_grad(ctx.has_pre_bias, C, x.device), None, None)


def _is_plain_linear_output(y2d, dense):
    fn = y2d.grad_fn
    if fn is None:
        return not y2d.requires_grad
    return (type(fn).__name__ == "LinearCLBackward" and not getattr(fn, "has_bias", True) and not getattr(fn, "has_addend", True)
            and len(fn.saved_tensors) == 2 and fn.saved_tensors[1].data_ptr() == dense.w.data_ptr()
            and fn.saved_tensors[0].data_ptr() == dense.h.data_ptr())


def _dense_input_ok(dense, x, rows, C, N):
    h, w = dense.h, dense.w
    return (x.is_cuda and h.dim() == 2 and w.dim() == 2 and h.shape[0] == rows and w.shape[0] == C and h.shape[1] == w.shape[1]
            and w.shape[1] % 4 == 0 and w.shape[1] <= 256 and w.stride(0) % 4 == 0 and w.data_ptr() % 16 == 0 and h.dtype == F32 and w.dtype == F32 and h.stride(1) == 1 and w.stride(1) == 1
            and (h.requires_grad or w.requires_grad) and rows >= _OWN_MIN_ROWS
            and (not w.requires_grad or (_CLOSED_DW and w.shape[1] >= 16 and (w.shape[1] & (w.shape[1] - 1)) == 0
                                         and h.stride(0) % 4 == 0 and h.data_ptr() % 16 == 0))
            and N <= 65535 and 2 * (N + min(N, C) + C) + 1040 + 4 * C <= 65536)


def bn_act_maxpool(x2d, bn, training, B, N, act="leaky_relu", pre_bias=None, partials=None, dense=None):
    y2d = x2d
    x2d, pre_bias = _fold_pre_bias(x2d, pre_bias, training)
    if dense is not None and not (x2d is y2d and _is_plain_linear_output(y2d, dense)):
        dense = None
    if x2d.shape[1] % 4:
        return bn_act(x2d, bn, training, act=act, pre_bias=pre_bias).view(B, N, -1).max(dim=1)[0]
    if training and bn.track_running_stats:
        _PENDING_COUNTS[bn.num_batches_tracked] = _PENDING_COUNTS.get(bn.num_batches_tracked, 0) + 1
    return BNActMaxPool.apply(x2d, bn.weight, bn.bias, bn.running_mean, bn.running_var, training, bn.momentum, bn.eps,
                              ACT[act], B, N, pre_bias, partials, dense)


class PointMax(Function):

    @staticmethod
    def forward(ctx, x):
        x = x.contiguous()
        require(x, "x", F32, 3)
        b, n, c = x.shape
        L = _lib.lib()
        ns = int(L.pdgn_point_max_scratch(b, n, c))
        sval = torch.empty(ns, dtype=F32, device=x.device)
        sarg = torch.empty(ns, dtype=torch.int32, device=x.device)
        out = torch.empty((b, c), dtype=F32, device=x.device)
        arg = torch.empty((b, c), dtype=torch.int32, device=x.device)
        check(L.pdgn_point_max(b, n, c, ptr(x), ptr(sval), ptr(sarg), ptr(out), ptr(arg), stream_of(x)), "pdgn_point_max")
        ctx.save_for_backward(arg)
        ctx.n = n
        return out

    @staticmethod
    def backward(ctx, g):
        arg, = ctx.saved_tensors
        b, c = arg.shape
        g = g.contiguous()
        if c % 4:
            dx = torch.zeros((b, ctx.n, c), dtype=F32, device=g.device)
            return dx.scatter_(1, arg.long().unsqueeze(1), g.unsqueeze(1))
        dx = torch.empty((b, ctx.n, c), dtype=F32, device=g.device)
        check(_lib.lib().pdgn_point_max_backward(b, ctx.n, c, ptr(g), ptr(arg), ptr(dx), stream_of(g)),
              "pdgn_point_max_backward")
        return dx


def point_max(x):
    return PointMax.apply(x) if x.is_cuda else x.max(dim=1)[0]
```

### pdgn_amd/generator.py

```python
import torch
import torch.nn as nn
import torch.nn.functional as F

from . import deconv as _deconv
from .deconv import PointDeconv


def _bn_act(x2d, bn, training, act="leaky_relu", pre_bias=None):
    return _deconv.bn_act(x2d, bn, training, act=act, pre_bias=pre_bias)


def _small_seq(seq, x, training):
    return _deconv.small_sequential(seq, x, training)


def _point_max(x):
    from .fused import point_max
    return point_max(x)


def _linear(rows, weight, bias=None):
    return _deconv.linear_cl(rows, weight, bias)


# ... 28 lines not shown
        super().__init__()
        self.level = level
        if level == 1:
            self.upsample_cov = nn.Sequential(PointDeconv(Fin, Fout, num_k // 2, bilateral=False),
                                              nn.BatchNorm1d(Fout), nn.LeakyReLU(inplace=True))
        else:
            self.upsample_cov = PointDeconv(Fin, Fout, num_k // 2, bilateral=True, softmax=softmax)
            self.bn_uc = nn.BatchNorm1d(Fout)
        self.fc = nn.Sequential(nn.Linear(Fin, Fin), nn.BatchNorm1d(Fin), nn.LeakyReLU(inplace=True),
                                nn.Linear(Fin, Fout), nn.BatchNorm1d(Fout), nn.LeakyReLU(inplace=True))
        if level < 4:
            self.g_fc = nn.Sequential(nn.Linear(Fout, 512), nn.BatchNorm1d(512), nn.LeakyReLU(inplace=True))

    def forward_cl(self, xt, pct=None, idx=None, const=None, idx_ready=None):
        B, N, _ = xt.shape
        pooled = _point_max(xt)
        if const is not None:
            pooled = torch.cat((const, pooled), 1)
        xs = _small_seq(self.fc, pooled, self.training)
        if self.level == 1:
            dec, bn = self.upsample_cov[0], self.upsample_cov[1]
        else:
            dec, bn = self.upsample_cov, self.bn_uc
        x_ec = dec.forward_cl(xt, pct, idx=idx, const=const, idx_ready=idx_ready)
        x_ec = _bn_act(x_ec.reshape(B * 2 * N, -1), bn, self.training).view(B, 2 * N, -1)
        g = _small_seq(self.g_fc, xs, self.training) if self.level < 4 else None
        return xs, x_ec, g

    def forward(self, x, pc=None, idx=None):
        xs, x_ec, g = self.forward_cl(x.transpose(1, 2).contiguous(),
                                      pc.transpose(1, 2).contiguous() if pc is not None else None, idx=idx)
        _deconv.flush_bn_counters()
        N2 = x_ec.shape[1]
        x_ec = x_ec.transpose(1, 2)
        x_out = torch.cat((xs.unsqueeze(2).expand(-1, -1, N2), x_ec), 1)
        if g is None:
            return x_out
        return x_out, torch.cat((g.unsqueeze(2).expand(-1, -1, N2), x_ec), 1)


def _mlp_head(cin):
    return nn.Sequential(nn.Conv1d(cin, 256, 1), nn.LeakyReLU(inplace=True), nn.Conv1d(256, 64, 1),
                         nn.LeakyReLU(inplace=True), nn.Conv1d(64, 3, 1, bias=True))


class PointGenerator(nn.Module):

    def __init__(self, num_point=2048, num_k=20, softmax=True, base_points=128):
        super().__init__()
        self.num_point, self.num_k, self.base_points = num_point, num_k, base_points
        self.fc1 = nn.Sequential(nn.Linear(128, 32 * base_points), nn.BatchNorm1d(32 * base_points),
                                 nn.LeakyReLU(inplace=True))
        self.bilateral1 = BilateralBlock(1, 32, 32, num_k)
        self.bilateral2 = BilateralBlock(2, 64, 64, num_k, softmax)
        self.bilateral3 = BilateralBlock(3, 128, 128, num_k, softmax)
        self.bilateral4 = BilateralBlock(4, 256, 256, num_k, softmax)
        self.mlp1, self.mlp2 = _mlp_head(512 + 32), _mlp_head(512 + 64)
        self.mlp3, self.mlp4 = _mlp_head(512 + 128), _mlp_head(512)

    def forward(self, z, idx=(None, None, None, None), stage_hook=None):
        s = self.begin(z)
        for lvl in range(4):
            self.level(s, lvl, idx, stage_hook)
        return self.finish(s)

    def begin(self, z):
        B = z.shape[0]
        xt = _small_seq(self.fc1, z, self.training).view(B, 32, self.base_points).transpose(1, 2).contiguous()
        return {"B": B, "xt": xt, "pct": None, "const": None, "clouds": [], "pending": (None, None)}

    def level(self, s, lvl, idx=(None, None, None, None), stage_hook=None):
        B = s["B"]
        blocks = (self.bilateral1, self.bilateral2, self.bilateral3, self.bilateral4)
        heads = (self.mlp1, self.mlp2, self.mlp3, self.mlp4)
        xt, pct, const, clouds = s["xt"], s["pct"], s["const"], s["clouds"]
        lvl_idx, lvl_ready = (idx[lvl], None) if idx[lvl] is not None else s["pending"]
        xs, x_ec, g = blocks[lvl].forward_cl(xt, pct, idx=lvl_idx, const=const, idx_ready=lvl_ready)
        s["pending"] = (None, None)
        if lvl < 3 and idx[lvl + 1] is None and x_ec.is_cuda:
            nxt = blocks[lvl + 1].upsample_cov
            s["pending"] = _deconv.start_feature_knn(x_ec, xs, nxt.k)
        M, Fo = x_ec.shape[1], x_ec.shape[2]
        rows = x_ec.reshape(B * M, Fo)
        if lvl < 3:
            p = _head_rows(heads[lvl], rows, B, g=g, n_const=512)
        else:
            p = _head_rows(heads[lvl], rows, B, g=xs, n_const=Fo)
        pct = p.view(B, M, 3)
        clouds.append(pct.transpose(1, 2))
        if stage_hook is not None:
            _deconv.flush_bn_counters()
            stage_hook(lvl, clouds[-1])
        s["xt"], s["const"], s["pct"] = x_ec, xs, pct

    def finish(self, s):
        _deconv.flush_bn_counters()
        return tuple(s["clouds"])

    def _deconvs(self):
        blocks = (self.bilateral1, self.bilateral2, self.bilateral3, self.bilateral4)
        return [(b.upsample_cov[0] if b.level == 1 else b.upsample_cov) for b in blocks]

    def preassemble(self, deepest_without_graph=False):
        decs = self._deconvs()
        for lvl, dec in enumerate(decs):
            Fc = 0 if lvl == 0 else dec.Fin - decs[lvl - 1].Fout
            if deepest_without_graph and lvl == len(decs) - 1:
                with torch.no_grad():
                    dec.preassemble(Fc)
            else:
                dec.preassemble(Fc)

    def drop_preassembled(self):
        for dec in self._deconvs():
            dec.drop_preassembled()

    def forward_hints(self):
        return [dec.forward_hints() for dec in self._deconvs()]

    def restore_forward_hints(self, hints):
        for dec, h in zip(self._deconvs(), hints):
            dec.restore_forward_hints(h)


class PointDiscriminator(nn.Module):

    WIDTHS = {1: (64, 128, 256), 2: (64, 128, 256, 512), 3: (64, 128, 256, 512), 4: (64, 128, 256, 1024)}
    HIDDEN = {1: (128, 64), 2: (256, 64), 3: (256, 64), 4: (512, 256, 64)}

    def __init__(self, level, num_point=None):
        super().__init__()
        self.level = level
        self.num_point = num_point if num_point is not None else 128 << level
        layers, cin = [], 3
        for w in self.WIDTHS[level]:
            layers += [nn.Conv1d(cin, w, 1), nn.BatchNorm1d(w), nn.LeakyReLU(inplace=True)]
            cin = w
        self.fc1 = nn.Sequential(*layers)
        mlp = []
        for h in self.HIDDEN[level]:
            mlp += [nn.Linear(cin, h), nn.LeakyReLU(inplace=True)]
            cin = h
        mlp.append(nn.Linear(cin, 1))
        self.mlp = nn.Sequential(*mlp)

    def forward(self, x, aug=None):
        B, _, N = x.shape
        h = x.transpose(1, 2).reshape(B * N, 3) if aug is None else aug.rows(x)
        last = len(self.fc1) - 3
        for i in range(0, last, 3):
            y, part = _linear_stats(h, _deconv._w2d(self.fc1[i]), self.training)
            h = _deconv.bn_act(y, self.fc1[i + 1], self.training, pre_bias=self.fc1[i].bias, partials=part)
        w_last = _deconv._w2d(self.fc1[last])
        y, part = _linear_stats(h, w_last, self.training and not _deconv.STATS_MAX)
        pooled = _deconv.bn_act_maxpool(y, self.fc1[last + 1], self.training, B, N, pre_bias=self.fc1[last].bias, partials=part,
                                        dense=_deconv.DenseInput(h, w_last))
        _deconv.flush_bn_counters()
        return _small_seq(self.mlp, pooled, self.training)


def PointDiscriminator_1(num_point=256):
    return PointDiscriminator(1, num_point)


def PointDiscriminator_2(num_point=512):
    return PointDiscriminator(2, num_point)


def PointDiscriminator_3(num_point=1024):
    return PointDiscriminator(3, num_point)


def PointDiscriminator_4(num_point=2048):
    return PointDiscriminator(4, num_point)


def load_reference_state_dict(module, state_dict):
    clean = {(k[len("module."):] if k.startswith("module.") else k): v for k, v in state_dict.items()}
    return module.load_state_dict(clean, strict=True)
```

Measured before the change: 3.085 million points/s.

## Fuse discriminator last GEMM with BN stats and max-pool epilogue

Adds a pooled GEMM epilogue that, instead of writing the full B*N x C product, emits per-block partial sums, shifted sum-of-squares and row max/min with argmax/argmin. A finalize kernel combines these into BN statistics and pooled outputs, and saves the best pre-activation value so backward no longer gathers from the full activation. This is meant to remove the large intermediate write/read of the last discriminator layer. The cost is an extra finalize kernel and a more complex epilogue. Stats now come from shifted partials combined in double, so numerics differ slightly from the previous path.

```diff
diff --git a/include/pdgn_hip.h b/include/pdgn_hip.h
--- a/include/pdgn_hip.h
+++ b/include/pdgn_hip.h
@@ -12,7 +12,7 @@
 
 typedef void *pdgn_stream_t;
 
-#define PDGN_ABI_VERSION 38
+#define PDGN_ABI_VERSION 39
 int pdgn_abi_version(void);
 
 int pdgn_knnquery(int b, int n, int m, int nsample, const float *xyz, const float *new_xyz,
@@ -115,6 +115,17 @@
 int pdgn_dense_bn_maxpool_input_grad(int b, int n, int c, int k, int act, const float *x, const float *dout,
                                      const int32_t *yarg, const float *stats, const float *h, int ldh,
                                      const float *W, int ldw, float *scratch, float *dh, pdgn_stream_t stream);
+
+long long pdgn_gemm_nt_pooled_part_rows(long long m, int n, int k, int rows_per_sample);
+int pdgn_gemm_nt_pooled_block_rows(long long m, int n, int k, int rows_per_sample);
+int pdgn_gemm_nt_pooled(long long m, int n, int k, const float *A, int lda, const float *W, int ldw, int rows_per_sample,
+                        float *part, pdgn_stream_t stream);
+int pdgn_bn_pooled_finalize(int b, int n, int c, int act, float eps, float momentum, long long nparts, int block_rows,
+                            const float *part, const float *gamma, const float *beta, const float *pre_bias, float *running_mean,
+                            float *running_var, float *stats, float *ymax, int32_t *yarg, float *xbest, pdgn_stream_t stream);
+int pdgn_dense_bn_maxpool_backward_pooled(int b, int n, int c, int k, int act, const float *xbest, const float *dout,
+                                          const int32_t *yarg, const float *stats, const float *h, int ldh, const float *W, int ldw,
+                                          float *scratch, float *dh, float *dW, int lddw, float *bsums, pdgn_stream_t stream);
 
 int pdgn_group_colsum(long long groups, long long group_rows, int c, const float *x, long long ldx, float *out,
                       pdgn_stream_t stream);
diff --git a/pdgn_amd/csrc/bnact.hip b/pdgn_amd/csrc/bnact.hip
--- a/pdgn_amd/csrc/bnact.hip
+++ b/pdgn_amd/csrc/bnact.hip
@@ -960,7 +960,8 @@
                                                               const float *__restrict__ x, const float *__restrict__ dout,
                                                               const int32_t *__restrict__ yarg, const float *__restrict__ stats,
                                                               float *__restrict__ dz, float *__restrict__ bsums,
-                                                              float *__restrict__ coef, float *__restrict__ zero, int nzero) {
+                                                              float *__restrict__ coef, float *__restrict__ zero, int nzero,
+                                                              const float *__restrict__ xbest) {
     __shared__ double p1[16][17], p2[16][17];
     for (int e = blockIdx.x * 256 + threadIdx.x; e < nzero; e += gridDim.x * 256) zero[e] = 0.f;
     const int cl = threadIdx.x & 15, bl = threadIdx.x >> 4;
@@ -974,7 +975,7 @@
         const float sh = stats[C + c];
         for (int b = bl; b < B; b += 16) {
             const int n = yarg[b * C + c];
-            const float v = x[((size_t)b * N + n) * C + c];
+            const float v = xbest ? xbest[b * C + c] : x[((size_t)b * N + n) * C + c];
             const float g = dout[b * C + c] * act_grad(__fmaf_rn(v, sc, sh), act);
             dz[b * C + c] = g;
             s1 += g;
@@ -1078,7 +1079,7 @@
     hipStream_t s = (hipStream_t)stream;
     float *dz = scratch, *coef = scratch + (size_t)b * c;
     hipLaunchKernelGGL(cl_max_bwd_sums_kernel, dim3(cdiv(c, 16)), dim3(256), 0, s, b, n, c, act, training, x, dout, yarg,
-                       stats, dz, bsums, coef, nullptr, 0);
+                       stats, dz, bsums, coef, nullptr, 0, nullptr);
     int cgb, gx;
     mp_geometry(c, &cgb, &gx);
     hipLaunchKernelGGL(cl_max_bwd_apply_kernel, dim3(gx, MP_SPLIT, b), dim3(BN_THREADS), 0, s, n, c, cgb, x, stats, coef, dz,
@@ -1297,10 +1298,11 @@
     return (long long)b * c + 2LL * c + 2LL * ((long long)k * k + k) + (long long)c * k;
 }
 
-extern "C" int pdgn_dense_bn_maxpool_backward(int b, int n, int c, int k, int act, const float *x, const float *dout,
-                                              const int32_t *yarg, const float *stats, const float *h, int ldh, const float *W,
-                                              int ldw, float *scratch, float *dh, float *dW, int lddw, float *bsums,
-                                              pdgn_stream_t stream) {
+static int dense_bn_maxpool_backward(int b, int n, int c, int k, int act, const float *x, const float *xbest, const float *dout,
+                                     const int32_t *yarg, const float *stats, const float *h, int ldh, const float *W,
+                                     int ldw, float *scratch, float *dh, float *dW, int lddw, float *bsums,
+                                     pdgn_stream_t stream) {
+    if ((x == nullptr) == (xbest == nullptr)) return PDGN_ERR_INVALID;
     if (b < 1 || n < 1 || n > 65535 || c < 4 || c % 4 || k < 4 || k % 4 || k > 256 || ldw % 4 || ((uintptr_t)W & 15) ||
         ((uintptr_t)dh & 15) || act < 0 || act > 2 || b > 65535 || cf_scatter_lds(n, c) > 64 * 1024)
         return PDGN_ERR_INVALID;
@@ -1311,7 +1313,7 @@
     float *dz = scratch, *coef = dz + (size_t)b * c, *G = coef + 2 * (size_t)c, *v = G + kk, *H = v + k, *hs = H + kk, *T = hs + k;
     float *bs = bsums ? bsums : T;
     hipLaunchKernelGGL(cl_max_bwd_sums_kernel, dim3(cdiv(c, 16)), dim3(256), 0, s, b, n, c, act, 1, x, dout, yarg, stats, dz, bs,
-                       coef, G, (int)(2 * (kk + k)));
+                       coef, G, (int)(2 * (kk + k)), xbest);
     int rc = pdgn_launch_status();
     if (rc) return rc;
     if (dh) {
@@ -1334,6 +1336,18 @@
     }
     return rc;
 }
+extern "C" int pdgn_dense_bn_maxpool_backward(int b, int n, int c, int k, int act, const float *x, const float *dout,
+                                              const int32_t *yarg, const float *stats, const float *h, int ldh, const float *W,
+                                              int ldw, float *scratch, float *dh, float *dW, int lddw, float *bsums,
+                                              pdgn_stream_t stream) {
+    return dense_bn_maxpool_backward(b, n, c, k, act, x, nullptr, dout, yarg, stats, h, ldh, W, ldw, scratch, dh, dW, lddw, bsums, stream);
+}
+extern "C" int pdgn_dense_bn_maxpool_backward_pooled(int b, int n, int c, int k, int act, const float *xbest, const float *dout,
+                                                     const int32_t *yarg, const float *stats, const float *h, int ldh, const float *W,
+                                                     int ldw, float *scratch, float *dh, float *dW, int lddw, float *bsums,
+                                                     pdgn_stream_t stream) {
+    return dense_bn_maxpool_backward(b, n, c, k, act, nullptr, xbest, dout, yarg, stats, h, ldh, W, ldw, scratch, dh, dW, lddw, bsums, stream);
+}
 
 extern "C" long long pdgn_dense_bn_maxpool_input_grad_scratch(int b, int c, int k) {
     return pdgn_dense_bn_maxpool_backward_scratch(b, c, k);
@@ -1344,6 +1358,92 @@
                                                 const float *W, int ldw, float *scratch, float *dh, pdgn_stream_t stream) {
     return pdgn_dense_bn_maxpool_backward(b, n, c, k, act, x, dout, yarg, stats, h, ldh, W, ldw, scratch, dh, nullptr, 4, nullptr,
                                           stream);
+}
+
+#define PF_CH 8
+#define PF_PL 64
+__global__ __launch_bounds__(PF_CH * PF_PL) void cl_pooled_finalize_kernel(
+    int B, int N, int C, int nparts, int rpp, int act, float eps, float momentum, const float *__restrict__ part,
+    const float *__restrict__ gamma, const float *__restrict__ beta, const float *__restrict__ pre_bias,
+    float *__restrict__ running_mean, float *__restrict__ running_var, float *__restrict__ stats, float *__restrict__ ymax,
+    int32_t *__restrict__ yarg, float *__restrict__ xbest) {
+    __shared__ double red[PF_PL][PF_CH], red2[PF_PL][PF_CH];
+    __shared__ float s_sc[PF_CH], s_sh[PF_CH];
+    const int cl = threadIdx.x % PF_CH, pl = threadIdx.x / PF_CH;
+    const int c = blockIdx.x * PF_CH + cl;
+    const bool ok = c < C;
+    const double R = (double)B * (double)N, n = (double)rpp, inv = 1.0 / (double)rpp;
+    double a = 0, b = 0;
+    if (ok)
+#pragma unroll 4
+        for (int p = pl; p < nparts; p += PF_PL) {
+            const float *q = part + (size_t)p * 7 * C + c;
+            const double s = (double)q[0], sq = (double)q[C], pv = (double)q[2 * C];
+            const double mb = pv + s * inv;
+            a += n * mb;
+            b += (sq - s * s * inv) + n * mb * mb;
+        }
+    red[pl][cl] = a;
+    red2[pl][cl] = b;
+    __syncthreads();
+    for (int h = PF_PL / 2; h > 0; h >>= 1) {
+        if (pl < h) {
+            red[pl][cl] += red[pl + h][cl];
+            red2[pl][cl] += red2[pl + h][cl];
+        }
+        __syncthreads();
+    }
+    if (ok && pl == 0) {
+        const double mean = red[0][cl] / R;
+        double var = red2[0][cl] / R - mean * mean;
+        var = var < 0 ? 0 : var;
+        const float invstd = (float)(1.0 / sqrt(var + (double)eps));
+        const float g = gamma ? gamma[c] : 1.f, be = beta ? beta[c] : 0.f;
+        const float scale = g * invstd, shift = be - (float)mean * scale;
+        stats[c] = scale;
+        stats[C + c] = shift;
+        stats[2 * C + c] = (float)mean;
+        stats[3 * C + c] = invstd;
+        s_sc[cl] = scale;
+        s_sh[cl] = shift;
+        if (running_mean) {
+            const double unbiased = R > 1 ? var * R / (R - 1) : var;
+            const float mb = (float)mean + (pre_bias ? pre_bias[c] : 0.f);
+            running_mean[c] = (1.f - momentum) * running_mean[c] + momentum * mb;
+            running_var[c] = (1.f - momentum) * running_var[c] + momentum * (float)unbiased;
+        }
+    }
+    __syncthreads();
+    if (!ok) return;
+    const float sc = s_sc[cl], sh = s_sh[cl];
+    const bool up = sc >= 0.f;
+    const int pps = N / rpp;
+    for (int bb = pl; bb < B; bb += PF_PL) {
+        const float *q = part + ((size_t)bb * pps) * 7 * C + (up ? 3 : 5) * C + c;
+        float best = q[0];
+        int arg = __float_as_int(q[C]);
+#pragma unroll 8
+        for (int s = 1; s < pps; ++s) {
+            const float v = q[(size_t)s * 7 * C];
+            const int r = __float_as_int(q[(size_t)s * 7 * C + C]);
+            if (up ? v > best : v < best) { best = v; arg = r; }
+        }
+        ymax[(size_t)bb * C + c] = act_fwd(__fmaf_rn(best, sc, sh), act);
+        yarg[(size_t)bb * C + c] = arg;
+        xbest[(size_t)bb * C + c] = best;
+    }
+}
+
+extern "C" int pdgn_bn_pooled_finalize(int b, int n, int c, int act, float eps, float momentum, long long nparts, int block_rows,
+                                       const float *part, const float *gamma, const float *beta, const float *pre_bias,
+                                       float *running_mean, float *running_var, float *stats, float *ymax, int32_t *yarg,
+                                       float *xbest, pdgn_stream_t stream) {
+    if (b < 1 || n < 1 || c < 4 || act < 0 || act > 2 || block_rows < 1 || n % block_rows || nparts != (long long)b * (n / block_rows) ||
+        nparts > 0x7fffffffLL || !part || !stats || !ymax || !yarg || !xbest)
+        return PDGN_ERR_INVALID;
+    hipLaunchKernelGGL(cl_pooled_finalize_kernel, dim3(cdiv(c, PF_CH)), dim3(PF_CH * PF_PL), 0, (hipStream_t)stream, b, n, c, (int)nparts,
+                       block_rows, act, eps, momentum, part, gamma, beta, pre_bias, running_mean, running_var, stats, ymax, yarg, xbest);
+    return pdgn_launch_status();
 }
 
 __global__ __launch_bounds__(256) void group_colsum_kernel(long long group_rows, int C, const float *__restrict__ x, long long ldx,
diff --git a/pdgn_amd/csrc/gemm_shared.h b/pdgn_amd/csrc/gemm_shared.h
--- a/pdgn_amd/csrc/gemm_shared.h
+++ b/pdgn_amd/csrc/gemm_shared.h
@@ -51,6 +51,8 @@
     const unsigned short *Wp;
     long long wplane;
     const unsigned *max_a, *max_w;
+    float *pool_part;
+    int pool_n;
 };
 
 __device__ __forceinline__ int x2_exponent(unsigned maxbits) {
diff --git a/pdgn_amd/csrc/gemm_x3.hip b/pdgn_amd/csrc/gemm_x3.hip
--- a/pdgn_amd/csrc/gemm_x3.hip
+++ b/pdgn_amd/csrc/gemm_x3.hip
@@ -88,15 +88,17 @@
     return x3_dpp_add<0x118, 0xf>(v);
 }
 
-template <int TM, int TN, int WM, int WN, int OCC, bool ATOMIC, bool WT, bool AT, bool EPI = false, bool PW = false, int MS = 32, int NP = 3>
+template <int TM, int TN, int WM, int WN, int OCC, bool ATOMIC, bool WT, bool AT, bool EPI = false, bool PW = false, int MS = 32, int NP = 3,
+          bool POOL = false>
 __global__ __launch_bounds__(64 * WM * WN, OCC) void gemm_x3_kernel(const NtArgs p) {
     static_assert(!PW || (!WT && !AT), "pre-split second operand: row-major (N x K) planes only");
     static_assert(MS == 32 || MS == 16, "matrix instruction: 32x32x16 or 16x16x32");
     static_assert(NP == 3 || (NP == 2 && MS == 32), "parts: three bf16, or two fp16 on the 32x32x16 instruction");
+    static_assert(!POOL || (MS == 32 && !ATOMIC && !EPI && !WT && !AT), "pooled epilogue: plain row-major product on the 32x32x16 instruction");
     constexpr int NW = WM * WN, NTH = 64 * NW, BM = 32 * TM * WM, BN = 32 * TN * WN;
     constexpr int PART_A = BM * 64, PART_W = BN * 64, STAGE = NP * (PART_A + PART_W);
     constexpr int UNT = NP == 2 ? (BM + BN) * 4 : 0;
-    constexpr bool STG = OCC == 1 && !ATOMIC && !(X3_ABLATE & 128) && 2 * STAGE + NW * 4096 + UNT <= 160 * 1024;
+    constexpr bool STG = OCC == 1 && !ATOMIC && !POOL && !(X3_ABLATE & 128) && 2 * STAGE + NW * 4096 + UNT <= 160 * 1024;
     __shared__ __attribute__((aligned(1024))) unsigned char smem[2 * STAGE + (STG ? NW * 4096 : 0) + UNT];
     float *const untab = reinterpret_cast<float *>(smem + 2 * STAGE + (STG ? NW * 4096 : 0));
 
@@ -496,7 +498,7 @@
         const int n0 = tn * BN;
         const bool to_ws = !ATOMIC && p.sk_ws != nullptr;
         if (NP == 2) {
-            if (!ATOMIC) {
+            if (!ATOMIC && !POOL) {
                 float ua[TM];
 #pragma unroll
                 for (int a = 0; a < TM; ++a) ua[a] = untab[mloc0 + 32 * a];
@@ -524,7 +526,49 @@
         }
         const long long mrows = to_ws ? BM : min((long long)BM, p.M - m0);
         const int ncols = to_ws ? BN : min(BN, p.N - n0);
-        if (!ATOMIC) {
+        if (POOL) {
+            const int nla = wn * 32 * TN + li;
+            const int row0 = (int)((m0 + wm * 32 * TM) % p.pool_n);
+            float *P = p.pool_part + ((size_t)tm * WM + wm) * 7 * p.N + n0;
+#pragma unroll
+            for (int b = 0; b < TN; ++b) {
+                const float pv = __int_as_float(__builtin_amdgcn_ds_bpermute(4 * li, __float_as_int(acc[0][b][0])));
+                float cs = 0.f, cq = 0.f, mx = -INFINITY, mn = INFINITY;
+                int amx = 0, amn = 0;
+#pragma unroll
+                for (int a = 0; a < TM; ++a)
+#pragma unroll
+                    for (int j = 0; j < 16; ++j) {
+                        const float x = acc[a][b][j];
+                        const int r = 32 * a + 8 * (j >> 2) + (j & 3);
+                        const float d = x - pv;
+                        cs += d;
+                        cq = __fmaf_rn(d, d, cq);
+                        if (x > mx) { mx = x; amx = r; }
+                        if (x < mn) { mn = x; amn = r; }
+                    }
+                amx += 4 * lg;
+                amn += 4 * lg;
+                const int o = 4 * (lane ^ 32);
+                const float os = __int_as_float(__builtin_amdgcn_ds_bpermute(o, __float_as_int(cs)));
+                const float oq = __int_as_float(__builtin_amdgcn_ds_bpermute(o, __float_as_int(cq)));
+                const float omx = __int_as_float(__builtin_amdgcn_ds_bpermute(o, __float_as_int(mx)));
+                const float omn = __int_as_float(__builtin_amdgcn_ds_bpermute(o, __float_as_int(mn)));
+                const int oamx = __builtin_amdgcn_ds_bpermute(o, amx), oamn = __builtin_amdgcn_ds_bpermute(o, amn);
+                if (omx > mx || (omx == mx && oamx < amx)) { mx = omx; amx = oamx; }
+                if (omn < mn || (omn == mn && oamn < amn)) { mn = omn; amn = oamn; }
+                const int nl = nla + 32 * b;
+                if (lg == 0 && nl < ncols) {
+                    P[nl] = cs + os;
+                    P[p.N + nl] = cq + oq;
+                    P[2 * p.N + nl] = pv;
+                    P[3 * p.N + nl] = mx;
+                    P[4 * p.N + nl] = __int_as_float(row0 + amx);
+                    P[5 * p.N + nl] = mn;
+                    P[6 * p.N + nl] = __int_as_float(row0 + amn);
+                }
+            }
+        } else if (!ATOMIC) {
             if (to_ws) rsC = __builtin_amdgcn_make_buffer_rsrc((void *)(p.sk_ws + (size_t)(p.sk_seg ? v * p.sk_seg + (cp.j - 1) : v) * BM * BN), 0,
                                                                BM * BN * 4, 0x00020000);
             else rsC = __builtin_amdgcn_make_buffer_rsrc((void *)(p.C + m0 * p.ldc + n0), 0, (int)(mrows * p.ldc * 4), 0x00020000);
@@ -704,7 +748,7 @@
                             if (STG) {
                                 if (a + b > 0) flush_block(b ? a : a - 1, b ? b - 1 : TN - 1);
                                 stage_block(a, b);
-                            } else if (!ATOMIC) {
+                            } else if (!ATOMIC && !POOL) {
                                 store_block(a, b);
                             }
 #pragma unroll
@@ -715,11 +759,11 @@
                         if (NP == 2) {
                             const int u = t + 4 - NPROD;
                             const u32x4 ap = u <= 1 ? A.l : A.h, wp = (u == 0 || u == 2) ? W.l : W.h;
-                            acc[a][b] = ATOMIC ? x2_mfma(ap, wp, c) : x2_mfma(wp, ap, c);
+                            acc[a][b] = (ATOMIC || POOL) ? x2_mfma(ap, wp, c) : x2_mfma(wp, ap, c);
                         } else {
                         const u32x4 ap = t == 0 ? A.l : (t == 1 || t == 3) ? A.m : A.h;
                         const u32x4 wp = t == 2 ? W.l : (t == 1 || t == 4) ? W.m : W.h;
-                        acc[a][b] = ATOMIC ? x3_mfma(ap, wp, c) : x3_mfma(wp, ap, c);
+                        acc[a][b] = (ATOMIC || POOL) ? x3_mfma(ap, wp, c) : x3_mfma(wp, ap, c);
                         }
                         if (idx % X3_FENCE == 0) __builtin_amdgcn_sched_barrier(0);
                         if (!(X3_ABLATE & 16)) {
@@ -768,7 +812,7 @@
                     if (STG) {
                         if (sb > 0) flush_block((sb - 1) / TN, (sb - 1) % TN);
                         stage_block(a32, b32);
-                    } else if (!ATOMIC) {
+                    } else if (!ATOMIC && !POOL) {
                         store_block(a32, b32);
                     }
                 }
@@ -903,7 +947,7 @@
         __builtin_amdgcn_sched_barrier(0);
         next_item(cp);
     }
-    if (!ATOMIC) {
+    if (!ATOMIC && !POOL) {
 #pragma unroll
         for (int a = 0; a < TM; ++a)
 #pragma unroll
@@ -1227,6 +1271,31 @@
         return (long long)at_slices(pl) * T * BM * BN;
     }
 
+    static constexpr int POOL_WM_TWO = 4;
+    static int launch_pool(long long m, int n, int k, const float *A, int lda, const float *W, int ldw, int rows_per_sample, float *part,
+                           bool two, hipStream_t s) {
+        const Plan pl = plan(m, n, k, false);
+        NtArgs a = {};
+        a.M = m; a.N = n; a.K = k; a.lda = lda; a.ldw = ldw; a.ldc = n;
+        a.A = A; a.W = W;
+        a.rows_per_group = 1;
+        a.pool_part = part; a.pool_n = rows_per_sample;
+        if (two) {
+            if (CFG != 0) return PDGN_ERR_INVALID;
+            const unsigned *hand_a = x2_cur_max_a, *hand_w = x2_cur_max_w;
+            x2_cur_max_a = x2_cur_max_w = nullptr;
+            a.max_a = hand_a ? hand_a : x2_scan(A, m, k, lda, false, s);
+            a.max_w = hand_w ? hand_w : x2_scan(W, n, k, ldw, false, s);
+            if (!a.max_a || !a.max_w) return PDGN_ERR_INVALID;
+        }
+        a.tiles_m = pl.tiles_m; a.tiles_n = pl.tiles_n; a.kchunks = pl.kchunks;
+        a.tile_begin = 0; a.tile_end = pl.tiles_m * pl.tiles_n; a.sk_per_wg = 0;
+        const int grid = a.tile_end < nt_cus() * WG_PER_CU ? a.tile_end : nt_cus() * WG_PER_CU;
+        if (two) x3_launch_h2(32, grid, s, a, true);
+        else hipLaunchKernelGGL((gemm_x3_kernel<TM, TN, WM, WN, OCC, false, false, false, false, false, 32, 3, true>), dim3(grid), dim3(64 * WM * WN), 0, s, a);
+        return pdgn_launch_status();
+    }
+
     template <bool WT, bool AT = false>
     static int launch(long long m, int n, int k, const float *A, int lda, const float *W, int ldw, const float *bias,
                       const float *addend, int ldadd, float *C, int ldc, float *stat_part, hipStream_t s,
@@ -1245,6 +1314,7 @@
         a.sk_ws = nullptr;
         a.sk_seg = 0;
         a.max_a = a.max_w = nullptr;
+        a.pool_part = nullptr; a.pool_n = 0;
         const unsigned *hand_a = x2_cur_max_a, *hand_w = x2_cur_max_w;
         x2_cur_max_a = x2_cur_max_w = nullptr;
         const bool two = Wp ? parts == 2
@@ -1436,6 +1506,52 @@
     return x3_dispatch<false>(m, n, k, A, lda, W, ldw, bias, addend, ldadd, C, ldc, stat_part, (hipStream_t)stream);
 }
 
+struct X3PoolPlan {
+    int cfg;
+    bool two;
+    int block_rows;
+    long long part_rows;
+};
+static X3PoolPlan x3_pool_plan(long long m, int n, int k, int rows_per_sample) {
+    X3PoolPlan pp = {-1, false, 0, 0};
+    if (!x3_mode() || m < 1 || n < 4 || k < 4 || n % 4 || k % 4 || rows_per_sample < 1 || m % rows_per_sample || m >= (1LL << 31)) return pp;
+    pp.two = x2_pays(x3_pick(m, n, k, false), m, n, k, (long long)m * k * 4 + (long long)n * k * 4);
+    int cfg = pp.two ? 0 : x3_pick(m, n, k, true);
+    if (cfg == 0 && rows_per_sample % X3Big::BM) {
+        if (pp.two) return pp;
+        cfg = X3Square::plan(m, n, k, false).cost <= X3Narrow::plan(m, n, k, false).cost ? 1 : 2;
+    }
+    if (rows_per_sample % (cfg == 0 ? X3Big::BM : X3Square::BM)) return pp;
+    if (!pp.two && x3_shape16(cfg, false, false, false)) return pp;
+    const int bm = cfg == 0 ? X3Big::BM : X3Square::BM;
+    const int wm = pp.two ? X3Big::POOL_WM_TWO : 2;
+    pp.cfg = cfg;
+    pp.block_rows = bm / wm;
+    pp.part_rows = m / pp.block_rows;
+    return pp;
+}
+extern "C" long long pdgn_gemm_nt_pooled_part_rows(long long m, int n, int k, int rows_per_sample) {
+    const X3PoolPlan pp = x3_pool_plan(m, n, k, rows_per_sample);
+    return pp.cfg < 0 ? PDGN_ERR_INVALID : pp.part_rows;
+}
+extern "C" int pdgn_gemm_nt_pooled_block_rows(long long m, int n, int k, int rows_per_sample) {
+    const X3PoolPlan pp = x3_pool_plan(m, n, k, rows_per_sample);
+    return pp.cfg < 0 ? PDGN_ERR_INVALID : pp.block_rows;
+}
+extern "C" int pdgn_gemm_nt_pooled(long long m, int n, int k, const float *A, int lda, const float *W, int ldw, int rows_per_sample,
+                                   float *part, pdgn_stream_t stream) {
+    const X3Handover handover;
+    if (!x3_mode() || !part || !x3_args_ok(m, n, k, lda, ldw, 0, n, nullptr, false)) return PDGN_ERR_INVALID;
+    const X3PoolPlan pp = x3_pool_plan(m, n, k, rows_per_sample);
+    hipStream_t s = (hipStream_t)stream;
+    switch (pp.cfg) {
+        case 0: return X3Big::launch_pool(m, n, k, A, lda, W, ldw, rows_per_sample, part, pp.two, s);
+        case 1: return X3Square::launch_pool(m, n, k, A, lda, W, ldw, rows_per_sample, part, false, s);
+        case 2: return X3Narrow::launch_pool(m, n, k, A, lda, W, ldw, rows_per_sample, part, false, s);
+        default: return PDGN_ERR_INVALID;
+    }
+}
+
 extern "C" int pdgn_gemm_nn(long long m, int n, int k, const float *A, int lda, const float *Wt, int ldw,
                             const float *bias, const float *addend, int ldadd, float *C, int ldc, float *stat_part,
                             pdgn_stream_t stream) {
diff --git a/pdgn_amd/csrc/gemm_x3_h2.hip b/pdgn_amd/csrc/gemm_x3_h2.hip
--- a/pdgn_amd/csrc/gemm_x3_h2.hip
+++ b/pdgn_amd/csrc/gemm_x3_h2.hip
@@ -20,6 +20,7 @@
 }
 
 const void *x3_symbol_h2(int flags, bool eight_waves) {
+    if (flags == 32) return eight_waves ? (const void *)gemm_x3_kernel<2, 2, 4, 2, 1, false, false, false, false, false, 32, 2, true> : nullptr;
     return eight_waves ? x2_symbol_tile<2, 2, 4, 2>(flags) : x2_symbol_tile<4, 2, 2, 2>(flags);
 }
 
diff --git a/pdgn_amd/deconv.py b/pdgn_amd/deconv.py
--- a/pdgn_amd/deconv.py
+++ b/pdgn_amd/deconv.py
@@ -12,6 +12,7 @@
                     small_sequential, bn_act_maxpool, bn_softmax_slots_permute, flush_bn_counters,
                     has_zero_colsum, linear_cl, softmax_slots_permute, DenseInput, group_colsum, mark_maxima, row_maxima_buffer)
 from .fused import _STATS_MAX as STATS_MAX
+from .fused import dense_bn_act_maxpool
 
 F32, I32 = torch.float32, torch.int32
 _KNN_OVERLAP = __import__("os").environ.get("PDGN_KNN_OVERLAP", "1") == "1"
diff --git a/pdgn_amd/fused.py b/pdgn_amd/fused.py
--- a/pdgn_amd/fused.py
+++ b/pdgn_amd/fused.py
@@ -59,6 +59,7 @@
 _CLOSED_TAIL = os.environ.get("PDGN_CLOSED_TAIL", "1") == "1"
 _STATS_MAX = os.environ.get("PDGN_STATS_MAX", "1") == "1"
 _CLOSED_DW = os.environ.get("PDGN_CLOSED_DW", "1") == "1"
+_POOLED_TAIL = os.environ.get("PDGN_POOLED_TAIL", "1") == "1"
 
 
 class DenseInput:
@@ -1152,6 +1153,90 @@
                               ACT[act], B, N, pre_bias, partials, dense)
 
 
+class DenseBNActMaxPool(Function):
+
+    @staticmethod
+    def forward(ctx, h, w, gamma, beta, running_mean, running_var, momentum, eps, act, B, N, pre_bias=None):
+        L = _lib.lib()
+        rows, K = h.shape
+        C = w.shape[0]
+        dev = h.device
+        _slots(h)
+        if GEMM_LOG is not None:
+            GEMM_LOG.append(("nt", rows, C, K))
+        nparts = L.pdgn_gemm_nt_pooled_part_rows(rows, C, K, N)
+        block = L.pdgn_gemm_nt_pooled_block_rows(rows, C, K, N)
+        if nparts < 0 or block < 0:
+            raise _lib.PdgnHipError("pdgn_gemm_nt_pooled refuses (%d, %d, %d) in samples of %d rows" % (rows, C, K, N))
+        g, b = gamma.detach().contiguous(), beta.detach().contiguous()
+        pb = pre_bias.detach().contiguous() if pre_bias is not None else None
+        part = torch.empty((nparts, 7 * C), dtype=F32, device=dev)
+        stats = torch.empty(4 * C, dtype=F32, device=dev)
+        ymax = torch.empty((B, C), dtype=F32, device=dev)
+        xbest = torch.empty((B, C), dtype=F32, device=dev)
+        yarg = torch.empty((B, C), dtype=torch.int32, device=dev)
+        st = stream_of(h)
+        check(L.pdgn_gemm_nt_pooled(rows, C, K, ptr(h), h.stride(0), ptr(w), w.stride(0), N, ptr(part), st), "pdgn_gemm_nt_pooled")
+        check(L.pdgn_bn_pooled_finalize(B, N, C, act, eps, momentum, nparts, block, ptr(part), ptr(g), ptr(b), ptr(pb), ptr(running_mean),
+                                        ptr(running_var), ptr(stats), ptr(ymax), ptr(yarg), ptr(xbest), st), "pdgn_bn_pooled_finalize")
+        ctx.save_for_backward(h, w, stats, yarg, xbest)
+        ctx.cfg = (B, N, C, K, act)
+        ctx.has_pre_bias = pre_bias is not None
+        ctx.mark_non_differentiable(yarg, xbest)
+        return ymax, yarg, xbest
+
+    @staticmethod
+    def backward(ctx, dout, *unused):
+        h, w, stats, yarg, xbest = ctx.saved_tensors
+        B, N, C, K, act = ctx.cfg
+        dev = h.device
+        L = _lib.lib()
+        dout = dout.contiguous()
+        want_h, want_w, want_bn = ctx.needs_input_grad[0], ctx.needs_input_grad[1], any(ctx.needs_input_grad[2:4])
+        scr = torch.empty(L.pdgn_dense_bn_maxpool_backward_scratch(B, C, K), dtype=F32, device=dev)
+        dh = torch.empty((B * N, K), dtype=F32, device=dev) if want_h else None
+        dw = torch.empty((C, K), dtype=F32, device=dev) if want_w else None
+        bs = torch.empty(2 * C, dtype=F32, device=dev) if want_bn else None
+        check(L.pdgn_dense_bn_maxpool_backward_pooled(B, N, C, K, act, ptr(xbest), ptr(dout), ptr(yarg), ptr(stats), ptr(h), h.stride(0),
+                                                      ptr(w), w.stride(0), ptr(scr), ptr(dh), ptr(dw), K, ptr(bs), stream_of(h)),
+              "pdgn_dense_bn_maxpool_backward_pooled")
+        return (dh, dw, bs[C:] if want_bn else None, bs[:C] if want_bn else None, None, None, None, None, None, None, None,
+                _pre_bias_grad(ctx.has_pre_bias, C, dev))
+
+
+def set_pooled_tail(on):
+    global _POOLED_TAIL
+    old, _POOLED_TAIL = _POOLED_TAIL, bool(on)
+    return old
+
+
+def pooled_tail_takes(h, w, bn, training, B, N, pre_bias=None):
+    if not (_POOLED_TAIL and training and _CLOSED_TAIL and _STATS_MAX and not _NO_FOLD and h.is_cuda and h.dim() == 2 and w.dim() == 2):
+        return False
+    rows, C = h.shape[0], w.shape[0]
+    if rows != B * N or C % 4 or not _lib.matrix_core_mode() or bn.weight is None or bn.running_mean is None or bn.momentum is None:
+        return False
+    if pre_bias is not None and pre_bias.requires_grad and not _CLOSED_DW:
+        return False
+    K = w.shape[1]
+    if not (h.shape[1] == K and K % 4 == 0 and K <= 256 and h.dtype == F32 and w.dtype == F32 and h.stride(1) == 1 and w.stride(1) == 1
+            and h.stride(0) % 4 == 0 and w.stride(0) % 4 == 0 and h.data_ptr() % 16 == 0 and w.data_ptr() % 16 == 0
+            and (h.requires_grad or w.requires_grad) and torch.is_grad_enabled()
+            and (not w.requires_grad or (_CLOSED_DW and K >= 16 and (K & (K - 1)) == 0))
+            and B <= 65535 and N <= 65535 and 2 * (N + min(N, C) + C) + 1040 + 4 * C <= 65536):
+        return False
+    return _lib.lib().pdgn_gemm_nt_pooled_part_rows(rows, C, K, N) > 0
+
+
+def dense_bn_act_maxpool(h, w, bn, training, B, N, act="leaky_relu", pre_bias=None):
+    if not pooled_tail_takes(h, w, bn, training, B, N, pre_bias):
+        return None
+    if bn.track_running_stats:
+        _PENDING_COUNTS[bn.num_batches_tracked] = _PENDING_COUNTS.get(bn.num_batches_tracked, 0) + 1
+    return DenseBNActMaxPool.apply(h, w, bn.weight, bn.bias, bn.running_mean, bn.running_var, bn.momentum, bn.eps, ACT[act], B, N,
+                                   pre_bias)[0]
+
+
 class PointMax(Function):
 
     @staticmethod
diff --git a/pdgn_amd/generator.py b/pdgn_amd/generator.py
--- a/pdgn_amd/generator.py
+++ b/pdgn_amd/generator.py
@@ -204,9 +204,11 @@
             y, part = _linear_stats(h, _deconv._w2d(self.fc1[i]), self.training)
             h = _deconv.bn_act(y, self.fc1[i + 1], self.training, pre_bias=self.fc1[i].bias, partials=part)
         w_last = _deconv._w2d(self.fc1[last])
-        y, part = _linear_stats(h, w_last, self.training and not _deconv.STATS_MAX)
-        pooled = _deconv.bn_act_maxpool(y, self.fc1[last + 1], self.training, B, N, pre_bias=self.fc1[last].bias, partials=part,
-                                        dense=_deconv.DenseInput(h, w_last))
+        pooled = _deconv.dense_bn_act_maxpool(h, w_last, self.fc1[last + 1], self.training, B, N, pre_bias=self.fc1[last].bias)
+        if pooled is None:
+            y, part = _linear_stats(h, w_last, self.training and not _deconv.STATS_MAX)
+            pooled = _deconv.bn_act_maxpool(y, self.fc1[last + 1], self.training, B, N, pre_bias=self.fc1[last].bias, partials=part,
+                                            dense=_deconv.DenseInput(h, w_last))
         _deconv.flush_bn_counters()
         return _small_seq(self.mlp, pooled, self.training)
 
```

Result: no change. 3.113 million points/s, median of 6 (+0.9%).
